# PolarisRisingWar/rgb-experiment

Measured on AMD Instinct MI355X. Metric: aggregated edges/sec (full-graph GCN d=128, reference epoch = train fwd+bwd+Adam + 2 eval fwd), higher is better.
Workload: dtype f32

## Files before the change

include/rgbx_hip.h:

```cpp
#ifndef RGBX_HIP_H
#define RGBX_HIP_H

#include <stddef.h>
#include <stdint.h>

#ifdef __cplusplus
extern "C" {
#endif

#define RGBX_VERSION 501

#define RGBX_OK 0
#define RGBX_E_ARG (-1)
#define RGBX_E_RANGE (-2)
#define RGBX_E_ALIGN (-3)
#define RGBX_E_WS (-4)
#define RGBX_E_SHAPE (-5)

typedef void* rgbx_stream_t;

enum {
  RGBX_LOOPS_KEEP = 0,
  RGBX_LOOPS_ADD_REMAINING = 1,
  RGBX_LOOPS_REMOVE_ADD = 2
// ... 169 lines not shown
  int64_t N, K, Nout;
  const rgbx_row_split_t* split;
  const float* w_pos;
  float* z_pos_out;
  const uint8_t* col_sel;
} rgbx_fused_layer_t;

int rgbx_fused_layer_f32(const rgbx_fused_layer_t* layer, rgbx_stream_t stream);

int rgbx_blocked_to_rows_f32(const float* src, int64_t blk_cols, int64_t blk_stride, float* dst, int64_t ldd,
                             int64_t n, int64_t d, const float* bias, rgbx_stream_t stream);

int rgbx_appnp_f32(const int32_t* rowptr, const int32_t* col, const float* w, const float* h,
                   int64_t ldh, float* out, float* tmp, int64_t ldo, int64_t N, int64_t d, int K,
                   float alpha, const rgbx_row_split_t* split, rgbx_stream_t stream);


int rgbx_dagnn_gate_fwd_f32(const float* h0, int64_t ld0, const float* hops, int64_t hop_stride, int64_t ldh,
                            const float* s, const float* b, float* out, int64_t ldo, int64_t N, int64_t d, int K,
                            rgbx_stream_t stream);

int rgbx_dagnn_gate_bwd_workspace_bytes(int64_t d, size_t* bytes);
int rgbx_dagnn_gate_bwd_f32(const float* h0, int64_t ld0, const float* hops, int64_t hop_stride, int64_t ldh,
                            const float* s, const float* b, const float* gout, int64_t ldg, float* d0,
                            int64_t ldd0, float* dk, int64_t d_stride, int64_t ldd, float* g_s, float* g_b,
                            void* ws, size_t ws_bytes, int64_t N, int64_t d, int K, rgbx_stream_t stream);


int rgbx_gru_step_supported(int64_t C);
int rgbx_gru_step_f32(const int32_t* rowptr, const int32_t* col, const float* x, int64_t ldx, const float* wt,
                      const float* wt_root, const float* bias, float* out, int64_t ldo, float* z_out, int64_t ldz,
                      float* pre_out, int64_t ldp, int64_t N, int64_t C, const rgbx_row_split_t* split,
                      rgbx_stream_t stream);

int rgbx_gru_gate_fwd_f32(const float* pre, int64_t ldp, const float* x, int64_t ldx, float* out, int64_t ldo,
                          int64_t N, int64_t C, rgbx_stream_t stream);

int rgbx_gru_gate_bwd_f32(const float* pre, int64_t ldp, const float* x, int64_t ldx, const float* gout, int64_t ldg,
                          float* dpre, int64_t lddp, float* dx, int64_t lddx, int64_t N, int64_t C,
                          rgbx_stream_t stream);


int rgbx_gat_scores_f32(const float* hfeat, int64_t ldh, const float* att_src,
                        const float* att_dst, float* a_src, float* a_dst, int64_t n, int H, int C,
                        rgbx_stream_t stream);

int rgbx_gat_scores_bwd_scratch_floats(int64_t n, int H, int C, int64_t* count);

int rgbx_gat_scores_bwd_f32(const float* hfeat, int64_t ldh, const float* g_a_src, const float* g_a_dst,
                            int64_t n_dst, const float* att_src, const float* att_dst, float* g_hfeat,
                            int64_t ldgh, float* g_att_src, float* g_att_dst, float* scratch,
                            int64_t scratch_floats, int64_t n, int H, int C, rgbx_stream_t stream);

int rgbx_gat_aggregate_fwd_f32(const int32_t* rowptr, const int32_t* col, const float* hfeat,
                               int64_t ldh, const float* a_src, const float* att_src,
                               float* a_dst, const float* att_dst, const float* out_scale, const float* bias,
                               float* out, int64_t ldo, float* m, float* rden, float* out_pos, float* a_pos,
                               int64_t N, int H, int C, float slope, const rgbx_row_split_t* split,
                               rgbx_stream_t stream);

int rgbx_gat_edge_softmax_f32(const int32_t* rowptr, const int32_t* col, const float* a_src, const float* a_dst,
                              float slope, float* alpha, float* alpha_pos, float* m, float* rden, float* a_pos,
                              int64_t N, const rgbx_row_split_t* split, rgbx_stream_t stream);

int rgbx_gat_bwd_dst_f32(const int32_t* rowptr, const int32_t* col, const float* hfeat,
                         int64_t ldh, const float* a_src, const float* a_dst, const float* m,
                         const float* rden, const float* out, int64_t ldo, const float* gout,
                         int64_t ldg, float* nodeq, float* g_a_dst, int64_t N, int H, int C,
                         float slope, rgbx_stream_t stream);

int rgbx_gat_bwd_prep_f32(const float* a_dst, const float* m, const float* rden, const float* out,
                          int64_t ldo, const float* bias, const float* gout, int64_t ldg, float* nodeq,
                          const float* out_pos, const float* a_pos, float slope, float* g_a_dst,
                          int64_t N, int H, int C, rgbx_stream_t stream);

int rgbx_gat_bwd_src_f32(const int32_t* rowptr_t, const int32_t* col_t, const float* hfeat,
                         int64_t ldh, const float* a_src, const float* nodeq, const float* gout,
                         int64_t ldg, float* g_hfeat, int64_t ldgh, float* g_a_src, float* ds,
                         const float* att2, const float* g_a_dst, int64_t N, int H, int C, float slope,
                         const rgbx_row_split_t* split, rgbx_stream_t stream);



int rgbx_supergat_supported(int H, int C);

int rgbx_supergat_loss_records(int64_t N, const rgbx_row_split_t* split, int64_t* count);

int rgbx_supergat_aggregate_fwd_f32(const int32_t* rowptr, const int32_t* col, const float* hfeat, int64_t ldh,
                                    const float* att_l, const float* att_r, const float* bias, float* out, int64_t ldo,
                                    float* m, float* rden, int64_t N, int H, int C, float slope, const uint32_t* seed,
                                    float p_drop, float pos_ratio, float* loss_records, int64_t n_loss_records,
                                    double* pos_stats, const rgbx_row_split_t* split, rgbx_stream_t stream);

int rgbx_supergat_bwd_dst_f32(const int32_t* rowptr, const int32_t* col, const float* hfeat, int64_t ldh,
                              const float* att_l, const float* att_r, const float* m, const float* rden,
                              const float* out, int64_t ldo, const float* bias, const float* gout, int64_t ldg,
                              float* nodeq, float* g_hfeat, int64_t ldgh, float* g_ar, int64_t N, int H, int C,
                              float slope, const uint32_t* seed, float p_drop, float pos_ratio, const float* gl,
                              const rgbx_row_split_t* split, rgbx_stream_t stream);

int rgbx_supergat_bwd_src_f32(const int32_t* rowptr_t, const int32_t* col_t, const int32_t* t2f, const float* hfeat,
                              int64_t ldh, const float* att_l, const float* nodeq, const float* gout, int64_t ldg,
                              float* g_hfeat, int64_t ldgh, float* g_al, int64_t N, int H, int C, float slope,
                              const uint32_t* seed, float p_drop, float pos_ratio, const float* gl,
                              const rgbx_row_split_t* split, rgbx_stream_t stream);

int rgbx_supergat_sample_negatives(const uint64_t* keys, int64_t n_keys, int64_t N, const uint32_t* seed, int64_t n_neg,
                                   int redraws, int64_t* neg, uint8_t* valid, rgbx_stream_t stream);

int rgbx_supergat_neg_loss_fwd_f32(const float* hfeat, int64_t ldh, const int64_t* neg, const uint8_t* valid,
                                   int64_t n_neg, int H, int C, float* loss_records, int64_t n_loss_records,
                                   double* neg_stats, rgbx_stream_t stream);

int rgbx_supergat_neg_loss_bwd_f32(const float* hfeat, int64_t ldh, const int64_t* neg, const uint8_t* valid,
                                   int64_t n_neg, int H, int C, const float* gl, float* g_hfeat, int64_t ldgh,
                                   rgbx_stream_t stream);

int rgbx_supergat_draws_u8(const uint32_t* seed, int64_t nnz, int H, float p_drop, float pos_ratio, uint8_t* pos,
                           uint8_t* drop, rgbx_stream_t stream);



int rgbx_gatv2_supported(int H, int C);

int rgbx_gatv2_fwd_f32(const int32_t* rowptr, const int32_t* col, const float* xl, int64_t ldl, const float* xr,
                       int64_t ldr, const float* att, const float* bias, float* out, int64_t ldo, float* m, float* rden,
                       int64_t N, int H, int C, float slope, const uint32_t* seed, float p_drop,
                       const rgbx_row_split_t* split, rgbx_stream_t stream);

int rgbx_gatv2_att_partial_floats(int64_t N, int H, int C, const rgbx_row_split_t* split, int64_t* count);

int rgbx_gatv2_bwd_dst_f32(const int32_t* rowptr, const int32_t* col, const float* xl, int64_t ldl, const float* xr,
                           int64_t ldr, const float* att, const float* m, const float* rden, const float* out,
                           int64_t ldo, const float* bias, const float* gout, int64_t ldg, float* nodeq, float* g_xr,
                           int64_t ldgr, float* g_att, float* att_partial, int64_t n_att_partial, int64_t N, int H,
                           int C, float slope, const uint32_t* seed, float p_drop, const rgbx_row_split_t* split,
                           rgbx_stream_t stream);

int rgbx_gatv2_bwd_src_f32(const int32_t* rowptr_t, const int32_t* col_t, const int32_t* t2f, const float* xl,
                           int64_t ldl, const float* xr, int64_t ldr, const float* att, const float* nodeq,
                           const float* gout, int64_t ldg, float* g_xl, int64_t ldgl, int64_t N, int H, int C,
                           float slope, const uint32_t* seed, float p_drop, const rgbx_row_split_t* split,
                           rgbx_stream_t stream);

int rgbx_gatv2_draws_u8(const uint32_t* seed, int64_t nnz, int H, float p_drop, uint8_t* keep, rgbx_stream_t stream);


int rgbx_gemm_tn_workspace_bytes(int64_t K, int64_t M, int64_t N, size_t* bytes);

int rgbx_gemm_tn_f32(const float* A, int64_t lda, const float* B, int64_t ldb, float* C, int64_t ldc,
                     float* a_colsum, int64_t K, int64_t M, int64_t N, float alpha, void* workspace,
                     size_t workspace_bytes, rgbx_stream_t stream);


int rgbx_bn_scratch_doubles(int64_t N, int64_t d, int64_t* count);

int rgbx_bn_stats_f32(const float* x, int64_t ldx, int64_t N, int64_t d, double* sums, double* scratch,
                      int64_t scratch_doubles, rgbx_stream_t stream);

int rgbx_bn_finalize_f32(const double* packed, const float* weight, const float* bias, float eps, float momentum,
                         float* running_mean, float* running_var, float* mean, float* rstd, float* scale,
                         float* shift, int64_t d, rgbx_stream_t stream);

int rgbx_fold_bn_linear_f32(const float* W, int64_t ldw, const float* Wr, int64_t ldwr, const float* bias,
                            const float* bias2, const float* gamma, const float* beta, const float* running_mean,
                            const float* running_var, float eps, float* wt, float* wrt, float* b_out, int64_t Nout,
                            int64_t K, rgbx_stream_t stream);

int rgbx_bn_bwd_finalize_f32(const double* glob, const double* local, const double* count, const float* weight,
                             const float* rstd, float* ca, float* cb, float* ck, float* g_weight, float* g_bias,
                             int64_t d, rgbx_stream_t stream);

int rgbx_affine_cols_f32(const float* x, int64_t ldx, const float* scale, const float* shift, float* y,
                         int64_t ldy, int64_t N, int64_t d, rgbx_stream_t stream);

int rgbx_bn_bwd_reduce_f32(const float* gy, int64_t ldg, const float* x, int64_t ldx, const float* mean,
                           const float* rstd, int64_t N, int64_t d, double* sums, double* scratch,
                           int64_t scratch_doubles, rgbx_stream_t stream);

int rgbx_bn_bwd_apply_f32(const float* gy, int64_t ldg, const float* x, int64_t ldx, const float* mean,
                          const float* rstd, const float* ca, const float* cb, const float* ck, float* gx,
                          int64_t ldgx, int64_t N, int64_t d, rgbx_stream_t stream);


int rgbx_masked_nll_scratch_doubles(int64_t N, int want_accuracy, int64_t* count);

int rgbx_masked_nll_fwd_f32(const float* logp, int64_t ld, const int64_t* y, const uint8_t* mask,
                            int64_t N, int64_t C, double* stats, double* scratch,
                            int64_t scratch_doubles, int want_accuracy, rgbx_stream_t stream);

int rgbx_masked_nll_bwd_f32(const int64_t* y, const uint8_t* mask, int64_t N, int64_t C,
                            const float* scale, float* grad, int64_t ldg, rgbx_stream_t stream);

int rgbx_masked_ce_fwd_f32(const float* logits, int64_t ld, const int64_t* y, const uint8_t* mask, int64_t N,
                           int64_t C, double* stats, double* scratch, int64_t scratch_doubles,
                           rgbx_stream_t stream);

int rgbx_masked_ce_fwd_blocked_f32(const float* logits, int64_t blk_cols, int64_t blk_stride, const float* bias,
                                   const int64_t* y, const uint8_t* mask, int64_t N, int64_t C, double* stats,
                                   double* scratch, int64_t scratch_doubles, rgbx_stream_t stream);

int rgbx_masked_ce_bwd_f32(const float* logits, int64_t ld, const int64_t* y, const uint8_t* mask, int64_t N,
                           int64_t C, const float* scale, float* grad, int64_t ldg, rgbx_stream_t stream);


int rgbx_coalesce_workspace_bytes(int64_t E, int64_t N, int mirror, size_t* bytes);
int rgbx_coalesce_keys_i64(const int64_t* row, const int64_t* col, int64_t E, int64_t N, int mirror,
                           uint64_t* keys_out, uint64_t* counts, void* workspace, size_t workspace_bytes,
                           rgbx_stream_t stream);
int rgbx_split_edge_keys_i64(const uint64_t* keys, const uint64_t* counts, int64_t cap, int64_t N, int64_t* out_row,
                             int64_t* out_col, rgbx_stream_t stream);

int rgbx_py_random_shuffle_i64(int64_t seed, int64_t n, int64_t* perm);


int rgbx_gather_rows_f32(const float* src, int64_t lds, const int32_t* idx, int64_t n, int64_t d,
                         float* dst, int64_t ldd, rgbx_stream_t stream);

int rgbx_scatter_add_rows_f32(const float* src, int64_t lds, const int32_t* idx, int64_t n,
                              int64_t d, float* dst, int64_t ldd, rgbx_stream_t stream);

int rgbx_paced_copy_f32(const float* src, float* dst, int64_t n, int workgroups, int nontemporal, rgbx_stream_t stream);



int rgbx_faconv_supported(int64_t C);

int rgbx_faconv_scores_f32(const float* x, int64_t ldx, const float* att_l, const float* att_r, float* alr, int64_t N,
                           int64_t C, rgbx_stream_t stream);

int rgbx_faconv_fwd_f32(const int32_t* rowptr, const int32_t* col, const float* w, const float* x, int64_t ldx,
                        const float* alr, const float* x0, int64_t ldx0, float eps, float* out, int64_t ldo, int64_t N,
                        int64_t C, const uint32_t* seed, float p_drop, const rgbx_row_split_t* split,
                        rgbx_stream_t stream);

int rgbx_faconv_bwd_dst_f32(const int32_t* rowptr, const int32_t* col, const float* w, const float* x, int64_t ldx,
                            const float* alr, const float* gout, int64_t ldg, float* g_alr, int64_t N, int64_t C,
                            const uint32_t* seed, float p_drop, const rgbx_row_split_t* split, rgbx_stream_t stream);

int rgbx_faconv_bwd_src_f32(const int32_t* rowptr_t, const int32_t* col_t, const float* w_t, const int32_t* t2f,
                            const float* x, int64_t ldx, const float* alr, const float* gout, int64_t ldg,
                            const float* att_l, const float* att_r, float* g_alr, float* g_x, int64_t ldgx, int64_t N,
                            int64_t C, const uint32_t* seed, float p_drop, const rgbx_row_split_t* split,
                            rgbx_stream_t stream);

int rgbx_faconv_edge_coef_f32(const int32_t* rowptr, const int32_t* col, const float* w, const int32_t* slot,
                              const float* alr, int transposed, int64_t N, const uint32_t* seed, float p_drop,
                              float* coef, float* q, rgbx_stream_t stream);

int rgbx_faconv_edge_dot_f32(const int32_t* rowptr, const int32_t* col, const float* q, const float* a, int64_t lda,
                             const float* b, int64_t ldb, float* out, int64_t out_stride, int64_t N, int64_t C,
                             rgbx_stream_t stream);

int rgbx_faconv_draws_u8(const uint32_t* seed, int64_t nnz, float p_drop, uint8_t* keep, rgbx_stream_t stream);

#ifdef __cplusplus
}
#endif
#endif
```

rgb_experiment_amd/_lib.py:

```python
import ctypes
import os

import torch

_HERE = os.path.dirname(os.path.abspath(__file__))
LIB_PATH = os.path.join(_HERE, "csrc", "librgbx_hip.so")

_P = ctypes.c_void_p
_I64 = ctypes.c_int64
_I = ctypes.c_int
_F = ctypes.c_float

class RowSplit(ctypes.Structure):
    _fields_ = [("threshold", ctypes.c_int32), ("n_chunks", ctypes.c_int32), ("n_long", ctypes.c_int32),
                ("chunk_begin", ctypes.c_void_p), ("chunk_end", ctypes.c_void_p), ("chunk_row", ctypes.c_void_p),
                ("long_row", ctypes.c_void_p),
                ("long_chunk_ptr", ctypes.c_void_p), ("partial", ctypes.c_void_p)]


class MultiOut(ctypes.Structure):
    _fields_ = [(f, t) for name in ("sum", "mean", "var", "std", "max", "argmax", "min", "argmin")
                for f, t in ((name, ctypes.c_void_p), ("ld_" + name, ctypes.c_int64))]


class MultiGrad(ctypes.Structure):
    _fields_ = [(f, t) for name in ("a", "b", "x", "gmax", "argmax", "gmin", "argmin")
                for f, t in ((name, ctypes.c_void_p), ("ld_" + name, ctypes.c_int64))]


class CeEpilogue(ctypes.Structure):
    _fields_ = [("y", ctypes.c_void_p), ("mask", ctypes.c_void_p), ("grad_scale", ctypes.c_void_p),
                ("stats", ctypes.c_void_p), ("scratch", ctypes.c_void_p), ("mask_groups", ctypes.c_int32),
                ("rows", ctypes.c_void_p), ("n_rows", ctypes.c_int64), ("skip_unselected", ctypes.c_int32)]


class SpmmEpilogue(ctypes.Structure):
    _fields_ = [("ce", ctypes.c_void_p), ("n_classes", ctypes.c_int64), ("out_colsums", ctypes.c_void_p),
                ("stats_ws", ctypes.c_void_p), ("stats_ws_bytes", ctypes.c_size_t)]


class FusedLayer(ctypes.Structure):
    _fields_ = [("rowptr", _P), ("col", _P), ("w", _P), ("rs", _P), ("x", _P), ("ldx", _I64),
                ("x_blk_cols", _I64), ("x_blk_stride", _I64), ("wt", _P), ("x_root", _P), ("ldr", _I64),
                ("xr_blk_cols", _I64), ("xr_blk_stride", _I64), ("wt_root", _P), ("bias", _P), ("out", _P),
                ("ldo", _I64), ("out_blk", _P), ("ob_cols", _I64), ("ob_stride", _I64), ("z_out", _P), ("ldz", _I64),
                ("pre_scale", _P), ("pre_shift", _P), ("pre_rowsum", _P), ("out_colsums", _P), ("stats_ws", _P),
                ("stats_ws_bytes", ctypes.c_size_t), ("ce", _P), ("N", _I64), ("K", _I64), ("Nout", _I64),
                ("split", _P), ("w_pos", _P), ("z_pos_out", _P), ("col_sel", _P)]


SIGNATURES = {
    "rgbx_csr_workspace_bytes": [_I64, _I64, ctypes.POINTER(ctypes.c_size_t)],
    "rgbx_csr_build": [_P, _P, _I64, _I64, _I, _P, _P, _P, _P, ctypes.c_size_t, _P],
    "rgbx_deg_inv_sqrt_f32": [_P, _I64, _P, _P],
    "rgbx_gcn_norm_f32": [_P, _P, _I64, _P, _P, _P],
    "rgbx_inv_degree_f32": [_P, _I64, _P, _P],
    "rgbx_loop_weights_f32": [_P, _P, _P, _I64, _I64, _I, _F, _P, _P, _P],
    "rgbx_edge_slot_weights_f32": [_P, _I64, _P, _I64, _P, _P, _P],
    "rgbx_weighted_deg_inv_sqrt_f32": [_P, _P, _I64, _P, _P],
    "rgbx_gcn_norm_weighted_f32": [_P, _P, _P, _I64, _P, _P, _P],
    "rgbx_edge_dot_supported": [_I64],
    "rgbx_edge_dot_f32": [_P, _P, _P, _I64, _P, _I64, _P, _I64, _I64, _P, _P],
    "rgbx_gcn_norm_bwd_f32": [_P, _P, _P, _P, _P, _P, _P, _P, _P, _P, _I64, _I64, _P, _P, _P],
    "rgbx_spmm_csr_f32": [_P, _P, _P, _P, _P, _I64, _P, _I64, _P, _P, _I64, _I64, _I64, _F, _F, _P, _P],
    "rgbx_spmm_csr_extremum_supported": [_I64],
    "rgbx_spmm_csr_extremum_f32": [_P, _P, _P, _I64, _P, _I64, _P, _I64, _I64, _I, _P, _P],
    "rgbx_extremum_bwd_f32": [_P, _P, _P, _P, _I64, _P, _P, _I64, _I64, _I64, _P, _P],
    "rgbx_spmm_csr_multi_supported": [_I64],
    "rgbx_spmm_csr_multi_partial_words": [_I64, _I64, _I, ctypes.POINTER(ctypes.c_int64)],
    "rgbx_spmm_csr_multi_f32": [_P, _P, _P, _I64, _P, _I64, _I64, _P, _P],
    "rgbx_multi_bwd_f32": [_P, _P, _P, _P, _P, _I64, _I64, _I64, _P, _P],
    "rgbx_spmm_csr_epilogue_supported": [_I64],
    "rgbx_spmm_csr_epilogue_f32": [_P, _P, _P, _P, _P, _I64, _P, _I64, _P, _P, _I64, _I64, _I64, _F, _F, _P, _P, _P],
    "rgbx_spmm_csr_short_rows_supported": [_I64],
    "rgbx_spmm_csr_short_rows_f32": [_P, _P, _P, _P, _I64, _P, _P, _I64, _I64, _I64, _P],
    "rgbx_spmm_linear_supported": [_I64, _I64, _I],
    "rgbx_spmm_linear_stats_workspace_bytes": [_I64, _I64, ctypes.POINTER(ctypes.c_size_t)],
    "rgbx_spmm_linear_f32": [_P, _P, _P, _P, _P, _I64, _P, _P, _I64, _P, _P, _P, _I64, _P, _I64, _P, _P, _P, _P, _P,
                             ctypes.c_size_t, _P, _I64, _I64, _I64, _P, _P],
    "rgbx_fused_layer_f32": [_P, _P],
    "rgbx_blocked_to_rows_f32": [_P, _I64, _I64, _P, _I64, _I64, _I64, _P, _P],
    "rgbx_appnp_f32": [_P, _P, _P, _P, _I64, _P, _P, _I64, _I64, _I64, _I, _F, _P, _P],
    "rgbx_dagnn_gate_fwd_f32": [_P, _I64, _P, _I64, _I64, _P, _P, _P, _I64, _I64, _I64, _I, _P],
    "rgbx_dagnn_gate_bwd_workspace_bytes": [_I64, ctypes.POINTER(ctypes.c_size_t)],
    "rgbx_dagnn_gate_bwd_f32": [_P, _I64, _P, _I64, _I64, _P, _P, _P, _I64, _P, _I64, _P, _I64, _I64, _P, _P, _P,
                                ctypes.c_size_t, _I64, _I64, _I, _P],
    "rgbx_gru_step_supported": [_I64],
    "rgbx_gru_step_f32": [_P, _P, _P, _I64, _P, _P, _P, _P, _I64, _P, _I64, _P, _I64, _I64, _I64, _P, _P],
    "rgbx_gru_gate_fwd_f32": [_P, _I64, _P, _I64, _P, _I64, _I64, _I64, _P],
    "rgbx_gru_gate_bwd_f32": [_P, _I64, _P, _I64, _P, _I64, _P, _I64, _P, _I64, _I64, _I64, _P],
    "rgbx_gat_scores_f32": [_P, _I64, _P, _P, _P, _P, _I64, _I, _I, _P],
    "rgbx_gat_scores_bwd_scratch_floats": [_I64, _I, _I, ctypes.POINTER(ctypes.c_int64)],
    "rgbx_gat_scores_bwd_f32": [_P, _I64, _P, _P, _I64, _P, _P, _P, _I64, _P, _P, _P, _I64, _I64, _I, _I, _P],
    "rgbx_gat_aggregate_fwd_f32": [_P, _P, _P, _I64, _P, _P, _P, _P, _P, _P, _P, _I64, _P, _P, _P, _P, _I64, _I, _I, _F, _P,
                                   _P],
    "rgbx_gat_edge_softmax_f32": [_P, _P, _P, _P, _F, _P, _P, _P, _P, _P, _I64, _P, _P],
    "rgbx_gat_bwd_dst_f32": [_P, _P, _P, _I64, _P, _P, _P, _P, _P, _I64, _P, _I64, _P, _P, _I64, _I, _I,
                             _F, _P],
    "rgbx_gat_bwd_prep_f32": [_P, _P, _P, _P, _I64, _P, _P, _I64, _P, _P, _P, _F, _P, _I64, _I, _I, _P],
    "rgbx_gat_bwd_src_f32": [_P, _P, _P, _I64, _P, _P, _P, _I64, _P, _I64, _P, _P, _P, _P, _I64, _I, _I, _F, _P, _P],
    "rgbx_supergat_supported": [_I, _I],
    "rgbx_supergat_loss_records": [_I64, _P, ctypes.POINTER(ctypes.c_int64)],
    "rgbx_supergat_aggregate_fwd_f32": [_P, _P, _P, _I64, _P, _P, _P, _P, _I64, _P, _P, _I64, _I, _I, _F, _P, _F, _F, _P,
                                        _I64, _P, _P, _P],
    "rgbx_supergat_bwd_dst_f32": [_P, _P, _P, _I64, _P, _P, _P, _P, _P, _I64, _P, _P, _I64, _P, _P, _I64, _P, _I64, _I, _I,
                                  _F, _P, _F, _F, _P, _P, _P],
    "rgbx_supergat_bwd_src_f32": [_P, _P, _P, _P, _I64, _P, _P, _P, _I64, _P, _I64, _P, _I64, _I, _I, _F, _P, _F, _F, _P,
                                  _P, _P],
    "rgbx_supergat_sample_negatives": [_P, _I64, _I64, _P, _I64, _I, _P, _P, _P],
    "rgbx_supergat_neg_loss_fwd_f32": [_P, _I64, _P, _P, _I64, _I, _I, _P, _I64, _P, _P],
    "rgbx_supergat_neg_loss_bwd_f32": [_P, _I64, _P, _P, _I64, _I, _I, _P, _P, _I64, _P],
    "rgbx_supergat_draws_u8": [_P, _I64, _I, _F, _F, _P, _P, _P],
    "rgbx_gatv2_supported": [_I, _I],
    "rgbx_gatv2_fwd_f32": [_P, _P, _P, _I64, _P, _I64, _P, _P, _P, _I64, _P, _P, _I64, _I, _I, _F, _P, _F, _P, _P],
    "rgbx_gatv2_att_partial_floats": [_I64, _I, _I, _P, ctypes.POINTER(ctypes.c_int64)],
    "rgbx_gatv2_bwd_dst_f32": [_P, _P, _P, _I64, _P, _I64, _P, _P, _P, _P, _I64, _P, _P, _I64, _P, _P, _I64, _P, _P, _I64,
                               _I64, _I, _I, _F, _P, _F, _P, _P],
    "rgbx_gatv2_bwd_src_f32": [_P, _P, _P, _P, _I64, _P, _I64, _P, _P, _P, _I64, _P, _I64, _I64, _I, _I, _F, _P, _F, _P,
                               _P],
    "rgbx_gatv2_draws_u8": [_P, _I64, _I, _F, _P, _P],
    "rgbx_gemm_tn_workspace_bytes": [_I64, _I64, _I64, ctypes.POINTER(ctypes.c_size_t)],
    "rgbx_gemm_tn_f32": [_P, _I64, _P, _I64, _P, _I64, _P, _I64, _I64, _I64, _F, _P, ctypes.c_size_t, _P],
    "rgbx_bn_scratch_doubles": [_I64, _I64, ctypes.POINTER(ctypes.c_int64)],
    "rgbx_bn_stats_f32": [_P, _I64, _I64, _I64, _P, _P, _I64, _P],
    "rgbx_bn_finalize_f32": [_P, _P, _P, _F, _F, _P, _P, _P, _P, _P, _P, _I64, _P],
    "rgbx_fold_bn_linear_f32": [_P, _I64, _P, _I64, _P, _P, _P, _P, _P, _P, _F, _P, _P, _P, _I64, _I64, _P],
    "rgbx_bn_bwd_finalize_f32": [_P, _P, _P, _P, _P, _P, _P, _P, _P, _P, _I64, _P],
    "rgbx_affine_cols_f32": [_P, _I64, _P, _P, _P, _I64, _I64, _I64, _P],
    "rgbx_bn_bwd_reduce_f32": [_P, _I64, _P, _I64, _P, _P, _I64, _I64, _P, _P, _I64, _P],
    "rgbx_bn_bwd_apply_f32": [_P, _I64, _P, _I64, _P, _P, _P, _P, _P, _P, _I64, _I64, _I64, _P],
    "rgbx_masked_nll_scratch_doubles": [_I64, _I, ctypes.POINTER(ctypes.c_int64)],
    "rgbx_masked_nll_fwd_f32": [_P, _I64, _P, _P, _I64, _I64, _P, _P, _I64, _I, _P],
    "rgbx_masked_ce_fwd_f32": [_P, _I64, _P, _P, _I64, _I64, _P, _P, _I64, _P],
    "rgbx_masked_ce_fwd_blocked_f32": [_P, _I64, _I64, _P, _P, _P, _I64, _I64, _P, _P, _I64, _P],
    "rgbx_masked_ce_bwd_f32": [_P, _I64, _P, _P, _I64, _I64, _P, _P, _I64, _P],
    "rgbx_masked_nll_bwd_f32": [_P, _P, _I64, _I64, _P, _P, _I64, _P],
    "rgbx_coalesce_workspace_bytes": [_I64, _I64, _I, ctypes.POINTER(ctypes.c_size_t)],
    "rgbx_coalesce_keys_i64": [_P, _P, _I64, _I64, _I, _P, _P, _P, ctypes.c_size_t, _P],
    "rgbx_split_edge_keys_i64": [_P, _P, _I64, _I64, _P, _P, _P],
    "rgbx_gather_rows_f32": [_P, _I64, _P, _I64, _I64, _P, _I64, _P],
    "rgbx_scatter_add_rows_f32": [_P, _I64, _P, _I64, _I64, _P, _I64, _P],
    "rgbx_paced_copy_f32": [_P, _P, _I64, _I, _I, _P],
    "rgbx_py_random_shuffle_i64": [_I64, _I64, _P],
    "rgbx_faconv_supported": [_I64],
    "rgbx_faconv_scores_f32": [_P, _I64, _P, _P, _P, _I64, _I64, _P],
    "rgbx_faconv_fwd_f32": [_P, _P, _P, _P, _I64, _P, _P, _I64, _F, _P, _I64, _I64, _I64, _P, _F, _P, _P],
    "rgbx_faconv_bwd_dst_f32": [_P, _P, _P, _P, _I64, _P, _P, _I64, _P, _I64, _I64, _P, _F, _P, _P],
    "rgbx_faconv_bwd_src_f32": [_P, _P, _P, _P, _P, _I64, _P, _P, _I64, _P, _P, _P, _P, _I64, _I64, _I64, _P, _F, _P,
                                _P],
    "rgbx_faconv_edge_coef_f32": [_P, _P, _P, _P, _P, _I, _I64, _P, _F, _P, _P, _P],
    "rgbx_faconv_edge_dot_f32": [_P, _P, _P, _P, _I64, _P, _I64, _P, _I64, _I64, _I64, _P],
    "rgbx_faconv_draws_u8": [_P, _I64, _F, _P, _P],
}
EXPORTS = ["rgbx_version", "rgbx_last_error_string"] + list(SIGNATURES)

_lib = None


def bind(path, strict=True):
    lib = ctypes.CDLL(path)
    lib.rgbx_version.restype = _I
    lib.rgbx_version.argtypes = []
    lib.rgbx_last_error_string.restype = ctypes.c_char_p
    lib.rgbx_last_error_string.argtypes = []
    for name, argtypes in SIGNATURES.items():
        if not strict and not hasattr(lib, name):
            continue
        fn = getattr(lib, name)
        fn.restype = _I
        fn.argtypes = argtypes
    return lib


def load():
    global _lib
    if _lib is not None:
        return _lib
    if not os.path.exists(LIB_PATH):
        raise RuntimeError(
            f"rgb_experiment_amd: {LIB_PATH} is not built — run `python -c 'import __graft_entry__ as g; "
            "g.build()'` (or `make -C rgb_experiment_amd/csrc`). There is no CPU fallback.")
    _lib = bind(LIB_PATH)
    return _lib


def use(lib):
    global _lib
    _lib = lib


def check(rc, what):
    if rc != 0:
        msg = load().rgbx_last_error_string().decode(errors="replace")
        kind = "argument error" if rc < 0 else "hipError"
        raise RuntimeError(f"{what} failed ({kind} {rc}): {msg}")


def require_device(*tensors):
    for t in tensors:
        if t is not None and not t.is_cuda:
            raise RuntimeError(
                "rgb_experiment_amd: the message-passing path runs in HIP kernels on an MI355X device; "
                f"got a tensor on '{t.device}'. There is no CPU fallback (oracle/ is test-only).")


def stream_ptr():
    return torch.cuda.current_stream().cuda_stream


def ptr(t):
    return 0 if t is None else t.data_ptr()


def mat(t, name="tensor"):
    if t.dtype != torch.float32 or t.dim() != 2:
        raise RuntimeError(f"{name}: expected a 2-D float32 tensor, got {t.dtype} {tuple(t.shape)}")
    if t.size(1) > 1 and t.stride(1) != 1:
        raise RuntimeError(f"{name}: rows must be contiguous (stride {t.stride()})")
    ld = t.stride(0) if t.size(0) > 1 else max(t.size(1), 1)
    return t.data_ptr(), ld
```

rgb_experiment_amd/csrc/bn.hip:

```cpp
#include "rgbx_common.h"

namespace rgbx {
namespace {

constexpr int kMaxBlocks = 1024;

struct ColMap {
  int cv;
  int rg;
};

__host__ __device__ inline ColMap col_map(int d, int vec) {
  int cv = (d + vec - 1) / vec;
  if (cv > 256) cv = 256;
  ColMap m{cv, 256 / cv};
  return m;
}

template <int VEC, bool BWD>
__global__ void __launch_bounds__(256)
col_reduce_kernel(const float* __restrict__ a, int64_t lda, const float* __restrict__ b, int64_t ldb,
                  const float* __restrict__ mean, const float* __restrict__ rstd, int64_t N, int d,
                  double* __restrict__ part) {
  extern __shared__ double sh[];
  const ColMap M = col_map(d, VEC);
  const int tid = threadIdx.x;
  const int cvi = tid % M.cv, rgi = tid / M.cv;
  const bool thread_ok = rgi < M.rg;
  const int stride_c = M.cv * VEC;
  for (int cbase = 0; cbase < d; cbase += stride_c) {
    const int c = cbase + cvi * VEC;
    const bool active = thread_ok && c < d;
    double s0[VEC], s1[VEC];
    float mu[VEC], rs[VEC];
#pragma unroll
    for (int i = 0; i < VEC; ++i) { s0[i] = s1[i] = 0.0; mu[i] = 0.f; rs[i] = 1.f; }
    if (BWD && active) {
      load_vec<VEC>(mu, mean + c);
      load_vec<VEC>(rs, rstd + c);
    }
    if (active) {
      for (int64_t r = (int64_t)blockIdx.x * M.rg + rgi; r < N; r += (int64_t)gridDim.x * M.rg) {
        float va[VEC];
        load_vec<VEC>(va, a + r * lda + c);
        if constexpr (BWD) {
          float vb[VEC];
          load_vec<VEC>(vb, b + r * ldb + c);
#pragma unroll
          for (int i = 0; i < VEC; ++i) {
            s0[i] += (double)va[i];
            s1[i] += (double)(va[i] * ((vb[i] - mu[i]) * rs[i]));
          }
        } else {
#pragma unroll
          for (int i = 0; i < VEC; ++i) {
            s0[i] += (double)va[i];
            s1[i] += (double)va[i] * (double)va[i];
          }
        }
      }
    }
    __syncthreads();
    if (thread_ok) {
#pragma unroll
      for (int i = 0; i < VEC; ++i) {
        sh[(rgi * 2 + 0) * stride_c + cvi * VEC + i] = s0[i];
        sh[(rgi * 2 + 1) * stride_c + cvi * VEC + i] = s1[i];
      }
    }
    __syncthreads();
    if (rgi == 0 && active) {
#pragma unroll
      for (int i = 0; i < VEC; ++i) {
        if (c + i < d) {
          double t0 = 0.0, t1 = 0.0;
          for (int g = 0; g < M.rg; ++g) {
            t0 += sh[(g * 2 + 0) * stride_c + cvi * VEC + i];
            t1 += sh[(g * 2 + 1) * stride_c + cvi * VEC + i];
          }
          part[((int64_t)blockIdx.x * 2 + 0) * d + c + i] = t0;
          part[((int64_t)blockIdx.x * 2 + 1) * d + c + i] = t1;
        }
      }
    }
  }
}

__global__ void __launch_bounds__(256)
col_finish_kernel(const double* __restrict__ part, int n_blocks, int d, double* __restrict__ sums) {
  __shared__ double sh[32][8];
  const int j = threadIdx.x & 7, q = threadIdx.x >> 3;
  const int c = blockIdx.x * 8 + j;
  double s = 0.0;
  if (c < 2 * d) {
    const int which = c / d, col = c % d;
    for (int b = q; b < n_blocks; b += 32) s += part[((int64_t)b * 2 + which) * d + col];
  }
  sh[q][j] = s;
  __syncthreads();
  if (q == 0 && c < 2 * d) {
    double t = 0.0;
#pragma unroll
    for (int k = 0; k < 32; ++k) t += sh[k][j];
    sums[c] = t;
  }
}

template <int VEC>
__global__ void __launch_bounds__(256)
affine_kernel(const float* __restrict__ x, int64_t ldx, const float* __restrict__ scale,
              const float* __restrict__ shift, float* __restrict__ y, int64_t ldy, int64_t N, int d) {
  const int per_row = (d + VEC - 1) / VEC;
  const int64_t total = N * per_row;
  for (int64_t idx = (int64_t)blockIdx.x * blockDim.x + threadIdx.x; idx < total;
       idx += (int64_t)gridDim.x * blockDim.x) {
    const int64_t r = idx / per_row;
    const int c = (int)(idx % per_row) * VEC;
    float v[VEC], sc[VEC], sf[VEC];
    load_vec<VEC>(v, x + r * ldx + c);
    load_vec<VEC>(sc, scale + c);
    load_vec<VEC>(sf, shift + c);
#pragma unroll
    for (int i = 0; i < VEC; ++i) v[i] = fmaf(v[i], sc[i], sf[i]);
    store_vec<VEC>(y + r * ldy + c, v);
  }
}

template <int VEC>
__global__ void __launch_bounds__(256)
bn_bwd_apply_kernel(const float* __restrict__ gy, int64_t ldg, const float* __restrict__ x, int64_t ldx,
                    const float* __restrict__ mean, const float* __restrict__ rstd, const float* __restrict__ ca,
                    const float* __restrict__ cb, const float* __restrict__ ck, float* __restrict__ gx,
                    int64_t ldgx, int64_t N, int d) {
  const int per_row = (d + VEC - 1) / VEC;
  const int64_t total = N * per_row;
  for (int64_t idx = (int64_t)blockIdx.x * blockDim.x + threadIdx.x; idx < total;
       idx += (int64_t)gridDim.x * blockDim.x) {
    const int64_t r = idx / per_row;
    const int c = (int)(idx % per_row) * VEC;
    float g[VEC], v[VEC], mu[VEC], rs[VEC], a[VEC], b[VEC], k[VEC];
    load_vec<VEC>(g, gy + r * ldg + c);
    load_vec<VEC>(v, x + r * ldx + c);
    load_vec<VEC>(mu, mean + c);
    load_vec<VEC>(rs, rstd + c);
    load_vec<VEC>(a, ca + c);
    load_vec<VEC>(b, cb + c);
    load_vec<VEC>(k, ck + c);
#pragma unroll
    for (int i = 0; i < VEC; ++i) g[i] = (g[i] - a[i] - (v[i] - mu[i]) * rs[i] * b[i]) * k[i];
    store_vec<VEC>(gx + r * ldgx + c, g);
  }
}

int reduce_grid(int64_t N, int d, int vec) {
  const ColMap M = col_map(d, vec);
  int64_t b = cdiv(N, (int64_t)M.rg * 16);
  if (b > kMaxBlocks) b = kMaxBlocks;
  return (int)(b < 1 ? 1 : b);
}

bool vec4_ok(int64_t d, std::initializer_list<const void*> ptrs, std::initializer_list<int64_t> lds) {
  bool ok = d % 4 == 0;
  for (const void* p : ptrs) ok = ok && aligned16(p);
  for (int64_t ld : lds) ok = ok && ld % 4 == 0;
  return ok;
}

template <bool BWD>
int run_reduce(const float* a, int64_t lda, const float* b, int64_t ldb, const float* mean, const float* rstd,
               int64_t N, int64_t d, double* sums, double* scratch, int64_t scratch_doubles, hipStream_t s,
               const char* name) {
  if (N < 0 || d <= 0 || !sums) return fail(RGBX_E_ARG, "%s: bad argument", name);
  if (d >= INT32_MAX) return fail(RGBX_E_RANGE, "%s: d exceeds int32", name);
  if (N == 0) {
    RGBX_HIP(hipMemsetAsync(sums, 0, 2 * d * sizeof(double), s));
    return RGBX_OK;
  }
  if (!a || lda < d || (BWD && (!b || ldb < d || !mean || !rstd)) || !scratch)
    return fail(RGBX_E_ARG, "%s: null pointer or leading dimension < d", name);
  const bool v4 = BWD ? vec4_ok(d, {a, b, mean, rstd}, {lda, ldb}) : vec4_ok(d, {a}, {lda});
  const int vec = v4 ? 4 : 1;
  const int grid = reduce_grid(N, (int)d, vec);
  if (scratch_doubles < (int64_t)grid * 2 * d)
    return fail(RGBX_E_WS, "%s: scratch %lld < %lld doubles", name, (long long)scratch_doubles,
                (long long)grid * 2 * d);
  const ColMap M = col_map((int)d, vec);
  const size_t lds = (size_t)M.rg * 2 * M.cv * vec * sizeof(double);
  if (v4)
    col_reduce_kernel<4, BWD><<<grid, 256, lds, s>>>(a, lda, b, ldb, mean, rstd, N, (int)d, scratch);
  else
    col_reduce_kernel<1, BWD><<<grid, 256, lds, s>>>(a, lda, b, ldb, mean, rstd, N, (int)d, scratch);
  RGBX_CHECK_LAUNCH(name);
  col_finish_kernel<<<(int)cdiv(2 * d, 8), 256, 0, s>>>(scratch, grid, (int)d, sums);
  RGBX_CHECK_LAUNCH("col_finish_kernel");
  return RGBX_OK;
}

__global__ void __launch_bounds__(256)
bn_finalize_kernel(const double* __restrict__ packed, const float* __restrict__ weight,
                   const float* __restrict__ bias, float eps, float momentum, float* __restrict__ running_mean,
                   float* __restrict__ running_var, float* __restrict__ mean, float* __restrict__ rstd,
                   float* __restrict__ scale, float* __restrict__ shift, int d) {
  const int c = blockIdx.x * blockDim.x + threadIdx.x;
  if (c >= d) return;
  const double n = packed[2 * d];
  const double m64 = packed[c] / n;
  double v64 = packed[d + c] / n - m64 * m64;
  v64 = v64 > 0.0 ? v64 : 0.0;
  const float m = (float)m64, var = (float)v64;
  const float r = 1.0f / sqrtf(var + eps);
  const float sc = weight[c] * r;
  mean[c] = m;
  rstd[c] = r;
  scale[c] = sc;
  shift[c] = bias[c] - m * sc;
  if (running_mean) {
    const double nm1 = n > 1.0 ? n - 1.0 : 1.0;
    const float unbiased = var * (float)(n / nm1);
    running_mean[c] = running_mean[c] * (1.0f - momentum) + momentum * m;
    running_var[c] = running_var[c] * (1.0f - momentum) + momentum * unbiased;
  }
}

__global__ void __launch_bounds__(256)
bn_bwd_finalize_kernel(const double* __restrict__ glob, const double* __restrict__ local,
                       const double* __restrict__ count, const float* __restrict__ weight,
                       const float* __restrict__ rstd, float* __restrict__ ca, float* __restrict__ cb,
                       float* __restrict__ ck, float* __restrict__ g_weight, float* __restrict__ g_bias, int d) {
  const int c = blockIdx.x * blockDim.x + threadIdx.x;
  if (c >= d) return;
  const double n = *count;
  ca[c] = (float)(glob[c] / n);
  cb[c] = (float)(glob[d + c] / n);
  ck[c] = weight[c] * rstd[c];
  g_bias[c] = (float)local[c];
  g_weight[c] = (float)local[d + c];
}

__global__ void __launch_bounds__(256)
fold_bn_linear_kernel(const float* __restrict__ W, int64_t ldw, const float* __restrict__ Wr, int64_t ldwr,
                      const float* __restrict__ bias, const float* __restrict__ bias2,
                      const float* __restrict__ gamma, const float* __restrict__ beta,
                      const float* __restrict__ rmean, const float* __restrict__ rvar, float eps,
                      float* __restrict__ wt, float* __restrict__ wrt, float* __restrict__ b_out, int Nout, int K) {
  __shared__ float tile[2][32][33];
  __shared__ float sc[32];
  const int n0 = blockIdx.x * 32, k0 = blockIdx.y * 32;
  const int tx = threadIdx.x & 31, ty = threadIdx.x >> 5;
  if (threadIdx.x < 32) {
    const int n = n0 + threadIdx.x;
    float s = 1.f, t = 0.f;
    if (n < Nout && gamma) {
      s = gamma[n] * (1.0f / sqrtf(rvar[n] + eps));
      t = beta[n] - rmean[n] * s;
    }
    sc[threadIdx.x] = s;
    if (n < Nout && b_out && blockIdx.y == 0) {
      float b = bias ? bias[n] : 0.f;
      if (bias2) b += bias2[n];
      b_out[n] = b * s + t;
    }
  }
  for (int r = ty; r < 32; r += 8) {
    const int n = n0 + r, k = k0 + tx;
    const bool ok = n < Nout && k < K;
    tile[0][r][tx] = ok ? W[(int64_t)n * ldw + k] : 0.f;
    if (Wr) tile[1][r][tx] = ok ? Wr[(int64_t)n * ldwr + k] : 0.f;
  }
  __syncthreads();
  for (int r = ty; r < 32; r += 8) {
    const int k = k0 + r, n = n0 + tx;
    if (k < K && n < Nout) {
      wt[(int64_t)k * Nout + n] = tile[0][tx][r] * sc[tx];
      if (Wr) wrt[(int64_t)k * Nout + n] = tile[1][tx][r] * sc[tx];
    }
  }
}

int elt_grid(int64_t total) {
  int64_t b = cdiv(total, 256);
  return (int)(b < kMaxGrid ? (b < 1 ? 1 : b) : kMaxGrid);
}

}
}

using namespace rgbx;

extern "C" int rgbx_fold_bn_linear_f32(const float* W, int64_t ldw, const float* Wr, int64_t ldwr, const float* bias,
                                       const float* bias2, const float* gamma, const float* beta,
                                       const float* running_mean, const float* running_var, float eps, float* wt,
                                       float* wrt, float* b_out, int64_t Nout, int64_t K, rgbx_stream_t stream) {
  if (Nout <= 0 || K <= 0) return fail(RGBX_E_ARG, "fold_bn_linear: bad size");
  if (!W || !wt || (Wr && !wrt)) return fail(RGBX_E_ARG, "fold_bn_linear: null pointer");
  const bool bn = gamma || beta || running_mean || running_var;
  if (bn && !(gamma && beta && running_mean && running_var))
    return fail(RGBX_E_ARG, "fold_bn_linear: gamma, beta, running_mean and running_var go together");
  if (ldw < K || (Wr && ldwr < K)) return fail(RGBX_E_ARG, "fold_bn_linear: leading dimension too small");
  if (Nout >= INT32_MAX || K >= INT32_MAX) return fail(RGBX_E_RANGE, "fold_bn_linear: size exceeds int32");
  dim3 grid((unsigned)cdiv(Nout, 32), (unsigned)cdiv(K, 32));
  fold_bn_linear_kernel<<<grid, 256, 0, (hipStream_t)stream>>>(W, ldw, Wr, ldwr, bias, bias2, gamma, beta, running_mean,
                                                            running_var, eps, wt, wrt, b_out, (int)Nout, (int)K);
// ... 80 lines not shown
```

rgb_experiment_amd/csrc/gemm.hip:

```cpp
#include "rgbx_common.h"

namespace rgbx {
namespace {

constexpr int BM = 128, BN = 128, KT = 32;
using f32x16 = __attribute__((ext_vector_type(16))) float;

template <int W>
__device__ __forceinline__ void stage_tile(float* __restrict__ lds, const float* __restrict__ src,
                                           int64_t ld, int64_t k0, int64_t k_end, int c0, int ncols) {
  const int tid = threadIdx.x;
#pragma unroll 4
  for (int p = 0; p < KT * W / 256; ++p) {
    const int idx = p * 256 + tid;
    const int r = idx / W, c = idx % W;
    const int64_t k = k0 + r;
    lds[r * W + c] = (k < k_end && c0 + c < ncols) ? src[k * ld + c0 + c] : 0.f;
  }
}

template <int W>
__device__ __forceinline__ void fetch_tile(float4 (&regs)[KT * (W / 4) / 256], const float* __restrict__ src, int64_t ld,
                                           int64_t k0, int64_t k_end, int c0, int ncols) {
#pragma unroll
  for (int p = 0; p < KT * (W / 4) / 256; ++p) {
    const int idx = p * 256 + threadIdx.x;
    const int r = idx / (W / 4), c = (idx % (W / 4)) * 4;
    const int64_t k = k0 + r;
    regs[p] = make_float4(0.f, 0.f, 0.f, 0.f);
    if (k < k_end && c0 + c < ncols) regs[p] = *reinterpret_cast<const float4*>(src + k * ld + c0 + c);
  }
}

template <int W>
__device__ __forceinline__ void put_tile(float* __restrict__ lds, const float4 (&regs)[KT * (W / 4) / 256]) {
#pragma unroll
  for (int p = 0; p < KT * (W / 4) / 256; ++p) {
    const int idx = p * 256 + threadIdx.x;
    const int r = idx / (W / 4), c = (idx % (W / 4)) * 4;
    *reinterpret_cast<float4*>(lds + r * W + c) = regs[p];
  }
}

template <bool VEC4, int MT>
__global__ void __launch_bounds__(256)
gemm_tn_partial_kernel(const float* __restrict__ A, int64_t lda, const float* __restrict__ B, int64_t ldb,
                       float* __restrict__ part, float* __restrict__ colpart, int64_t K, int M, int N,
                       int64_t slab) {
  constexpr int MI = MT / 64;
  __shared__ float lds[KT * (MT + 128)];
  float* la = lds;
  float* lb = lds + KT * MT;
  const int split = blockIdx.x;
  const int m0 = blockIdx.y * MT, n0 = blockIdx.z * BN;
  const int64_t k_begin = (int64_t)split * slab;
  const int64_t k_end = k_begin + slab < K ? k_begin + slab : K;
  const int wave = threadIdx.x >> 6, lane = threadIdx.x & 63;
  const int wm = (wave >> 1) * (MT / 2), wn = (wave & 1) * 64;
  const int kr = lane >> 5, cc = lane & 31;

  f32x16 acc[MI][2];
#pragma unroll
  for (int i = 0; i < MI; ++i)
#pragma unroll
    for (int j = 0; j < 2; ++j)
#pragma unroll
      for (int r = 0; r < 16; ++r) acc[i][j][r] = 0.f;

  const bool sums = colpart != nullptr && blockIdx.z == 0 && threadIdx.x < MT;
  float csum = 0.f;
  auto consume = [&]() {
    if (sums) {
#pragma unroll 8
      for (int r = 0; r < KT; ++r) csum += la[r * MT + threadIdx.x];
    }
#pragma unroll 4
    for (int kk = 0; kk < KT; kk += 2) {
      float a[MI];
#pragma unroll
      for (int i = 0; i < MI; ++i) a[i] = la[(kk + kr) * MT + wm + i * 32 + cc];
      const float b0 = lb[(kk + kr) * 128 + wn + cc];
      const float b1 = lb[(kk + kr) * 128 + wn + 32 + cc];
#pragma unroll
      for (int i = 0; i < MI; ++i) {
        acc[i][0] = __builtin_amdgcn_mfma_f32_32x32x2f32(a[i], b0, acc[i][0], 0, 0, 0);
        acc[i][1] = __builtin_amdgcn_mfma_f32_32x32x2f32(a[i], b1, acc[i][1], 0, 0, 0);
      }
    }
  };
  if constexpr (VEC4) {
    float4 ra[KT * (MT / 4) / 256], rb[KT * 32 / 256];
    fetch_tile<MT>(ra, A, lda, k_begin, k_end, m0, M);
    fetch_tile<128>(rb, B, ldb, k_begin, k_end, n0, N);
    for (int64_t k0 = k_begin; k0 < k_end; k0 += KT) {
      __syncthreads();
      put_tile<MT>(la, ra);
      put_tile<128>(lb, rb);
      __syncthreads();
      if (k0 + KT < k_end) {
        fetch_tile<MT>(ra, A, lda, k0 + KT, k_end, m0, M);
        fetch_tile<128>(rb, B, ldb, k0 + KT, k_end, n0, N);
      }
      consume();
    }
  } else {
    for (int64_t k0 = k_begin; k0 < k_end; k0 += KT) {
      __syncthreads();
      stage_tile<MT>(la, A, lda, k0, k_end, m0, M);
      stage_tile<128>(lb, B, ldb, k0, k_end, n0, N);
      __syncthreads();
      consume();
    }
  }

  if (sums && m0 + (int)threadIdx.x < M) colpart[(int64_t)split * M + m0 + threadIdx.x] = csum;
  float* out = part + (int64_t)split * M * N;
#pragma unroll
  for (int i = 0; i < MI; ++i)
#pragma unroll
    for (int j = 0; j < 2; ++j)
#pragma unroll
      for (int r = 0; r < 16; ++r) {
        const int m = m0 + wm + i * 32 + (r & 3) + 8 * (r >> 2) + 4 * kr;
        const int n = n0 + wn + j * 32 + cc;
        if (m < M && n < N) out[(int64_t)m * N + n] = acc[i][j][r];
      }
}

__global__ void __launch_bounds__(256)
gemm_tn_reduce_kernel(const float* __restrict__ part, int S, int64_t MN, float* __restrict__ C, int N,
                      int64_t ldc, float alpha) {
  __shared__ float sh[8][32];
  const int j = threadIdx.x & 31, q = threadIdx.x >> 5;
  for (int64_t base = (int64_t)blockIdx.x * 32; base < MN; base += (int64_t)gridDim.x * 32) {
    const int64_t i = base + j;
    float s = 0.f;
    if (i < MN)
      for (int p = q; p < S; p += 8) s += part[(int64_t)p * MN + i];
    __syncthreads();
    sh[q][j] = s;
    __syncthreads();
    if (q == 0 && i < MN) {
      float t = 0.f;
#pragma unroll
      for (int k = 0; k < 8; ++k) t += sh[k][j];
      C[(i / N) * ldc + (i % N)] = alpha * t;
    }
  }
}

int tile_rows(int M) { return M <= 64 ? 64 : BM; }

int choose_splits(int64_t K, int M, int N) {
  const int64_t tiles = cdiv(M, tile_rows(M)) * cdiv(N, BN);
  int64_t s = cdiv(tile_rows(M) == 64 ? 1024 : 768, tiles);
  const int64_t max_s = cdiv(K, 16 * KT);
  if (s > max_s) s = max_s;
  if (s < 1) s = 1;
  return (int)s;
}

}
}

using namespace rgbx;

extern "C" int rgbx_gemm_tn_workspace_bytes(int64_t K, int64_t M, int64_t N, size_t* bytes) {
  if (!bytes || K < 0 || M < 0 || N < 0) return fail(RGBX_E_ARG, "gemm_tn_workspace_bytes: bad argument");
  if (M >= INT32_MAX || N >= INT32_MAX) return fail(RGBX_E_RANGE, "gemm_tn: M or N exceeds int32");
  *bytes = (size_t)choose_splits(K, (int)M, (int)N) * ((size_t)M * (size_t)N + (size_t)M) * sizeof(float);
  return RGBX_OK;
}

extern "C" int rgbx_gemm_tn_f32(const float* A, int64_t lda, const float* B, int64_t ldb, float* C,
                                int64_t ldc, float* a_colsum, int64_t K, int64_t M, int64_t N, float alpha,
                                void* workspace, size_t workspace_bytes, rgbx_stream_t stream) {
  if (K < 0 || M < 0 || N < 0) return fail(RGBX_E_ARG, "gemm_tn: negative size");
  if (M == 0 || N == 0) return RGBX_OK;
  if (!C || (K > 0 && (!A || !B))) return fail(RGBX_E_ARG, "gemm_tn: null pointer");
  if (M >= INT32_MAX || N >= INT32_MAX) return fail(RGBX_E_RANGE, "gemm_tn: M or N exceeds int32");
  if (lda < M || ldb < N || ldc < N) return fail(RGBX_E_ARG, "gemm_tn: leading dimension too small");
  size_t need = 0;
  if (int rc = rgbx_gemm_tn_workspace_bytes(K, M, N, &need)) return rc;
  if (!workspace || workspace_bytes < need)
    return fail(RGBX_E_WS, "gemm_tn: workspace %zu < %zu bytes", workspace_bytes, need);
  hipStream_t s = (hipStream_t)stream;
  const int S = choose_splits(K, (int)M, (int)N);
  const int64_t slab = cdiv(cdiv(K > 0 ? K : 1, S), KT) * KT;
  float* part = static_cast<float*>(workspace);
  float* colpart = a_colsum ? part + (size_t)S * M * N : nullptr;
  const int mt = tile_rows((int)M);
  dim3 grid(S, (unsigned)cdiv(M, mt), (unsigned)cdiv(N, BN));
  const bool v4 = aligned16(A) && aligned16(B) && lda % 4 == 0 && ldb % 4 == 0;
#define RGBX_GEMM_TN(V4, MT) \
  gemm_tn_partial_kernel<V4, MT><<<grid, 256, 0, s>>>(A, lda, B, ldb, part, colpart, K, (int)M, (int)N, slab)
  if (v4) { if (mt == 64) RGBX_GEMM_TN(true, 64); else RGBX_GEMM_TN(true, 128); }
  else { if (mt == 64) RGBX_GEMM_TN(false, 64); else RGBX_GEMM_TN(false, 128); }
#undef RGBX_GEMM_TN
  RGBX_CHECK_LAUNCH("gemm_tn_partial_kernel");
  const int64_t MN = M * N;
  int64_t rb = cdiv(MN, 32);
  if (rb > kMaxGrid) rb = kMaxGrid;
  gemm_tn_reduce_kernel<<<(int)rb, 256, 0, s>>>(part, S, MN, C, (int)N, ldc, alpha);
  RGBX_CHECK_LAUNCH("gemm_tn_reduce_kernel");
  if (a_colsum) {
    gemm_tn_reduce_kernel<<<(int)cdiv(M, 32), 256, 0, s>>>(colpart, S, M, a_colsum, (int)M, M, 1.0f);
    RGBX_CHECK_LAUNCH("gemm_tn_reduce_kernel");
  }
  return RGBX_OK;
}
```

rgb_experiment_amd/csrc/rgbx_common.h:

```cpp
#pragma once
#include <cstring>
#include <hip/hip_runtime.h>

#include <algorithm>
#include <cstdarg>
#include <cstdint>
#include <cstdio>
#include <initializer_list>

#include "../../include/rgbx_hip.h"

namespace rgbx {

constexpr int kWave = 64;

char* err_buf();

inline int fail(int code, const char* fmt, ...) {
  va_list ap;
  va_start(ap, fmt);
  vsnprintf(err_buf(), 256, fmt, ap);
  va_end(ap);
  return code;
}

inline int hip_fail(hipError_t e, const char* what) {
  snprintf(err_buf(), 256, "%s: %s", what, hipGetErrorString(e));
  return (int)e;
}

#define RGBX_CHECK_LAUNCH(what)                               \
  do {                                                        \
    hipError_t e_ = hipGetLastError();                        \
    if (e_ != hipSuccess) return ::rgbx::hip_fail(e_, what);  \
  } while (0)

#define RGBX_HIP(call)                                         \
  do {                                                         \
    hipError_t e_ = (call);                                    \
    if (e_ != hipSuccess) return ::rgbx::hip_fail(e_, #call);  \
  } while (0)

inline bool aligned16(const void* p) { return (reinterpret_cast<uintptr_t>(p) & 15u) == 0; }

inline int64_t cdiv(int64_t a, int64_t b) { return (a + b - 1) / b; }

template <int VEC> struct VecT;
template <> struct VecT<4> { using type = float4; };
template <> struct VecT<2> { using type = float2; };
template <> struct VecT<1> { using type = float; };

template <int VEC>
__device__ __forceinline__ void load_vec(float (&v)[VEC], const float* p) {
  using V = typename VecT<VEC>::type;
  const V t = *reinterpret_cast<const V*>(p);
  if constexpr (VEC == 4) { v[0] = t.x; v[1] = t.y; v[2] = t.z; v[3] = t.w; }
  else if constexpr (VEC == 2) { v[0] = t.x; v[1] = t.y; }
  else { v[0] = t; }
}

template <int VEC>
__device__ __forceinline__ void store_vec(float* p, const float (&v)[VEC]) {
  using V = typename VecT<VEC>::type;
  V t;
  if constexpr (VEC == 4) { t.x = v[0]; t.y = v[1]; t.z = v[2]; t.w = v[3]; }
  else if constexpr (VEC == 2) { t.x = v[0]; t.y = v[1]; }
  else { t = v[0]; }
  *reinterpret_cast<V*>(p) = t;
}

constexpr int kMaxGrid = 256 * 8 * 4;

}
```

rgb_experiment_amd/models/_stack.py:

```python
import torch
import torch.nn as nn
import torch.nn.functional as F

from ..nn import BatchNorm1d


class ModelOutput(dict):

    _LAZY = ("out", "x")

    def __init__(self, logits):
        super().__init__(emb=logits)

    def _log_probs(self):
        out = F.log_softmax(dict.__getitem__(self, "emb"), dim=1)
        dict.__setitem__(self, "out", out)
        dict.__setitem__(self, "x", out)
        return out

    def __missing__(self, key):
        if key in self._LAZY:
            return self._log_probs()
        raise KeyError(key)

    def get(self, key, default=None):
        if key in self._LAZY and not dict.__contains__(self, key):
            return self._log_probs()
        return dict.get(self, key, default)

    def __contains__(self, key):
        return key in self._LAZY or dict.__contains__(self, key)

    def keys(self):
        return ["out", "emb", "x"]

    def __iter__(self):
        return iter(self.keys())

    def __len__(self):
        return 3

    def values(self):
        return [self[k] for k in self.keys()]

    def items(self):
        return [(k, self[k]) for k in self.keys()]

    def copy(self):
        return dict(self.items())

    def pop(self, key, *default):
        if key in self._LAZY and not dict.__contains__(self, key):
            self._log_probs()
        return dict.pop(self, key, *default)

    def __eq__(self, other):
        return dict(self.items()) == other

    __hash__ = None

    def __repr__(self):
        return repr(dict(self.items()))


def model_output(logits):
    return ModelOutput(logits)


class ConvStack(nn.Module):

    def __init__(self, num_layers, dropout_rate, widths, make_conv, bn_width):
        super().__init__()
        if num_layers < 2:
            raise ValueError("num_layers must be at least 2")
        self.num_layers = num_layers
        self.dropout_rate = dropout_rate
        self.convs = nn.ModuleList(make_conv(i, widths[i], widths[i + 1]) for i in range(num_layers))
        self.bns = nn.ModuleList(BatchNorm1d(bn_width) for _ in range(num_layers - 1))

    def forward(self, x, edge_index, edge_weight=None):
        return model_output(self._run(x, edge_index, edge_weight=edge_weight))

    def masked_ce(self, x, edge_index, y, mask, edge_weight=None):
        return self._run(x, edge_index, ce=(y, mask), edge_weight=edge_weight)

    def masked_ce_pair(self, x, edge_index, y, mask_a, mask_b, edge_weight=None):
        return self._run(x, edge_index, ce=(y, (mask_a, mask_b)), edge_weight=edge_weight)[1]

    def _run(self, x, edge_index, ce=None, edge_weight=None):
        from .. import ops
        last = self.num_layers - 1
        ew = {}
        if edge_weight is not None:
            if any(type(c).__name__ != "GCNConv" for c in self.convs):
                raise ValueError(f"{type(self).__name__}: edge_weight is taken by stacks of GCNConv only")
            ew["edge_weight"] = edge_weight
        learned = edge_weight is not None and edge_weight.requires_grad and torch.is_grad_enabled()
        pending = None
        if self.training and torch.is_grad_enabled():
            self._train_forwards = getattr(self, "_train_forwards", 0) + 1
        folded = self._eval_operands() if (not torch.is_grad_enabled() and not self.training and x.is_cuda) else None
        agg0 = (self._input_aggregate(x, edge_index, edge_weight)
                if getattr(self, "cache_input_aggregate", False) and not learned else None)
        if folded is not None and agg0 is None and getattr(self, "collapse_eval", True):
            out = self._run_collapsed(x, edge_index, ce, edge_weight)
            if out is not None:
                return out
        for i, conv in enumerate(self.convs):
            bn = self.bns[i] if i < last else None
            if i == 0 and agg0 is not None and i < last:
                if folded is not None and folded[0] is not None:
                    x = conv.forward_from_aggregate(agg0, x, folded=folded[0])
                    continue
                if torch.is_grad_enabled() or bn is None or bn.training:
                    want = (bn is not None and bn.training and torch.is_grad_enabled()
                            and hasattr(bn, "begin_training_step"))
                    x, pending = conv.forward_from_aggregate(agg0, x, want_colsums=want), bn
                    continue
            if folded is not None and pending is None and folded[i] is not None:
                res = conv.forward_folded(x, edge_index, folded[i], ce=ce if i == last else None, **ew)
                if res is not None:
                    x = res
                    continue
            extra = dict(ew)
            if (bn is not None and bn.training and torch.is_grad_enabled() and getattr(conv, "emits_colsums", False)
                    and hasattr(bn, "begin_training_step")):
                extra["want_colsums"] = True
            if (i == last and ce is not None and getattr(conv, "accepts_ce", False)
                    and (not isinstance(ce[1], (tuple, list)) or getattr(conv, "accepts_ce_pair", False))):
                extra["ce"] = ce
            if pending is not None:
                sums = getattr(x, ops.COLSUMS, None)
                after = getattr(conv, "forward_after_bn", None)
                if after is not None:
                    x, pending = after(x, edge_index, pending, colsums=sums, **extra), bn
                    continue
                x, pending = (pending(x, colsums=sums) if sums is not None else pending(x)), None
            affine = None
            if bn is not None and getattr(conv, "folds_post_affine", False) and not torch.is_grad_enabled():
                fold = getattr(bn, "eval_affine", None)
                affine = fold() if fold is not None else None
            if affine is not None:
                x = conv(x, edge_index, post_affine=affine, **ew)
            else:
                x, pending = conv(x, edge_index, **extra), bn
        if ce is not None and not isinstance(x, tuple):
            x = ops.ce_from_logits(x, ce[0], ce[1])
        return x


def _layer_maps(conv):
    from ..graph import LOOPS_ADD_REMAINING, LOOPS_KEEP, LOOPS_REMOVE_ADD
    name = type(conv).__name__
    if getattr(conv, "aggr", "mean") != "mean":
        return None
    if name == "GCNConv":
        return conv.lin.weight, None, conv.bias, "gcn", LOOPS_ADD_REMAINING
    if name == "MySAGEConv" and conv.add_self_loops:
        return conv.lin_l.weight, conv.lin_r.weight, conv.lin_l.bias + conv.lin_r.bias, "mean", LOOPS_REMOVE_ADD
    if name == "SAGEConv":
        return conv.lin_l.weight, conv.lin_r.weight, conv.lin_l.bias, "mean", LOOPS_KEEP
    return None


def _collapsed_operands(self):
    from .. import ops
    tensors = list(self.parameters()) + list(self.buffers())
    key = (getattr(self, "_train_forwards", 0), ops.weights_epoch()) + tuple((t._version, t.data_ptr()) for t in tensors)
    cached = getattr(self, "_collapsed", None)
    if cached is not None and cached[0] == key:
        return cached[1]
    out = None
    convs, last = list(self.convs), self.num_layers - 1
    maps = [_layer_maps(c) for c in convs]
    C = getattr(convs[-1], "out_channels", 0)
    Cp = (C + 3) // 4 * 4
    if (all(m is not None for m in maps) and len({(m[3], m[4]) for m in maps}) == 1 and 0 < Cp <= 256
            and all(c.out_channels > Cp for c in convs[:-1])):
        affines = [getattr(self.bns[i], "eval_affine", lambda: None)() for i in range(last)]
        if all(a is not None for a in affines):
            with torch.no_grad():
                Q, d = None, None
                for l, (wl, wr, b, _, _) in enumerate(maps):
                    scale, shift = affines[l] if l < last else (None, None)
                    ml = wl.t() if scale is None else wl.t() * scale[None, :]
                    mr = None if wr is None else (wr.t() if scale is None else wr.t() * scale[None, :])
                    if Q is None:
                        Q, d = [mr, ml], [None, None]
                    else:
                        nq, nd = [None] * (len(Q) + 1), [None] * (len(Q) + 1)
                        for k in range(len(Q)):
                            for src, m, dst in ((Q, mr, k), (Q, ml, k + 1)):
                                if src[k] is not None and m is not None:
                                    nq[dst] = src[k] @ m if nq[dst] is None else nq[dst] + src[k] @ m
                            for m, dst in ((mr, k), (ml, k + 1)):
                                if d[k] is not None and m is not None:
                                    nd[dst] = d[k] @ m if nd[dst] is None else nd[dst] + d[k] @ m
                        Q, d = nq, nd
                    const = b if scale is None else b * scale + shift
                    d[0] = const if d[0] is None else d[0] + const
                pad = torch.nn.functional.pad
                have = [k for k, q in enumerate(Q) if q is not None]
                weight = torch.cat([pad(Q[k].t(), (0, 0, 0, Cp - C)) for k in have], dim=0).contiguous()
                shifts = [None if v is None else pad(v.detach(), (0, Cp - C)).contiguous() for v in d]
                out = (weight, have, shifts, C, Cp, maps[0][3], maps[0][4])
    self._collapsed = (key, out)
    return out


def _run_collapsed(self, x, edge_index, ce, edge_weight=None):
    from .. import ops
    from ..graph import get_graph
    operands = self._collapsed_operands()
    if operands is None:
        return None
    weight, have, shifts, C, Cp, kind, loops_mode = operands
    graph = get_graph(edge_index, x.size(0), loops_mode, edge_weight)
    if getattr(graph, "is_distributed", False) or not ops.rows_epilogue_ok(graph, Cp, x, None if ce is None else ce[0]):
        return None
    z = ops.linear(x, weight)
    block = {k: z[:, j * Cp:(j + 1) * Cp] for j, k in enumerate(have)}
    w, rs = ops._kind_weights(graph, kind)
    top = len(shifts) - 1
    u = block[top]
    for k in range(top - 1, 0, -1):
        u = ops.spmm_raw(graph.fwd, w, rs, u, y=block.get(k), a=1.0, b=1.0, bias=shifts[k], kind=f"{kind}_fwd")
    if ce is None:
        return ops.spmm_raw(graph.fwd, w, rs, u, y=block.get(0), a=1.0, b=1.0, bias=shifts[0], kind=f"{kind}_fwd")[:, :C]
    labels, mask = ce
    _, stats = ops.spmm_epilogue_raw(graph.fwd, w, rs, u, y=block.get(0), a=1.0, b=1.0, bias=shifts[0],
                                     ce=(labels, mask, None), n_classes=C, kind=f"{kind}_fwd")
    return None, stats


ConvStack._collapsed_operands = _collapsed_operands
ConvStack._run_collapsed = _run_collapsed


def _eval_operands(self):
    tensors = list(self.parameters()) + list(self.buffers())
    from .. import ops
    key = (getattr(self, "_train_forwards", 0), ops.weights_epoch()) + tuple((t._version, t.data_ptr()) for t in tensors)
    cached = getattr(self, "_folded_eval", None)
    if cached is None or cached[0] != key:
        last = self.num_layers - 1
        out = []
        for i, conv in enumerate(self.convs):
            bn = self.bns[i] if i < last else None
            make = getattr(conv, "eval_operands", None)
            ok = make is not None and (bn is None or (hasattr(bn, "eval_affine") and bn.affine and bn.track_running_stats))
            out.append(make(bn) if ok else None)
        cached = (key, out)
        self._folded_eval = cached
    return cached[1]


ConvStack._eval_operands = _eval_operands


def _input_aggregate(self, x, edge_index, edge_weight=None):
    if x.requires_grad or not x.is_cuda:
        return None
    key = (x.data_ptr(), x._version, tuple(x.shape), edge_index.data_ptr(), edge_index._version, tuple(edge_index.shape))
    if edge_weight is not None:
        key += (edge_weight.data_ptr(), edge_weight._version, tuple(edge_weight.shape))
    cached = getattr(self, "_agg0", None)
    if cached is None or cached[0] != key:
        make = getattr(self.convs[0], "aggregate_input", None)
        args = (x, edge_index) if edge_weight is None else (x, edge_index, edge_weight)
        cached = (key, make(*args) if make is not None else None, x, edge_index, edge_weight)
        self._agg0 = cached
    return cached[1]


ConvStack._input_aggregate = _input_aggregate


def _weighted_call(fn, fwd):
    import inspect
    return set(fwd) == {"x", "edge_index", "edge_weight"} and "edge_weight" in inspect.signature(fn).parameters


def masked_ce_pair(model, fwd, y, mask_a, mask_b):
    from .. import ops
    fn = getattr(model, "masked_ce_pair", None)
    if fn is not None and set(fwd) == {"x", "edge_index"} and fwd["x"].is_cuda:
        return fn(fwd["x"], fwd["edge_index"], y, mask_a, mask_b)
    if fn is not None and fwd["x"].is_cuda and _weighted_call(fn, fwd):
        return fn(fwd["x"], fwd["edge_index"], y, mask_a, mask_b, edge_weight=fwd["edge_weight"])
    emb = model(**fwd)["emb"]
    return torch.stack([ops.masked_ce_accuracy(emb, y, mask_a), ops.masked_ce_accuracy(emb, y, mask_b)])


def masked_ce(model, fwd, y, mask):
    from .. import ops
    fn = getattr(model, "masked_ce", None)
    if fn is not None and set(fwd) == {"x", "edge_index"} and fwd["x"].is_cuda:
# ... 5 lines not shown
```

rgb_experiment_amd/nn/batchnorm.py:

```python
import ctypes

import torch
import torch.nn as nn

from .. import _lib


def _scratch(n, d, device):
    cnt = ctypes.c_int64(0)
    _lib.check(_lib.load().rgbx_bn_scratch_doubles(n, d, ctypes.byref(cnt)), "rgbx_bn_scratch_doubles")
    return torch.empty(cnt.value, dtype=torch.float64, device=device), cnt.value


def column_sums(x):
    if not x.is_cuda:
        xd = x.double()
        return torch.stack([xd.sum(0), (xd * xd).sum(0)])
    px, ldx = _lib.mat(x, "x")
    n, d = x.shape
    sums = torch.empty((2, d), dtype=torch.float64, device=x.device)
    scratch, cnt = _scratch(n, d, x.device)
    _lib.check(_lib.load().rgbx_bn_stats_f32(px, ldx, n, d, _lib.ptr(sums), _lib.ptr(scratch), cnt, _lib.stream_ptr()),
               "rgbx_bn_stats_f32")
    return sums


def affine_cols(x, scale, shift):
    if not x.is_cuda:
        return x * scale + shift
    px, ldx = _lib.mat(x, "x")
    y = torch.empty((x.size(0), x.size(1)), dtype=torch.float32, device=x.device)
    _lib.check(_lib.load().rgbx_affine_cols_f32(px, ldx, _lib.ptr(scale), _lib.ptr(shift), _lib.ptr(y), y.stride(0),
                                                x.size(0), x.size(1), _lib.stream_ptr()), "rgbx_affine_cols_f32")
    return y


def bwd_sums(gy, x, mean, rstd):
    if not gy.is_cuda:
        xhat = (x - mean) * rstd
        return torch.stack([gy.double().sum(0), (gy * xhat).double().sum(0)])
    pg, ldg = _lib.mat(gy, "gy")
    px, ldx = _lib.mat(x, "x")
    n, d = x.shape
    sums = torch.empty((2, d), dtype=torch.float64, device=x.device)
    scratch, cnt = _scratch(n, d, x.device)
    _lib.check(_lib.load().rgbx_bn_bwd_reduce_f32(pg, ldg, px, ldx, _lib.ptr(mean), _lib.ptr(rstd), n, d, _lib.ptr(sums),
                                                  _lib.ptr(scratch), cnt, _lib.stream_ptr()), "rgbx_bn_bwd_reduce_f32")
    return sums


def bwd_apply(gy, x, mean, rstd, ca, cb, ck):
    if not gy.is_cuda:
        return (gy - ca - (x - mean) * rstd * cb) * ck
    pg, ldg = _lib.mat(gy, "gy")
    px, ldx = _lib.mat(x, "x")
    gx = torch.empty((x.size(0), x.size(1)), dtype=torch.float32, device=x.device)
    _lib.check(_lib.load().rgbx_bn_bwd_apply_f32(pg, ldg, px, ldx, _lib.ptr(mean), _lib.ptr(rstd), _lib.ptr(ca),
                                                 _lib.ptr(cb), _lib.ptr(ck), _lib.ptr(gx), gx.stride(0), x.size(0),
                                                 x.size(1), _lib.stream_ptr()), "rgbx_bn_bwd_apply_f32")
    return gx


class _BNTrain(torch.autograd.Function):

    @staticmethod
    def forward(ctx, x, weight, bias, eps, reduce, running, colsums=None):
        x = x if x.stride(-1) == 1 else x.contiguous()
        mean, rstd, scale, shift, n = train_statistics(x, weight, bias, eps, reduce, running, colsums)
        y = affine_cols(x, scale.contiguous(), shift.contiguous())
        ctx.save_for_backward(x, weight, mean, rstd, n)
        ctx.reduce = reduce
        return y

    @staticmethod
    def backward(ctx, gy):
        x, weight, mean, rstd, n = ctx.saved_tensors
        gx, gw, gb = train_backward(gy, x, weight, mean, rstd, n, ctx.reduce)
        return gx, gw, gb, None, None, None, None


def pack_statistics(x, colsums=None):
    d = x.size(1)
    count = torch.full((1,), float(x.size(0)), dtype=torch.float64, device=x.device)
    sums = colsums if colsums is not None and tuple(colsums.shape) == (2, d) else column_sums(x)
    return torch.cat([sums.reshape(-1), count])


def train_statistics(x, weight, bias, eps, reduce, running, colsums=None, packed=None):
    d = x.size(1)
    if packed is None:
        packed = reduce(pack_statistics(x, colsums))
    n = packed[2 * d:2 * d + 1]
    if x.is_cuda:
        mean, rstd, scale, shift = (torch.empty(d, dtype=torch.float32, device=x.device) for _ in range(4))
        rm, rv, mom = running if running is not None else (None, None, 0.0)
        _lib.check(_lib.load().rgbx_bn_finalize_f32(
            _lib.ptr(packed), _lib.ptr(weight.detach().contiguous()), _lib.ptr(bias.detach().contiguous()),
            float(eps), float(mom), _lib.ptr(rm), _lib.ptr(rv), _lib.ptr(mean), _lib.ptr(rstd), _lib.ptr(scale),
            _lib.ptr(shift), d, _lib.stream_ptr()), "rgbx_bn_finalize_f32")
    else:
        mean64 = packed[:d] / n
        var64 = (packed[d:2 * d] / n - mean64 * mean64).clamp_(min=0.0)
        mean, var = mean64.float(), var64.float()
        rstd = torch.rsqrt(var + eps)
        scale = weight.detach() * rstd
        shift = bias.detach() - mean * scale
        if running is not None:
            rm, rv, mom = running
            unbiased = var * (n / (n - 1).clamp(min=1)).float()
            rm.mul_(1 - mom).add_(mean, alpha=mom)
            rv.mul_(1 - mom).add_(unbiased, alpha=mom)
    return mean, rstd, scale, shift, n


def train_backward(gy, x, weight, mean, rstd, n, reduce, grads_out=None, sums=None):
    gy = gy if gy.stride(-1) == 1 else gy.contiguous()
    d = x.size(1)
    if sums is None:
        local = bwd_sums(gy, x, mean, rstd)
        glob = reduce(local.reshape(-1).clone())
    else:
        local, glob = sums
    if gy.is_cuda:
        ca, cb, ck = (torch.empty(d, dtype=torch.float32, device=gy.device) for _ in range(3))
        gw, gb = grads_out if grads_out is not None else (torch.empty(d, dtype=torch.float32, device=gy.device)
                                                          for _ in range(2))
        _lib.check(_lib.load().rgbx_bn_bwd_finalize_f32(
            _lib.ptr(glob), _lib.ptr(local), _lib.ptr(n), _lib.ptr(weight.detach().contiguous()), _lib.ptr(rstd),
            _lib.ptr(ca), _lib.ptr(cb), _lib.ptr(ck), _lib.ptr(gw), _lib.ptr(gb), d, _lib.stream_ptr()),
            "rgbx_bn_bwd_finalize_f32")
    else:
        glob = glob.reshape(2, -1)
        ca = (glob[0] / n).float().contiguous()
        cb = (glob[1] / n).float().contiguous()
        ck = (weight * rstd).contiguous()
        gw, gb = local[1].float(), local[0].float()
        if grads_out is not None:
            grads_out[0].copy_(gw)
            grads_out[1].copy_(gb)
            gw, gb = grads_out
    return bwd_apply(gy, x, mean, rstd, ca, cb, ck), gw, gb


class _AffineCols(torch.autograd.Function):

    @staticmethod
    def forward(ctx, x, scale, shift):
        x = x if x.stride(-1) == 1 else x.contiguous()
        ctx.save_for_backward(x, scale)
        return affine_cols(x, scale.detach().contiguous(), shift.detach().contiguous())

    @staticmethod
    def backward(ctx, gy):
        x, scale = ctx.saved_tensors
        gy = gy if gy.stride(-1) == 1 else gy.contiguous()
        gx = g_scale = g_shift = None
        if ctx.needs_input_grad[0]:
            gx = affine_cols(gy, scale.detach().contiguous(), torch.zeros_like(scale))
        if ctx.needs_input_grad[1]:
            g_scale = (gy * x).sum(0)
        if ctx.needs_input_grad[2]:
            g_shift = gy.sum(0)
        return gx, g_scale, g_shift


class BatchNorm1d(nn.BatchNorm1d):

    def _reduce(self, packed):
        return packed

    def _reducer(self, x):
        return self._reduce

    def eval_affine(self):
        if self.training or not self.affine or not self.track_running_stats:
            return None
        scale = self.weight * torch.rsqrt(self.running_var + self.eps)
        return scale, self.bias - self.running_mean * scale

    def forward(self, x, colsums=None):
        if x.dim() != 2 or not self.affine or not self.track_running_stats:
            return super().forward(x)
        if not self.training:
            scale, shift = self.eval_affine()
            if torch.is_grad_enabled() and (x.requires_grad or self.weight.requires_grad or self.bias.requires_grad):
                return _AffineCols.apply(x, scale, shift)
            return affine_cols(x if x.stride(-1) == 1 else x.contiguous(), scale.contiguous(), shift.contiguous())
        return _BNTrain.apply(x, self.weight, self.bias, self.eps, self._reducer(x), self.begin_training_step(), colsums)

    def begin_training_step(self):
        with torch.no_grad():
            self.num_batches_tracked += 1
        if self.momentum is None:
            m = 1.0 / float(self.num_batches_tracked)
        else:
            m = self.momentum
        return self.running_mean, self.running_var, m

    def folds_into_next_layer(self, x):
        return (self.training and self.affine and self.track_running_stats and x.dim() == 2 and x.is_cuda
                and torch.is_grad_enabled())
```

rgb_experiment_amd/nn/conv.py:

```python
import math

import torch
import torch.nn as nn

from .. import _lib, ops
from ..graph import LOOPS_ADD_REMAINING, LOOPS_KEEP, LOOPS_REMOVE_ADD, get_graph


def glorot_(t):
    a = math.sqrt(6.0 / (t.size(-2) + t.size(-1)))
    with torch.no_grad():
        t.uniform_(-a, a)
    return t


def _no_weight_grad(edge_weight, who):
    if edge_weight is not None and edge_weight.requires_grad:
        raise ValueError(f"{who}: edge_weight must not require grad (the gradient in the edge weights is implemented for "
                         "GCNConv only)")


AGGRS = {"mean": "mean", "max": "max", "min": "min", "add": "add", "sum": "add", "std": "std", "var": "var"}


def _set_aggr(conv, aggr, lists=False):
    if isinstance(aggr, (list, tuple)):
        if not lists:
            raise ValueError(f"{type(conv).__name__}: aggr must be one name out of {sorted(AGGRS)} (the layer has no "
                             f"projection for a concatenation of aggregates), got {aggr!r}")
        names = tuple(AGGRS.get(a) if isinstance(a, str) else None for a in aggr)
        if not names or None in names or len(set(names)) != len(names):
            raise ValueError(f"{type(conv).__name__}: aggr must be one of {sorted(AGGRS)} or a non-empty list of distinct "
                             f"ones, got {aggr!r}")
        conv.aggr = names
    elif not isinstance(aggr, str) or aggr not in AGGRS:
        raise ValueError(f"{type(conv).__name__}: aggr must be one of {sorted(AGGRS)}, got {aggr!r}")
    else:
        conv.aggr = AGGRS[aggr]
    if conv.aggr != "mean":
        conv.accepts_ce = conv.accepts_ce_pair = conv.folds_post_affine = conv.emits_colsums = False
    return len(conv.aggr) if isinstance(conv.aggr, tuple) else 1


def _aggregate(x, graph, aggr):
    if getattr(graph, "is_distributed", False):
        raise NotImplementedError(f"aggr={aggr!r} is not implemented on the partitioned (distributed) route")
    if isinstance(aggr, tuple):
        return ops.propagate_multi(x, graph, aggr)
    if aggr == "add":
        return ops.propagate_sum(x, graph)
    if aggr in ("std", "var"):
        return ops.propagate_std(x, graph) if aggr == "std" else ops.propagate_var(x, graph)
    return ops.propagate_max(x, graph) if aggr == "max" else ops.propagate_min(x, graph)


def _finish_composed(out, post_affine, ce):
    if post_affine is not None:
        out = out * post_affine[0] + post_affine[1]
    return out if ce is None else ops.ce_from_logits(out, ce[0], ce[1])


def _forward_folded(conv, x, edge_index, operands, ce, loops_mode, kind, root, edge_weight=None):
    if operands is None or torch.is_grad_enabled() or not x.is_cuda:
        return None
    graph = get_graph(edge_index, x.size(0), loops_mode, edge_weight)
    if getattr(graph, "is_distributed", False) or not ops.fused_linear_ok(graph, conv.in_channels, conv.out_channels,
                                                                          root=root, x=x):
        return None
    wt, b, wtr = operands
    w = graph.w if kind == "gcn" else None
    rs = graph.inv_deg if kind == "mean" else None
    if ce is not None:
        y, mask = ce
        if not ops.fused_ce_ok(graph, conv.in_channels, conv.out_channels, root, x, y):
            return None
        _, _, stats = ops.fused_layer(x, wt, csr=graph.fwd, w=w, rs=rs, bias=b, x_root=x if root else None,
                                      wt_root=wtr if root else None, ce=(y, mask, None), kind=f"{kind}_linear_fwd",
                                      select_rows=True)
        return None, stats
    out, _, _ = ops.fused_layer(x, wt, csr=graph.fwd, w=w, rs=rs, bias=b, x_root=x if root else None,
                                wt_root=wtr if root else None, kind=f"{kind}_linear_fwd")
    return out


def _aggregate_input(x, edge_index, loops_mode, kind, edge_weight=None):
    if edge_weight is not None and edge_weight.requires_grad:
        return None
    graph = get_graph(edge_index, x.size(0), loops_mode, edge_weight)
    if getattr(graph, "is_distributed", False) or not x.is_cuda or x.requires_grad:
        return None
    with torch.no_grad():
        return ops.propagate_gcn(x, graph) if kind == "gcn" else ops.propagate_mean(x, graph)


def _folded_from_aggregate(z, x, operands, root):
    wt, b, wtr = operands
    out, _, _ = ops.fused_layer(z, wt, bias=b, x_root=x if root else None, wt_root=wtr if root else None,
                                kind="cached_aggregate_linear_fwd")
    return out


class GCNConv(nn.Module):

    folds_post_affine = True
    emits_colsums = True

    def __init__(self, in_channels, out_channels):
        super().__init__()
        self.in_channels, self.out_channels = in_channels, out_channels
        self.lin = nn.Linear(in_channels, out_channels, bias=False)
        self.bias = nn.Parameter(torch.zeros(out_channels))
        self.reset_parameters()

    def reset_parameters(self):
        glorot_(self.lin.weight)
        nn.init.zeros_(self.bias)

    accepts_ce = True
    accepts_ce_pair = True

    def forward(self, x, edge_index, edge_weight=None, post_affine=None, want_colsums=False, ce=None):
        if ce is not None:
            return self._ce(x, edge_index, ce, None, None, edge_weight)
        weight, bias = self.lin.weight, self.bias
        if post_affine is not None:
            scale, shift = post_affine
            weight, bias = weight * scale[:, None], bias * scale + shift
        return self._conv(x, edge_index, weight, bias, want_colsums, edge_weight)

    def eval_operands(self, bn=None):
        return ops.fold_bn_linear(self.lin.weight, self.bias, bn=bn)

    def aggregate_input(self, x, edge_index, edge_weight=None):
        if self.in_channels > self.out_channels or not ops.aggregate_linear_ok(self.in_channels, self.out_channels):
            return None
        return _aggregate_input(x, edge_index, LOOPS_ADD_REMAINING, "gcn", edge_weight)

    def forward_from_aggregate(self, z, x, want_colsums=False, folded=None):
        if folded is not None:
            return _folded_from_aggregate(z, x, folded, False)
        return ops.aggregate_linear(z, self.lin.weight, self.bias, want_colsums=want_colsums)

    def forward_folded(self, x, edge_index, operands, ce=None, edge_weight=None):
        return _forward_folded(self, x, edge_index, operands, ce, LOOPS_ADD_REMAINING, "gcn", False, edge_weight)

    @staticmethod
    def _learned(edge_weight):
        return edge_weight is not None and edge_weight.requires_grad and torch.is_grad_enabled()

    def _ce(self, x, edge_index, ce, bn, colsums, edge_weight=None):
        y, mask = ce
        if self._learned(edge_weight):
            if bn is not None:
                x = bn(x, colsums=colsums)
            return ops.ce_from_logits(self.forward(x, edge_index, edge_weight), y, mask)
        graph = get_graph(edge_index, x.size(0), LOOPS_ADD_REMAINING, edge_weight)
        hand_over = bn is not None and bn.folds_into_next_layer(x)
        if ops.fused_ce_ok(graph, self.in_channels, self.out_channels, False, x, y) and (bn is None or hand_over):
            return ops.propagate_linear_ce(x, graph, "gcn", self.lin.weight, self.bias, None, y, mask, bn=bn,
                                           colsums=colsums)
        if bn is not None:
            x = bn(x, colsums=colsums)
        weight, bias, n = ops.pad_rows4(self.lin.weight, self.bias)
        if ops.rows_epilogue_ok(graph, n, x, y) and not ops.fused_linear_ok(graph, self.in_channels, self.out_channels, x=x):
            return ops.propagate_rows_ce(ops.linear(x, weight), graph, "gcn", n, self.out_channels, y, mask, bias=bias)
        return ops.ce_from_logits(self.forward(x, edge_index, edge_weight), y, mask)

    def forward_after_bn(self, x, edge_index, bn, colsums=None, want_colsums=False, ce=None, edge_weight=None):
        if ce is not None:
            return self._ce(x, edge_index, ce, bn, colsums, edge_weight)
        if self._learned(edge_weight):
            return self.forward(bn(x, colsums=colsums), edge_index, edge_weight, want_colsums=want_colsums)
        graph = get_graph(edge_index, x.size(0), LOOPS_ADD_REMAINING, edge_weight)
        if (bn.folds_into_next_layer(x) and not getattr(graph, "is_distributed", False)
                and ops.fused_linear_ok(graph, self.in_channels, self.out_channels, x=x)):
            return ops.bn_propagate_linear(x, bn, graph, "gcn", self.lin.weight, self.bias, colsums=colsums,
                                           want_colsums=want_colsums)
        return self.forward(bn(x, colsums=colsums), edge_index, edge_weight, want_colsums=want_colsums)

    def _conv(self, x, edge_index, weight, bias, want_colsums=False, edge_weight=None):
        graph = get_graph(edge_index, x.size(0), LOOPS_ADD_REMAINING, edge_weight)
        if self._learned(edge_weight):
            return ops.propagate_gcn_edge_weight(ops.linear(x, weight), edge_weight, graph, bias=bias)
        if ops.fused_linear_ok(graph, self.in_channels, self.out_channels, x=x):
            return ops.propagate_linear(x, graph, "gcn", weight, bias, want_colsums=want_colsums)
        if not x.requires_grad and self.in_channels <= self.out_channels:
            return ops.linear(ops.propagate_gcn(x, graph), weight, bias)
        if want_colsums and ops.rows_epilogue_ok(graph, self.out_channels, x):
            return ops.propagate_rows(ops.linear(x, weight), graph, "gcn", bias=bias, want_colsums=True)
        return ops.propagate_gcn(ops.linear(x, weight), graph, bias=bias)


class SAGEConv(nn.Module):

    folds_post_affine = True
    emits_colsums = True

    def __init__(self, in_channels, out_channels, aggr="mean"):
        super().__init__()
        self.in_channels, self.out_channels = in_channels, out_channels
        k = _set_aggr(self, aggr, lists=True)
        self.lin_l = nn.Linear(k * in_channels, out_channels, bias=True)
        self.lin_r = nn.Linear(in_channels, out_channels, bias=False)

    accepts_ce = True
    accepts_ce_pair = True

    def eval_operands(self, bn=None):
        if self.aggr != "mean":
            return None
        return ops.fold_bn_linear(self.lin_l.weight, self.lin_l.bias, root_weight=self.lin_r.weight, bn=bn)

    def aggregate_input(self, x, edge_index):
        if (self.aggr != "mean" or self.in_channels > self.out_channels
                or not ops.aggregate_linear_ok(self.in_channels, self.out_channels, True)):
            return None
        return _aggregate_input(x, edge_index, LOOPS_KEEP, "mean")

    def _forward_composed(self, x, edge_index):
        graph = get_graph(edge_index, x.size(0), LOOPS_KEEP)
        agg = _aggregate(x, graph, self.aggr)
        return ops.linear(agg, self.lin_l.weight, self.lin_l.bias) + ops.linear(x, self.lin_r.weight)

    def forward_from_aggregate(self, z, x, want_colsums=False, folded=None):
        if folded is not None:
            return _folded_from_aggregate(z, x, folded, True)
        return ops.aggregate_linear(z, self.lin_l.weight, self.lin_l.bias, self.lin_r.weight, x, want_colsums)

    def forward_folded(self, x, edge_index, operands, ce=None):
        if self.aggr != "mean":
            return None
        return _forward_folded(self, x, edge_index, operands, ce, LOOPS_KEEP, "mean", True)

    def _ce(self, x, edge_index, ce, bn, colsums):
        y, mask = ce
        graph = get_graph(edge_index, x.size(0), LOOPS_KEEP)
        hand_over = bn is not None and bn.folds_into_next_layer(x)
        if ops.fused_ce_ok(graph, self.in_channels, self.out_channels, True, x, y) and (bn is None or hand_over):
            return ops.propagate_linear_ce(x, graph, "mean", self.lin_l.weight, self.lin_l.bias, self.lin_r.weight, y,
                                           mask, bn=bn, colsums=colsums)
        if bn is not None:
            x = bn(x, colsums=colsums)
        if (ops.rows_epilogue_ok(graph, (self.out_channels + 3) // 4 * 4, x, y)
                and not ops.fused_linear_ok(graph, self.in_channels, self.out_channels, root=True, x=x)):
            h, n = self._transform_first(x, self.lin_l.weight, self.lin_l.bias, self.lin_r.weight)
            return ops.propagate_rows_ce(h, graph, "mean", n, self.out_channels, y, mask)
        return ops.ce_from_logits(self.forward(x, edge_index), y, mask)

    @staticmethod
    def _transform_first(x, w_l, b_l, w_r):
        w_l, b_l, n = ops.pad_rows4(w_l, b_l)
        w_r = ops.pad_rows4(w_r)[0]
        return ops.linear(x, torch.cat([w_l, w_r]), torch.cat([torch.zeros_like(b_l), b_l])), n

    def forward_after_bn(self, x, edge_index, bn, colsums=None, want_colsums=False, ce=None):
        if self.aggr != "mean":
            return _finish_composed(self._forward_composed(bn(x, colsums=colsums), edge_index), None, ce)
        if ce is not None:
            return self._ce(x, edge_index, ce, bn, colsums)
        graph = get_graph(edge_index, x.size(0), LOOPS_KEEP)
        if (bn.folds_into_next_layer(x) and not getattr(graph, "is_distributed", False)
                and ops.fused_linear_ok(graph, self.in_channels, self.out_channels, root=True, x=x)):
            return ops.bn_propagate_linear(x, bn, graph, "mean", self.lin_l.weight, self.lin_l.bias,
                                           root_weight=self.lin_r.weight, colsums=colsums, want_colsums=want_colsums)
        return self.forward(bn(x, colsums=colsums), edge_index, want_colsums=want_colsums)

    def forward(self, x, edge_index, post_affine=None, want_colsums=False, ce=None):
        if self.aggr != "mean":
            return _finish_composed(self._forward_composed(x, edge_index), post_affine, ce)
        if ce is not None:
            return self._ce(x, edge_index, ce, None, None)
        w_l, b_l, w_r = self.lin_l.weight, self.lin_l.bias, self.lin_r.weight
        if post_affine is not None:
            scale, shift = post_affine
            w_l, b_l, w_r = w_l * scale[:, None], b_l * scale + shift, w_r * scale[:, None]
        graph = get_graph(edge_index, x.size(0), LOOPS_KEEP)
        if ops.fused_linear_ok(graph, self.in_channels, self.out_channels, root=True, x=x):
            return ops.propagate_linear(x, graph, "mean", w_l, b_l, root_weight=w_r, want_colsums=want_colsums)
        if self.in_channels > self.out_channels and x.is_cuda and not getattr(graph, "is_distributed", False):
            h, n = self._transform_first(x, w_l, b_l, w_r)
            out = ops.propagate_rows(h, graph, "mean", n=n, want_colsums=want_colsums and n == self.out_channels)
            return out if n == self.out_channels else out[:, :self.out_channels]
        x_r = ops.linear(ops.target_rows(x, graph), w_r)
        if ops.fused_linear_ok(graph, self.in_channels, self.out_channels, x=x):
            return ops.propagate_linear(x, graph, "mean", w_l, b_l) + x_r
        if self.in_channels > self.out_channels:
            return ops.propagate_mean(ops.linear(x, w_l), graph) + b_l + x_r
        agg = ops.propagate_mean(x, graph)
        return ops.linear(agg, w_l, b_l) + x_r


class MySAGEConv(nn.Module):

    folds_post_affine = True
    emits_colsums = True

    def __init__(self, in_channels, out_channels, add_self_loops=True, aggr="mean"):
        super().__init__()
        self.in_channels, self.out_channels = in_channels, out_channels
        self.add_self_loops = add_self_loops
        _set_aggr(self, aggr)
        self.lin_l = nn.Linear(in_channels, out_channels)
        self.lin_r = nn.Linear(in_channels, out_channels)

    accepts_ce = True
    accepts_ce_pair = True

    def _forward_composed(self, x, edge_index):
        graph = get_graph(edge_index, x.size(0), LOOPS_REMOVE_ADD if self.add_self_loops else LOOPS_KEEP)
        h, n = self._transform_both(x, self.lin_l.weight, self.lin_l.bias, self.lin_r.weight, self.lin_r.bias)
        out = _aggregate(h[:, :n], graph, self.aggr) + h[:, n:]
        return out if n == self.out_channels else out[:, :self.out_channels]

    def eval_operands(self, bn=None):
        if not self.add_self_loops or self.aggr != "mean":
            return None
        return ops.fold_bn_linear(self.lin_l.weight, self.lin_l.bias, self.lin_r.bias, root_weight=self.lin_r.weight,
                                  bn=bn)

    def aggregate_input(self, x, edge_index):
        if (not self.add_self_loops or self.aggr != "mean" or self.in_channels > self.out_channels
                or not ops.aggregate_linear_ok(self.in_channels, self.out_channels, True)):
            return None
        return _aggregate_input(x, edge_index, LOOPS_REMOVE_ADD, "mean")

    def forward_from_aggregate(self, z, x, want_colsums=False, folded=None):
        if folded is not None:
            return _folded_from_aggregate(z, x, folded, True)
        return ops.aggregate_linear(z, self.lin_l.weight, self.lin_l.bias + self.lin_r.bias, self.lin_r.weight, x,
                                    want_colsums)

    def forward_folded(self, x, edge_index, operands, ce=None):
        if self.aggr != "mean":
            return None
        return _forward_folded(self, x, edge_index, operands, ce, LOOPS_REMOVE_ADD, "mean", True)

    def _ce(self, x, edge_index, ce, bn, colsums):
        y, mask = ce
        if self.add_self_loops:
            graph = get_graph(edge_index, x.size(0), LOOPS_REMOVE_ADD)
            hand_over = bn is not None and bn.folds_into_next_layer(x)
            if ops.fused_ce_ok(graph, self.in_channels, self.out_channels, True, x, y) and (bn is None or hand_over):
                return ops.propagate_linear_ce(x, graph, "mean", self.lin_l.weight, self.lin_l.bias + self.lin_r.bias,
                                               self.lin_r.weight, y, mask, bn=bn, colsums=colsums)
        if bn is not None:
            x = bn(x, colsums=colsums)
        mode = LOOPS_REMOVE_ADD if self.add_self_loops else LOOPS_KEEP
        graph = get_graph(edge_index, x.size(0), mode)
        fused = self.add_self_loops and ops.fused_linear_ok(graph, self.in_channels, self.out_channels, root=True, x=x)
        if ops.rows_epilogue_ok(graph, (self.out_channels + 3) // 4 * 4, x, y) and not fused:
            h, n = self._transform_both(x, self.lin_l.weight, self.lin_l.bias, self.lin_r.weight, self.lin_r.bias)
            return ops.propagate_rows_ce(h, graph, "mean", n, self.out_channels, y, mask)
        return ops.ce_from_logits(self.forward(x, edge_index), y, mask)

    @staticmethod
    def _transform_both(x, w_l, b_l, w_r, b_r):
        w_l, b_l, n = ops.pad_rows4(w_l, b_l)
        w_r, b_r, _ = ops.pad_rows4(w_r, b_r)
        return ops.linear(x, torch.cat([w_l, w_r]), torch.cat([b_l, b_r])), n

    def forward_after_bn(self, x, edge_index, bn, colsums=None, want_colsums=False, ce=None):
        if self.aggr != "mean":
            return _finish_composed(self._forward_composed(bn(x, colsums=colsums), edge_index), None, ce)
        if ce is not None:
            return self._ce(x, edge_index, ce, bn, colsums)
        if self.add_self_loops:
            graph = get_graph(edge_index, x.size(0), LOOPS_REMOVE_ADD)
            if (bn.folds_into_next_layer(x) and not getattr(graph, "is_distributed", False)
                    and ops.fused_linear_ok(graph, self.in_channels, self.out_channels, root=True, x=x)):
                return ops.bn_propagate_linear(x, bn, graph, "mean", self.lin_l.weight,
                                               self.lin_l.bias + self.lin_r.bias, root_weight=self.lin_r.weight,
                                               colsums=colsums, want_colsums=want_colsums)
        return self.forward(bn(x, colsums=colsums), edge_index, want_colsums=want_colsums)

    def forward(self, x, edge_index, post_affine=None, want_colsums=False, ce=None):
        if self.aggr != "mean":
            return _finish_composed(self._forward_composed(x, edge_index), post_affine, ce)
        if ce is not None:
            return self._ce(x, edge_index, ce, None, None)
        w_l, b_l, w_r, b_r = self.lin_l.weight, self.lin_l.bias, self.lin_r.weight, self.lin_r.bias
        if post_affine is not None and self.add_self_loops:
            scale, shift = post_affine
            w_l, b_l = w_l * scale[:, None], b_l * scale
            w_r, b_r = w_r * scale[:, None], b_r * scale + shift
        out = self._conv(x, edge_index, w_l, b_l, w_r, b_r, want_colsums)
        if post_affine is not None and not self.add_self_loops:
            out = out * post_affine[0] + post_affine[1]
        return out

    def _conv(self, x, edge_index, w_l, b_l, w_r, b_r, want_colsums=False):
        mode = LOOPS_REMOVE_ADD if self.add_self_loops else LOOPS_KEEP
        graph = get_graph(edge_index, x.size(0), mode)
        if self.add_self_loops and ops.fused_linear_ok(graph, self.in_channels, self.out_channels, root=True, x=x):
            return ops.propagate_linear(x, graph, "mean", w_l, b_l + b_r, root_weight=w_r, want_colsums=want_colsums)
        fused_left = self.add_self_loops and ops.fused_linear_ok(graph, self.in_channels, self.out_channels, x=x)
        input_layer = not x.requires_grad and self.add_self_loops and self.in_channels <= self.out_channels
        if x.is_cuda and not getattr(graph, "is_distributed", False) and not fused_left and not input_layer:
            return self._conv_rows(x, graph, w_l, b_l, w_r, b_r, want_colsums)
        x_r = ops.linear(ops.target_rows(x, graph), w_r, b_r)
        if fused_left:
            return ops.propagate_linear(x, graph, "mean", w_l, b_l) + x_r
        if input_layer:
            return ops.linear(ops.propagate_mean(x, graph), w_l, b_l) + x_r
        x_l = ops.linear(x, w_l, b_l)
        return ops.propagate_mean(x_l, graph) + x_r

    def _conv_rows(self, x, graph, w_l, b_l, w_r, b_r, want_colsums):
        h, n = self._transform_both(x, w_l, b_l, w_r, b_r)
        out = ops.propagate_rows(h, graph, "mean", n=n, want_colsums=want_colsums and n == self.out_channels)
        return out if n == self.out_channels else out[:, :self.out_channels]


class GATConv(nn.Module):

    def __init__(self, in_channels, out_channels, heads=1, concat=True, negative_slope=0.2):
        super().__init__()
        self.in_channels, self.out_channels = in_channels, out_channels
        self.heads, self.concat, self.negative_slope = heads, concat, negative_slope
        self.lin_src = nn.Linear(in_channels, heads * out_channels, bias=False)
        self.lin_dst = self.lin_src
        self.att_src = nn.Parameter(torch.empty(1, heads, out_channels))
        self.att_dst = nn.Parameter(torch.empty(1, heads, out_channels))
        self.bias = nn.Parameter(torch.zeros(heads * out_channels if concat else out_channels))
        self.reset_parameters()

    def reset_parameters(self):
        glorot_(self.lin_src.weight)
        glorot_(self.att_src)
        glorot_(self.att_dst)
        nn.init.zeros_(self.bias)

    folds_post_affine = True
    accepts_ce = True

    @staticmethod
    def kernel_channels(C):
        if C <= 64 or (C % 2 == 0 and C <= 128) or (C % 4 == 0 and C <= 256):
            return C
        Cp = (C + 3) // 4 * 4
        if Cp > 256:
            raise NotImplementedError(f"GATConv: {C} channels per head; the attention kernels take at most 256")
        return Cp

    def forward(self, x, edge_index, post_affine=None, ce=None):
        H, C = self.heads, self.out_channels
        Cp = self.kernel_channels(C)
        if Cp == C:
            return self._forward(x, edge_index, self.lin_src.weight, self.att_src, self.att_dst, self.bias, C, post_affine, ce)
        pad = torch.nn.functional.pad
        in_kernel = self.concat or H == 1
        weight = pad(self.lin_src.weight.view(H, C, -1), (0, 0, 0, Cp - C)).reshape(H * Cp, -1)
        bias = pad(self.bias.view(H, C), (0, Cp - C)).reshape(-1) if in_kernel else pad(self.bias, (0, Cp - C))
        out = self._forward(x, edge_index, weight, pad(self.att_src, (0, Cp - C)), pad(self.att_dst, (0, Cp - C)), bias, Cp,
                            None, None)
        out = out.view(-1, H, Cp)[:, :, :C].reshape(-1, H * C) if (self.concat and H > 1) else out[:, :C]
        if post_affine is not None:
            out = out * post_affine[0] + post_affine[1]
        return out if ce is None else ops.ce_from_logits(out, ce[0], ce[1])

    def _forward(self, x, edge_index, weight, att_src, att_dst, bias, C, post_affine, ce):
        H = self.heads
        graph = get_graph(edge_index, x.size(0), LOOPS_REMOVE_ADD)
        if (H == 1 and post_affine is None
                and ops.gat_linear_ok(graph, self.in_channels, C, x, None if ce is None else ce[0])):
            return ops.gat_attend_linear(x, weight, att_src, att_dst, graph, self.negative_slope, bias=bias, ce=ce)
        if ce is not None:
            return ops.ce_from_logits(self._forward(x, edge_index, weight, att_src, att_dst, bias, C, post_affine, None),
                                      ce[0], ce[1])
        in_kernel = self.concat or H == 1
        dist_resident = getattr(graph, "is_distributed", False) and graph.is_resident(x)
        if dist_resident:
            out = graph.gat(x, att_src, att_dst, H, C, self.negative_slope, weight=weight)
            out = out + bias if in_kernel else out.view(-1, H, C).mean(dim=1) + bias
        else:
            h = ops.linear(x, weight)
            if in_kernel and post_affine is not None and not getattr(graph, "is_distributed", False):
                scale, shift = post_affine
                return ops.gat_attend(h, att_src, att_dst, graph, H, C, self.negative_slope,
                                      bias=bias * scale + shift, out_scale=scale)
            out = ops.gat_attend(h, att_src, att_dst, graph, H, C, self.negative_slope,
                                 bias=bias if in_kernel else None)
            if not in_kernel:
                out = out.view(-1, H, C).mean(dim=1) + bias
        if post_affine is not None:
            out = out * post_affine[0] + post_affine[1]
        return out


class APPNP(nn.Module):

    def __init__(self, K, alpha):
        super().__init__()
        self.K, self.alpha = K, alpha

    def forward(self, x, edge_index, edge_weight=None):
        _no_weight_grad(edge_weight, "APPNP")
        graph = get_graph(edge_index, x.size(0), LOOPS_ADD_REMAINING, edge_weight)
        return ops.appnp_propagate(x, graph, self.K, self.alpha)


class SGConv(nn.Module):

    def __init__(self, in_channels, out_channels, K=1, cached=False, add_self_loops=True, bias=True):
        super().__init__()
        self.in_channels, self.out_channels, self.K = in_channels, out_channels, K
        self.cached, self.add_self_loops = cached, add_self_loops
        self.lin = nn.Linear(in_channels, out_channels, bias=bias)
        self._cached_x = None

    def forward(self, x, edge_index, edge_weight=None):
        _no_weight_grad(edge_weight, "SGConv")
        h = self._cached_x
        if h is None:
            mode = LOOPS_ADD_REMAINING if self.add_self_loops else LOOPS_KEEP
            graph = get_graph(edge_index, x.size(0), mode, edge_weight)
            if not self.cached and self.in_channels > self.out_channels:
                out = ops.appnp_propagate(ops.linear(x, self.lin.weight), graph, self.K, 0.0)
                return out if self.lin.bias is None else out + self.lin.bias
            h = ops.appnp_propagate(x, graph, self.K, 0.0)
            if self.cached:
                self._cached_x = h if h.requires_grad else h.detach()
        return ops.linear(h, self.lin.weight, self.lin.bias)


class GINConv(nn.Module):

    def __init__(self, nn_module, eps=0.0, train_eps=False):
        super().__init__()
        self.nn = nn_module
        self.initial_eps = eps
        if train_eps:
            self.eps = nn.Parameter(torch.tensor([float(eps)]))
        else:
            self.register_buffer("eps", torch.tensor([float(eps)]))

    def forward(self, x, edge_index):
        graph = get_graph(edge_index, x.size(0), LOOPS_KEEP)
        first = self.nn[0] if isinstance(self.nn, nn.Sequential) and len(self.nn) else None
        if (isinstance(first, nn.Linear) and x.is_cuda
                and ops.fused_linear_ok(graph, first.in_features, first.out_features, root=True, x=x)):
            h = ops.propagate_linear(x, graph, "sum", first.weight, first.bias,
                                     root_weight=(1 + self.eps) * first.weight)
            for layer in list(self.nn)[1:]:
                h = layer(h)
            return h
        if isinstance(first, nn.Linear) and first.in_features > first.out_features:
            h = ops.linear(x, first.weight)
# ... 216 lines not shown
```

rgb_experiment_amd/ops.py:

```python
import ctypes

import torch

from . import _lib

_EVENT_SINK = None


def set_event_sink(sink):
    global _EVENT_SINK
    _EVENT_SINK = sink


class Kind(str):
    variant = None


class _Timed:
    def __init__(self, kind, variant=None):
        if variant is not None and _EVENT_SINK is not None:
            kind = Kind(kind)
            kind.variant = variant
        self.kind = kind

# ... 759 lines not shown
                                 _lib.ptr(ce_scratch), groups)
        if select_rows and not dense and w_pos is None:
            if grad_scale is not None:
                ce_arg.skip_unselected = 1
            elif not want_z and z is None and mask is not None:
                rows = selected_rows(y, mask, n_out)
                if rows is not None:
                    ce_arg.rows, ce_arg.n_rows = rows.data_ptr(), rows.numel()
                    keep.append(rows)
        keep += [y, mask, ce_scratch, ce_arg]
        L.ce = ctypes.addressof(ce_arg)
        want_out = grad_scale is not None
    if out is not None:
        if tuple(out.shape) != (N, n_out) or out.stride(1) != 1 or out.dtype != torch.float32:
            raise RuntimeError(f"fused_layer: out is {tuple(out.shape)}, expected a float32 [{N}, {n_out}] with contiguous rows")
    elif want_out:
        out = torch.empty((N, n_out), dtype=torch.float32, device=x.device)
    if out is not None:
        L.out, L.ldo = out.data_ptr(), out.stride(0) if N > 1 else n_out
    else:
        L.ldo = n_out
    if out_blocked is not None:
        L.out_blk, L.ob_cols, L.ob_stride = _blocked(out_blocked, "out_blocked")
        if out_blocked.size(1) != N or out_blocked.size(0) * out_blocked.size(2) != n_out:
            raise RuntimeError(f"fused_layer: out_blocked is {tuple(out_blocked.shape)} for a [{N}, {n_out}] output")
    if z is not None:
        if tuple(z.shape) != (N, K) or z.stride(1) != 1 or z.dtype != torch.float32:
            raise RuntimeError(f"fused_layer: z is {tuple(z.shape)}, expected a float32 [{N}, {K}] with contiguous rows")
    elif want_z or w_pos is not None:
        z = torch.empty((N, K), dtype=torch.float32, device=x.device)
    L.ldz = K
    if z is not None:
        L.z_out, L.ldz = z.data_ptr(), z.stride(0) if N > 1 else K
    z_pos = None
    if w_pos is not None:
        _lib.require_device(w_pos)
        z_pos = torch.empty_strided((N, K), (L.ldz, 1), dtype=torch.float32, device=x.device)
        keep.append(w_pos)
        L.w_pos, L.z_pos_out = w_pos.data_ptr(), z_pos.data_ptr()
    colsums = None
    if want_colsums:
        nbytes = ctypes.c_size_t(0)
        _lib.check(lib.rgbx_spmm_linear_stats_workspace_bytes(N, n_out, ctypes.byref(nbytes)),
                   "rgbx_spmm_linear_stats_workspace_bytes")
        ws = torch.empty(max(nbytes.value, 8), dtype=torch.uint8, device=x.device)
        colsums = torch.empty((2, n_out), dtype=torch.float64, device=x.device)
        keep.append(ws)
        L.out_colsums, L.stats_ws, L.stats_ws_bytes = colsums.data_ptr(), ws.data_ptr(), nbytes.value
    L.N, L.K, L.Nout = N, K, n_out
    variant = None
    if _EVENT_SINK is not None:
        variant = "+".join([name for name, on in (
            ("dense", dense), ("pre", pre is not None), ("root", wt_root is not None), ("z", z is not None),
            ("zpos", w_pos is not None), ("stats", want_colsums), ("ce_stats", ce is not None and ce[2] is None),
            ("ce_grad", ce is not None and ce[2] is not None), ("noout", out is None and out_blocked is None and ce is None),
            ("blk", out_blocked is not None)) if on]) or "plain"
    with _Timed(kind, variant):
        _lib.check(lib.rgbx_fused_layer_f32(ctypes.byref(L), _lib.stream_ptr()), "rgbx_fused_layer_f32")
    del keep
    if groups == 2:
        ce_stats = ce_stats.view(2, 3)
    return out, (z if w_pos is None else (z, z_pos)), (ce_stats if ce is not None else colsums)


def blocked_to_rows(src, out=None, bias=None):
    _lib.require_device(src, bias)
    ptr, bc, bs = _blocked(src, "src")
    n, d = src.size(1), src.size(0) * src.size(2)
    if out is None:
        out = torch.empty((n, d), dtype=torch.float32, device=src.device)
    b = None if bias is None else bias.detach().contiguous()
    _lib.check(_lib.load().rgbx_blocked_to_rows_f32(ptr, bc, bs, out.data_ptr(), out.stride(0), n, d, _lib.ptr(b),
                                                    _lib.stream_ptr()), "rgbx_blocked_to_rows_f32")
    return out


def spmm_linear_raw(csr, w, rs, x, wt, bias=None, want_z=False, x_root=None, wt_root=None, kind="linear", pre=None,
                    want_colsums=False, ce=None, select_rows=False):
    out, z, extra = fused_layer(x, wt, csr=csr, w=w, rs=rs, bias=bias, x_root=x_root if wt_root is not None else None,
                                wt_root=wt_root, pre=pre, want_z=want_z, want_colsums=want_colsums, ce=ce, kind=kind,
                                select_rows=select_rows)
    if ce is not None or want_colsums:
        return out, z, extra
    return out, z


class _AggregateLinear(torch.autograd.Function):

    @staticmethod
    def forward(ctx, z, weight, bias, root_weight, x_root, want_colsums):
        out, _, cs = fused_layer(z, weight_t(weight), bias=None if bias is None else bias.detach(),
                                 x_root=x_root if root_weight is not None else None,
                                 wt_root=None if root_weight is None else weight_t(root_weight),
                                 want_colsums=want_colsums, kind="cached_aggregate_linear_fwd")
        ctx.save_for_backward(z, x_root if root_weight is not None else None)
        ctx.has_bias = bias is not None
        if want_colsums:
            ctx.mark_non_differentiable(cs)
            return out, cs
        return out

    @staticmethod
    def backward(ctx, gy, _g_cs=None):
        z, x_root = ctx.saved_tensors
        gy = gy.contiguous()
        gw = gb = gwr = None
        want_b = ctx.has_bias and ctx.needs_input_grad[2]
        if ctx.needs_input_grad[1]:
            if want_b:
                gw, gb = gemm_tn(gy, z, colsum=True)
            else:
                gw = gemm_tn(gy, z)
        elif want_b:
            gb = gy.sum(0)
        if x_root is not None and ctx.needs_input_grad[3]:
            gwr = gemm_tn(gy, x_root)
        return None, gw, gb, gwr, None, None


def aggregate_linear_ok(in_channels, out_channels, root=False):
    return bool(_lib.load().rgbx_spmm_linear_supported(in_channels, out_channels, int(root)))


def aggregate_linear(z, weight, bias=None, root_weight=None, x_root=None, want_colsums=False):
    return _tag_colsums(_AggregateLinear.apply(z, weight, bias, root_weight, x_root, want_colsums), want_colsums)


def fold_bn_linear(weight, bias=None, bias2=None, root_weight=None, bn=None):
    _lib.require_device(weight, bias, bias2, root_weight)
    W = weight.detach()
    W = W if W.stride(-1) == 1 else W.contiguous()
    n_out, K = W.shape
    Wr = None
    if root_weight is not None:
        Wr = root_weight.detach()
        Wr = Wr if Wr.stride(-1) == 1 else Wr.contiguous()
    wt = torch.empty((K, n_out), dtype=torch.float32, device=W.device)
    wrt = torch.empty_like(wt) if Wr is not None else None
    has_b = bias is not None or bias2 is not None or bn is not None
    b_out = torch.empty(n_out, dtype=torch.float32, device=W.device) if has_b else None
    c = lambda t: None if t is None else t.detach().contiguous()
    b1, b2 = c(bias), c(bias2)
    g = be = rm = rv = None
    eps = 0.0
    if bn is not None:
        g, be, rm, rv, eps = c(bn.weight), c(bn.bias), c(bn.running_mean), c(bn.running_var), bn.eps
    _lib.check(_lib.load().rgbx_fold_bn_linear_f32(
        _lib.ptr(W), W.stride(0), _lib.ptr(Wr), 0 if Wr is None else Wr.stride(0), _lib.ptr(b1), _lib.ptr(b2),
        _lib.ptr(g), _lib.ptr(be), _lib.ptr(rm), _lib.ptr(rv), float(eps), _lib.ptr(wt), _lib.ptr(wrt), _lib.ptr(b_out),
        n_out, K, _lib.stream_ptr()), "rgbx_fold_bn_linear_f32")
    return wt, b_out, wrt


class _PropagateLinear(torch.autograd.Function):

    @staticmethod
    def forward(ctx, x, graph, kind, weight, bias, need_z=True, root_weight=None, x_root=None, want_colsums=False):
        x = x.contiguous()
        xr = x if x_root is None else x_root.contiguous()
        w = graph.w if kind == "gcn" else None
        rs = graph.inv_deg if kind == "mean" else None
        if kind not in ("gcn", "mean", "sum"):
            raise ValueError(kind)
        res = spmm_linear_raw(graph.fwd, w, rs, x, weight_t(weight), None if bias is None else bias.detach(),
                              need_z, xr if root_weight is not None else None,
                              None if root_weight is None else weight_t(root_weight),
                              kind=f"{getattr(graph, 'event_prefix', '')}{kind}_linear_fwd", want_colsums=want_colsums)
        out, z = res[0], res[1]
        ctx.save_for_backward(z, weight, root_weight, xr if root_weight is not None else None)
        ctx.graph, ctx.kind, ctx.has_bias = graph, kind, bias is not None
        if want_colsums:
            ctx.mark_non_differentiable(res[2])
            return out, res[2]
        return out

    @staticmethod
    def backward(ctx, gy, _g_colsums=None):
        z, weight, root_weight, x = ctx.saved_tensors
        g, kind = ctx.graph, ctx.kind
        gy = gy.contiguous()
        gx = gw = gb = gwr = None
        want_b = ctx.has_bias and ctx.needs_input_grad[4]
        if ctx.needs_input_grad[3]:
            if want_b:
                gw, gb = gemm_tn(gy, z, colsum=True)
            else:
                gw = gemm_tn(gy, z)
        elif want_b:
            gb = gy.sum(0)
        if root_weight is not None and ctx.needs_input_grad[6]:
            gwr = gemm_tn(gy, x)
        if ctx.needs_input_grad[0]:
            gx = _propagate_linear_input_grad(g, kind, gy, weight, root_weight)
        return gx, None, None, gw, gb, None, gwr, None, None


def _propagate_linear_input_grad(g, kind, gy, weight, root_weight, ce_sel=None):
    csr = g.bwd
    wt = {"gcn": lambda: g.w_t, "mean": lambda: g.w_mean_t, "sum": lambda: None}[kind]()
    prefix = getattr(g, "event_prefix", "")
    n_out, n_in = weight.shape
    if n_out <= n_in and _lib.load().rgbx_spmm_linear_supported(n_out, n_in, int(root_weight is not None)):
        gx, _, _ = fused_layer(gy, weight.detach().contiguous(), csr=csr, w=wt,
                               x_root=gy if root_weight is not None else None,
                               wt_root=None if root_weight is None else root_weight.detach().contiguous(),
                               col_sel=None if ce_sel is None else selected_cols(*ce_sel), kind=f"{prefix}{kind}_linear_bwd")
        return gx
    gz = gy @ weight
    gr = gy @ root_weight if root_weight is not None else None
    if gr is None:
        return spmm_raw(csr, wt, None, gz, kind=f"{prefix}{kind}_bwd")
    return spmm_raw(csr, wt, None, gz, y=gr, a=1.0, b=1.0, out=gr, kind=f"{prefix}{kind}_bwd")


class _BNPropagateLinear(torch.autograd.Function):

    @staticmethod
    def forward(ctx, x, bn_weight, bn_bias, graph, kind, weight, bias, root_weight, eps, reduce, running, need_z,
                colsums=None, want_colsums=False):
        from .nn import batchnorm as B
        x = x.contiguous()
        mean, rstd, scale, shift, n = B.train_statistics(x, bn_weight, bn_bias, eps, reduce, running, colsums)
        w, rs = (graph.w, None) if kind == "gcn" else (None, graph.inv_deg)
        res = spmm_linear_raw(graph.fwd, w, rs, x, weight_t(weight), None if bias is None else bias.detach(), need_z,
                              x if root_weight is not None else None,
                              None if root_weight is None else weight_t(root_weight), kind=f"{kind}_linear_fwd",
                              pre=(scale, shift, graph.rowsum(kind)), want_colsums=want_colsums)
        out, z = res[0], res[1]
        ctx.save_for_backward(x, bn_weight, mean, rstd, n, z, weight, root_weight, scale, shift)
        ctx.graph, ctx.kind, ctx.has_bias, ctx.reduce = graph, kind, bias is not None, reduce
        if want_colsums:
            ctx.mark_non_differentiable(res[2])
            return out, res[2]
        return out

    @staticmethod
    def backward(ctx, gy, _g_colsums=None):
        from .nn import batchnorm as B
        x, bn_weight, mean, rstd, n, z, weight, root_weight, scale, shift = ctx.saved_tensors
        g, kind = ctx.graph, ctx.kind
        gy = gy.contiguous()
        gw = gb = gwr = None
        if ctx.needs_input_grad[5]:
            gw, gcol = gemm_tn(gy, z, colsum=True)
            gb = gcol if ctx.has_bias and ctx.needs_input_grad[6] else None
        else:
            gcol = gy.sum(0)
            gb = gcol if ctx.has_bias and ctx.needs_input_grad[6] else None
        if root_weight is not None and ctx.needs_input_grad[7]:
            gwr = gemm_tn(gy, x) * scale + gcol[:, None] * shift
        g_h = _propagate_linear_input_grad(g, kind, gy, weight, root_weight)
        gx, g_bnw, g_bnb = B.train_backward(g_h, x, bn_weight, mean, rstd, n, ctx.reduce)
        return gx, g_bnw, g_bnb, None, None, gw, gb, gwr, None, None, None, None, None, None


_SCALE_CACHE = {}


def mask_scale(y, mask, C):
    key = (y.data_ptr(), y._version, y.numel(), None if mask is None else (mask.data_ptr(), mask._version), int(C))
    hit = _SCALE_CACHE.get(key)
    if hit is None:
        sel = (y >= 0) & (y < C)
        if mask is not None:
            sel = sel & mask.bool()
        hit = (_MadeOn((1.0 / sel.sum().double()).float().reshape(1)), y, mask)
        _SCALE_CACHE[key] = hit
        while len(_SCALE_CACHE) > 32:
            _SCALE_CACHE.pop(next(iter(_SCALE_CACHE)))
    return hit[0].get()


_GROUP_MASKS = {}


def group_masks(mask_a, mask_b):
    _lib.require_device(mask_a, mask_b)
    key = (mask_a.data_ptr(), mask_a._version, mask_b.data_ptr(), mask_b._version, mask_a.numel())
    hit = _GROUP_MASKS.get(key)
    if hit is None:
        g = (mask_a.bool().to(torch.uint8) | (mask_b.bool().to(torch.uint8) << 1)).contiguous()
        hit = (_MadeOn(g), mask_a, mask_b)
        _GROUP_MASKS[key] = hit
        while len(_GROUP_MASKS) > 16:
            _GROUP_MASKS.pop(next(iter(_GROUP_MASKS)))
    return hit[0].get()


def ce_selection(y, mask, C):
    sel = (y >= 0) & (y < C)
    if mask is not None:
        sel = sel & mask.bool()
    return sel


def _sel_key(y, mask, C):
    return (y.data_ptr(), y._version, y.numel(),
            None if mask is None else (mask.data_ptr(), mask._version, mask.numel()), int(C))


_SEL_ROWS = {}


def selected_rows(y, mask, C):
    key = _sel_key(y, mask, C)
    hit = _SEL_ROWS.get(key)
    if hit is None:
        if torch.cuda.is_current_stream_capturing():
            return None
        rows = ce_selection(y, mask, C).nonzero().reshape(-1).to(torch.int32).contiguous()
        hit = (_MadeOn(rows), y, mask)
        _SEL_ROWS[key] = hit
        while len(_SEL_ROWS) > 16:
            _SEL_ROWS.pop(next(iter(_SEL_ROWS)))
    return hit[0].get()


_SEL_COLS = {}


def selected_cols(y, mask, C):
    key = _sel_key(y, mask, C)
    hit = _SEL_COLS.get(key)
    if hit is None:
        if torch.cuda.is_current_stream_capturing():
            return None
        hit = (_MadeOn(ce_selection(y, mask, C).to(torch.uint8).contiguous()), y, mask)
        _SEL_COLS[key] = hit
        while len(_SEL_COLS) > 16:
            _SEL_COLS.pop(next(iter(_SEL_COLS)))
    return hit[0].get()



def ce_from_logits(logits, y, mask):
    if isinstance(mask, (tuple, list)):
        return None, torch.stack([masked_ce_accuracy(logits, y, m) for m in mask])
    if torch.is_grad_enabled() and logits.requires_grad:
        return masked_ce_loss(logits, y, mask, with_stats=True)
    stats = masked_ce_accuracy(logits, y, mask)
    return (stats[0] / stats[1]).float(), stats


def fused_ce_ok(graph, in_channels, out_channels, root, x, y):
    return (not _is_dist(graph) and out_channels <= 128 and y is not None and y.is_cuda and y.dtype == torch.int64
            and fused_linear_ok(graph, in_channels, out_channels, root=root, x=x))


class _PropagateLinearCE(torch.autograd.Function):

    @staticmethod
    def forward(ctx, x, graph, kind, weight, bias, root_weight, y, mask, want_grad, bn_weight, bn_bias, bn_args):
        from .nn import batchnorm as B
        x = x.contiguous()
        pre = None
        if bn_weight is not None:
            eps, reduce, running, colsums = bn_args
            mean, rstd, scale, shift, n = B.train_statistics(x, bn_weight, bn_bias, eps, reduce, running, colsums)
            pre = (scale, shift, graph.rowsum(kind))
        w, rs = (graph.w, None) if kind == "gcn" else (None, graph.inv_deg)
        grad_scale = mask_scale(y, mask, weight.size(0)) if want_grad else None
        dlogits, z, stats = spmm_linear_raw(
            graph.fwd, w, rs, x, weight_t(weight), None if bias is None else bias.detach(),
            want_grad and weight.requires_grad, x if root_weight is not None else None,
            None if root_weight is None else weight_t(root_weight), kind=f"{kind}_linear_fwd", pre=pre,
            ce=(y, mask, grad_scale), select_rows=True)
        ctx.graph, ctx.kind, ctx.has_bias, ctx.has_bn = graph, kind, bias is not None, bn_weight is not None
        ctx.ce_sel = (y, mask, weight.size(0)) if want_grad else None
        if want_grad:
            if ctx.has_bn:
                ctx.save_for_backward(dlogits, z, weight, root_weight, x, bn_weight, mean, rstd, n, scale, shift)
                ctx.reduce = bn_args[1]
            else:
                ctx.save_for_backward(dlogits, z, weight, root_weight, x if root_weight is not None else None)
        ctx.mark_non_differentiable(stats)
        if stats.dim() == 2:
            return stats.new_zeros(()).float(), stats
        return (stats[0] / stats[1]).float(), stats

    @staticmethod
    def backward(ctx, g, _g_stats):
        from .nn import batchnorm as B
        saved = ctx.saved_tensors
        if ctx.has_bn:
            gy, z, weight, root_weight, x, bn_weight, mean, rstd, n, scale, shift = saved
        else:
            gy, z, weight, root_weight, x = saved
        graph, kind = ctx.graph, ctx.kind
        g = g.reshape(()).float()
        gw = gb = gwr = gx = g_bnw = g_bnb = None
        gcol = None
        if ctx.needs_input_grad[3]:
            gw, gcol = gemm_tn(gy, z, colsum=True)
        if ctx.has_bias and ctx.needs_input_grad[4]:
            gb = gcol if gcol is not None else gy.sum(0)
        if root_weight is not None and ctx.needs_input_grad[5]:
            if ctx.has_bn:
                gcol = gcol if gcol is not None else gy.sum(0)
                gwr = gemm_tn(gy, x) * scale + gcol[:, None] * shift
            else:
                gwr = gemm_tn(gy, x)
        need_h = ctx.needs_input_grad[0] or (ctx.has_bn and (ctx.needs_input_grad[9] or ctx.needs_input_grad[10]))
        items = [(k, t) for k, t in (("gw", gw), ("gb", gb), ("gwr", gwr)) if t is not None]
        if need_h:
            items.append(("w", weight.detach()))
            if root_weight is not None:
                items.append(("wr", root_weight.detach()))
        sc = dict(zip((k for k, _ in items), torch._foreach_mul([t for _, t in items], g))) if items else {}
        gw, gb, gwr = sc.get("gw"), sc.get("gb"), sc.get("gwr")
        if need_h:
            g_h = _propagate_linear_input_grad(graph, kind, gy, sc["w"], sc.get("wr"), ce_sel=ctx.ce_sel)
            if ctx.has_bn:
                gx, g_bnw, g_bnb = B.train_backward(g_h, x, bn_weight, mean, rstd, n, ctx.reduce)
            else:
                gx = g_h
        return gx, None, None, gw, gb, gwr, None, None, None, g_bnw, g_bnb, None


def propagate_linear_ce(x, graph, kind, weight, bias, root_weight, y, mask, bn=None, colsums=None):
    want_grad = not isinstance(mask, (tuple, list)) and torch.is_grad_enabled() and any(
        t is not None and t.requires_grad
        for t in (weight, x, bias, root_weight) + ((bn.weight, bn.bias) if bn is not None else ()))
    if bn is not None:
        bn_args = (bn.eps, bn._reduce, bn.begin_training_step(), colsums)
        return _PropagateLinearCE.apply(x, graph, kind, weight, bias, root_weight, y, mask, want_grad, bn.weight, bn.bias,
                                        bn_args)
    return _PropagateLinearCE.apply(x, graph, kind, weight, bias, root_weight, y, mask, want_grad, None, None, None)


def bn_propagate_linear(x, bn, graph, kind, weight, bias=None, root_weight=None, colsums=None, want_colsums=False):
    need_z = weight.requires_grad
    return _tag_colsums(_BNPropagateLinear.apply(x, bn.weight, bn.bias, graph, kind, weight, bias, root_weight, bn.eps,
                                                 bn._reduce, bn.begin_training_step(), need_z, colsums, want_colsums),
                        want_colsums)


COLSUMS = "_rgbx_colsums"


def _tag_colsums(res, want_colsums):
    if not want_colsums:
        return res
    out, colsums = res
    setattr(out, COLSUMS, colsums)
    return out


def propagate_linear(x, graph, kind, weight, bias=None, root_weight=None, want_colsums=False):
    if _is_dist(graph):
        return graph.propagate_linear(x, kind, weight, bias, root_weight)
    need_z = torch.is_grad_enabled() and weight.requires_grad
    return _tag_colsums(_PropagateLinear.apply(x, graph, kind, weight, bias, need_z, root_weight, None, want_colsums),
                        want_colsums)


def appnp_raw(csr, w, h, K, alpha, kind="appnp"):
    _lib.require_device(h)
    h = h.contiguous()
    ph, ldh = _lib.mat(h, "h")
    out = torch.empty_like(h)
    tmp = torch.empty_like(h) if K > 1 else None
    po, ldo = _lib.mat(out, "out")
    split, _scratch = csr.split_arg(h.size(1), h.device)
    with _Timed(kind):
        _lib.check(
            _lib.load().rgbx_appnp_f32(_lib.ptr(csr.rowptr), _lib.ptr(csr.col), _lib.ptr(w), ph, ldh, po,
                                       _lib.ptr(tmp), ldo, csr.N, h.size(1), int(K), float(alpha),
                                       None if split is None else ctypes.byref(split), _lib.stream_ptr()),
            "rgbx_appnp_f32")
    return out


class _APPNP(torch.autograd.Function):

    @staticmethod
    def forward(ctx, h, graph, K, alpha):
        ctx.graph, ctx.K, ctx.alpha = graph, K, alpha
        return appnp_raw(graph.fwd, graph.w, h, K, alpha, kind="appnp_fwd")

    @staticmethod
    def backward(ctx, gy):
        g = ctx.graph
        return appnp_raw(g.bwd, g.w_t, gy, ctx.K, ctx.alpha, kind="appnp_bwd"), None, None, None


class _APPNPCE(torch.autograd.Function):

    @staticmethod
    def forward(ctx, h, graph, K, alpha, labels, mask, n_classes, want_grad):
        h = h.contiguous()
        z = appnp_raw(graph.fwd, graph.w, h, K - 1, alpha, kind="appnp_fwd") if K > 1 else h
        grad_scale = mask_scale(labels, mask, n_classes) if want_grad else None
        dlogits, stats = spmm_epilogue_raw(graph.fwd, graph.w, None, z, y=h, a=1.0 - alpha, b=alpha,
                                           ce=(labels, mask, grad_scale), n_classes=n_classes, kind="appnp_fwd")
        ctx.graph, ctx.K, ctx.alpha = graph, K, alpha
        if want_grad:
            ctx.save_for_backward(dlogits)
        ctx.mark_non_differentiable(stats)
        if stats.dim() == 2:
            return stats.new_zeros(()).float(), stats
        return (stats[0] / stats[1]).float(), stats

    @staticmethod
    def backward(ctx, g, _g_stats=None):
        if not ctx.saved_tensors:
            raise RuntimeError("appnp_propagate_ce: backward asked of a forward that was run without want_grad")
        gy = ctx.saved_tensors[0] * g.reshape(()).float()
        gr = ctx.graph
        return appnp_raw(gr.bwd, gr.w_t, gy, ctx.K, ctx.alpha, kind="appnp_bwd"), None, None, None, None, None, None, None


def appnp_propagate_ce(h, graph, K, alpha, n_classes, y, mask):
    pair = isinstance(mask, (tuple, list))
    want_grad = (not pair) and torch.is_grad_enabled() and h.requires_grad
    loss, stats = _APPNPCE.apply(h, graph, int(K), float(alpha), y, mask, int(n_classes), want_grad)
    return (None if pair else loss), stats


def appnp_propagate(h, graph, K, alpha):
    if _is_dist(graph):
        out = graph.appnp(h, K, alpha)
        if out is not None:
            return out
        z = h
        for _ in range(K):
            z = (1.0 - alpha) * graph.propagate(z, "gcn") + alpha * h
        return z
    hp, d = _pad4(h)
    out = _APPNP.apply(hp, graph, K, alpha)
    return out if hp is h else out[:, :d]


class _DAGNNProp(torch.autograd.Function):

    @staticmethod
    def forward(ctx, x, graph, K, s, b):
        lib = _lib.load()
        N, d = x.shape
        x = x.contiguous()
        hops = torch.empty((K, N, d), dtype=torch.float32, device=x.device)
        src = x
        for k in range(K):
            spmm_raw(graph.fwd, graph.w, None, src, out=hops[k], kind="gcn_fwd")
            src = hops[k]
        out = torch.empty_like(x)
        sv = s.detach().reshape(-1).contiguous()
        bv = None if b is None else b.detach().reshape(-1).contiguous()
        with _Timed("dagnn_gate_fwd"):
            _lib.check(lib.rgbx_dagnn_gate_fwd_f32(_lib.ptr(x), x.stride(0), _lib.ptr(hops), N * d, d, _lib.ptr(sv),
                                                   _lib.ptr(bv), _lib.ptr(out), out.stride(0), N, d, K,
                                                   _lib.stream_ptr()), "rgbx_dagnn_gate_fwd_f32")
        ctx.graph, ctx.K, ctx.has_b = graph, K, b is not None
        ctx.save_for_backward(x, hops, sv, bv)
        return out

    @staticmethod
    def backward(ctx, gout):
        lib = _lib.load()
        x, hops, sv, bv = ctx.saved_tensors
        g, K = ctx.graph, ctx.K
        N, d = x.shape
        gout = gout.contiguous()
        d0 = torch.empty_like(x)
        dk = torch.empty((K, N, d), dtype=torch.float32, device=x.device)
        g_s = torch.empty(d, dtype=torch.float32, device=x.device)
        g_b = torch.empty(1, dtype=torch.float32, device=x.device) if ctx.has_b else None
        need = ctypes.c_size_t(0)
        _lib.check(lib.rgbx_dagnn_gate_bwd_workspace_bytes(d, ctypes.byref(need)), "rgbx_dagnn_gate_bwd_workspace_bytes")
        ws = torch.empty(need.value, dtype=torch.uint8, device=x.device)
        with _Timed("dagnn_gate_bwd"):
            _lib.check(lib.rgbx_dagnn_gate_bwd_f32(_lib.ptr(x), x.stride(0), _lib.ptr(hops), N * d, d, _lib.ptr(sv),
                                                   _lib.ptr(bv), _lib.ptr(gout), gout.stride(0), _lib.ptr(d0),
                                                   d0.stride(0), _lib.ptr(dk), N * d, d, _lib.ptr(g_s), _lib.ptr(g_b),
                                                   _lib.ptr(ws), need.value, N, d, K, _lib.stream_ptr()),
                       "rgbx_dagnn_gate_bwd_f32")
        gx = None
        if ctx.needs_input_grad[0]:
            cur = dk[K - 1] if K else d0
            for k in range(K - 1, -1, -1):
                dst = dk[k - 1] if k else d0
                spmm_raw(g.bwd, g.w_t, None, cur, y=dst, a=1.0, b=1.0, out=dst, kind="gcn_bwd")
                cur = dst
            gx = d0
        return gx, None, None, g_s, g_b


def dagnn_prop(x, graph, K, proj_weight, proj_bias=None):
    if _is_dist(graph) or x.size(1) > 256:
        return None
    _lib.require_device(x, proj_weight, proj_bias)
    xp, d = _pad4(x)
    s = proj_weight.reshape(-1)
    if xp is not x:
        s = torch.nn.functional.pad(s, (0, xp.size(1) - d))
    out = _DAGNNProp.apply(xp, graph, int(K), s, proj_bias)
    return out if xp is x else out[:, :d]



GRU_FORMS = ("fused", "composed", "general")
GRU_FORM = None


def gru_step_supported(C):
    return bool(_lib.load().rgbx_gru_step_supported(int(C)))

# ... 807 lines not shown
                                                        _lib.stream_ptr()), "rgbx_faconv_edge_dot_f32")


class _FAConv(torch.autograd.Function):

    @staticmethod
    def forward(ctx, x, x0, att_l, att_r, graph, eps, train, p_drop, form, record):
        _lib.require_device(x, x0, att_l, att_r)
        lib = _lib.load()
        csr, N, dev = graph.fwd, graph.fwd.N, x.device
        x = x.contiguous()
        C = x.size(1)
        if x.size(0) != N:
            raise RuntimeError(f"faconv: {x.size(0)} feature rows for a graph of {N} nodes")
        use_x0 = x0 is not None and eps != 0.0
        x0c = x0.contiguous() if use_x0 else None
        att = torch.cat([att_l.detach().reshape(1, C), att_r.detach().reshape(1, C)]).contiguous()
        seed = None
        if train and p_drop > 0.0:
            seed = torch.randint(0, 2 ** 31 - 1, (2,), dtype=torch.int32, device=dev)
        if record is not None:
            record.update(seed=seed, p_drop=float(p_drop))
        alr = torch.empty((N, 2), dtype=torch.float32, device=dev)
        px, ldx = _lib.mat(x, "x")
        with _Timed("faconv_scores"):
            _lib.check(lib.rgbx_faconv_scores_f32(px, ldx, att[0].data_ptr(), att[1].data_ptr(), _lib.ptr(alr), N, C,
                                                  _lib.stream_ptr()), "rgbx_faconv_scores_f32")
        if form == "fused":
            out = torch.empty((N, C), dtype=torch.float32, device=dev)
            po, ldo = _lib.mat(out, "out")
            p0, ld0 = _lib.mat(x0c, "x_0") if use_x0 else (None, 0)
            split, _scratch = csr.split_arg(C + 1, dev)
            with _Timed("faconv_fwd"):
                _lib.check(lib.rgbx_faconv_fwd_f32(_lib.ptr(csr.rowptr), _lib.ptr(csr.col), _lib.ptr(graph.w), px, ldx,
                                                   _lib.ptr(alr), p0, ld0, float(eps), po, ldo, N, C, _lib.ptr(seed),
                                                   float(p_drop), None if split is None else ctypes.byref(split),
                                                   _lib.stream_ptr()), "rgbx_faconv_fwd_f32")
        else:
            coef, _ = _faconv_edge_coef(csr, graph.w, None, alr, 0, seed, p_drop, False)
            out = spmm_raw(csr, coef, None, x, y=x0c, a=1.0, b=float(eps), kind="faconv_fwd_composed")
        ctx.graph, ctx.eps, ctx.p_drop, ctx.form, ctx.use_x0 = graph, float(eps), float(p_drop), form, use_x0
        ctx.att_shapes = (att_l.shape, att_r.shape)
        ctx.save_for_backward(x, alr, att, seed)
        return out

    @staticmethod
    def backward(ctx, gout):
        x, alr, att, seed = ctx.saved_tensors
        g, p_drop = ctx.graph, ctx.p_drop
        lib = _lib.load()
        N, C, dev = x.size(0), x.size(1), x.device
        gout = gout.contiguous()
        g_alr = torch.empty((N, 2), dtype=torch.float32, device=dev)
        px, ldx = _lib.mat(x, "x")
        pg, ldg = _lib.mat(gout, "gout")
        t2f = g.t2f if seed is not None else None
        if ctx.form == "fused":
            g_x = torch.empty_like(x)
            pgx, ldgx = _lib.mat(g_x, "g_x")
            split, _scratch = g.fwd.split_arg(C + 1, dev)
            with _Timed("faconv_bwd_dst"):
                _lib.check(lib.rgbx_faconv_bwd_dst_f32(_lib.ptr(g.fwd.rowptr), _lib.ptr(g.fwd.col), _lib.ptr(g.w), px, ldx,
                                                       _lib.ptr(alr), pg, ldg, _lib.ptr(g_alr), N, C, _lib.ptr(seed), p_drop,
                                                       None if split is None else ctypes.byref(split),
                                                       _lib.stream_ptr()), "rgbx_faconv_bwd_dst_f32")
            split, _scratch2 = g.bwd.split_arg(C + 1, dev)
            with _Timed("faconv_bwd_src"):
                _lib.check(lib.rgbx_faconv_bwd_src_f32(_lib.ptr(g.bwd.rowptr), _lib.ptr(g.bwd.col), _lib.ptr(g.w_t),
                                                       _lib.ptr(t2f), px, ldx, _lib.ptr(alr), pg, ldg, att[0].data_ptr(),
                                                       att[1].data_ptr(), _lib.ptr(g_alr), pgx, ldgx, N, C, _lib.ptr(seed),
                                                       p_drop, None if split is None else ctypes.byref(split),
                                                       _lib.stream_ptr()), "rgbx_faconv_bwd_src_f32")
        else:
            _, q = _faconv_edge_coef(g.fwd, g.w, None, alr, 0, seed, p_drop, True)
            _faconv_edge_dot(g.fwd, q, gout, x, g_alr, 1)
            coef_t, q_t = _faconv_edge_coef(g.bwd, g.w_t, t2f, alr, 1, seed, p_drop, True)
            _faconv_edge_dot(g.bwd, q_t, x, gout, g_alr, 0)
            g_x = torch.addmm(spmm_raw(g.bwd, coef_t, None, gout, kind="faconv_bwd_composed"), g_alr, att)
        g_att = gemm_tn(g_alr, x)
        g_x0 = gout * ctx.eps if ctx.use_x0 and ctx.needs_input_grad[1] else None
        return (g_x, g_x0, g_att[0].reshape(ctx.att_shapes[0]), g_att[1].reshape(ctx.att_shapes[1]), None, None, None,
                None, None, None)


def faconv(x, x0, att_l, att_r, graph, eps=0.1, training=False, p_drop=0.0, form=None, record=None):
    if _is_dist(graph):
        raise RuntimeError("FAConv has no node-partitioned form: run it on one GPU")
    _lib.require_device(x, x0, att_l, att_r)
    if not (0.0 <= p_drop < 1.0):
        raise ValueError("faconv: dropout must be in [0, 1)")
    return _FAConv.apply(x, x0, att_l, att_r, graph, float(eps), bool(training), float(p_drop),
                         faconv_form(x.size(1), form), record)


def _scores_in_kernel(C):
    vec = 4 if C % 4 == 0 else (2 if C % 2 == 0 else 1)
    lanes = 1
    while lanes * vec < C:
        lanes *= 2
    return lanes <= 8


def gather_rows(src, idx, out=None):
    _lib.require_device(src, idx)
    ps, lds = _lib.mat(src, "src")
    n, d = idx.numel(), src.size(1)
    if out is None:
        out = torch.empty((n, d), dtype=torch.float32, device=src.device)
    po, ldo = _lib.mat(out, "dst")
    _lib.check(_lib.load().rgbx_gather_rows_f32(ps, lds, _lib.ptr(idx), n, d, po, ldo, _lib.stream_ptr()),
               "rgbx_gather_rows_f32")
    return out


def scatter_add_rows(src, idx, dst):
    _lib.require_device(src, idx, dst)
    ps, lds = _lib.mat(src, "src")
    pd, ldd = _lib.mat(dst, "dst")
    _lib.check(
        _lib.load().rgbx_scatter_add_rows_f32(ps, lds, _lib.ptr(idx), idx.numel(), src.size(1), pd, ldd,
                                              _lib.stream_ptr()), "rgbx_scatter_add_rows_f32")
    return dst



def gemm_tn(a, b, alpha=1.0, colsum=False, out=None, sums_out=None):
    _lib.require_device(a, b)
    a = a if a.stride(-1) == 1 and _rows_padded_readable(a) else a.contiguous()
    b = b if b.stride(-1) == 1 and _rows_padded_readable(b) else b.contiguous()
    if a.size(0) >= 4096:
        a, b = (_aligned_rows(t) for t in (a, b))
    pa, lda = _lib.mat(a, "a")
    pb, ldb = _lib.mat(b, "b")
    K, M, N = a.size(0), a.size(1), b.size(1)
    lib = _lib.load()
    nbytes = ctypes.c_size_t(0)
    _lib.check(lib.rgbx_gemm_tn_workspace_bytes(K, M, N, ctypes.byref(nbytes)), "rgbx_gemm_tn_workspace_bytes")
    ws = torch.empty(max(nbytes.value, 1), dtype=torch.uint8, device=a.device)
    if out is None:
        out = torch.empty((M, N), dtype=torch.float32, device=a.device)
    elif tuple(out.shape) != (M, N) or not out.is_contiguous() or out.dtype != torch.float32:
        raise RuntimeError(f"gemm_tn: out must be a contiguous float32 [{M}, {N}] tensor")
    sums = None
    if colsum:
        sums = sums_out if sums_out is not None else torch.empty(M, dtype=torch.float32, device=a.device)
        if tuple(sums.shape) != (M,) or not sums.is_contiguous() or sums.dtype != torch.float32:
            raise RuntimeError(f"gemm_tn: sums_out must be a contiguous float32 [{M}] tensor")
    with _Timed("gemm_tn", f"{M}x{N}" if _EVENT_SINK is not None else None):
        _lib.check(lib.rgbx_gemm_tn_f32(pa, lda, pb, ldb, _lib.ptr(out), N, _lib.ptr(sums), K, M, N, float(alpha),
                                        _lib.ptr(ws), ws.numel(), _lib.stream_ptr()), "rgbx_gemm_tn_f32")
    return (out, sums) if colsum else out


class _Linear(torch.autograd.Function):

    @staticmethod
    def forward(ctx, x, weight, bias):
        ctx.save_for_backward(x, weight)
        ctx.has_bias = bias is not None
        if _EVENT_SINK is None or not x.is_cuda:
            return torch.nn.functional.linear(x, weight, bias)
        with _Timed("linear_fwd", f"{weight.size(1)}->{weight.size(0)}"):
            return torch.nn.functional.linear(x, weight, bias)

    @staticmethod
    def backward(ctx, gy):
        x, weight = ctx.saved_tensors
        gy = gy.contiguous()
        gx = gy @ weight if ctx.needs_input_grad[0] else None
        gw = gb = None
        want_b = ctx.has_bias and ctx.needs_input_grad[2]
        if ctx.needs_input_grad[1] and gy.is_cuda and want_b:
            gw, gb = gemm_tn(gy, x, colsum=True)
        else:
            if ctx.needs_input_grad[1]:
                gw = gemm_tn(gy, x) if gy.is_cuda else gy.t() @ x
            gb = gy.sum(0) if want_b else None
        return gx, gw, gb


def linear(x, weight, bias=None):
    sp = getattr(x, "_rgbx_sparse", None)
    if sp is not None and not x.requires_grad:
        return _SparseRowsLinear.apply(sp, weight, bias)
    return _Linear.apply(x, weight, bias)


SHORT_ROWS_TABLE_BYTES = 2 << 20
SHORT_ROWS_MEAN_SLOTS = 64


def short_rows_ok(csr, table):
    d = table.size(1)
    return (table.is_cuda and d % 4 == 0 and 4 <= d <= 64 and table.numel() * 4 <= SHORT_ROWS_TABLE_BYTES
            and csr.nnz <= SHORT_ROWS_MEAN_SLOTS * max(csr.N, 1))


def spmm_short_rows_raw(csr, w, x, bias=None, kind="spmm"):
    _lib.require_device(x, w, bias)
    px, ldx = _lib.mat(x, "x")
    N, d = csr.N, x.size(1)
    out = torch.empty((N, d), dtype=torch.float32, device=x.device)
    with _Timed(kind, f"shortrows+d{d}" if _EVENT_SINK is not None else None):
        _lib.check(_lib.load().rgbx_spmm_csr_short_rows_f32(_lib.ptr(csr.rowptr), _lib.ptr(csr.col), _lib.ptr(w), px, ldx,
                                                            _lib.ptr(bias), _lib.ptr(out), d, N, d, _lib.stream_ptr()),
                   "rgbx_spmm_csr_short_rows_f32")
    return out


class SparseFeatures:
    requires_grad = False

    def __init__(self, sp, like):
        self._rgbx_sparse, self.shape, self.device, self.dtype, self.is_cuda = sp, like.shape, like.device, like.dtype, True

    def size(self, dim=None):
        return self.shape if dim is None else self.shape[dim]

    def dim(self):
        return len(self.shape)


def dropout(x, p, training):
    sp = getattr(x, "_rgbx_sparse", None)
    if sp is None or not training or p <= 0.0 or x.requires_grad:
        return torch.nn.functional.dropout(x, p=p, training=training)
    if p >= 1.0:
        return SparseFeatures(sp.with_values(torch.zeros_like(sp.val)), x)
    keep = torch.rand(sp.val.numel(), device=sp.val.device) >= p
    return SparseFeatures(sp.with_values(sp.val * keep * (1.0 / (1.0 - p))), x)


class SparseRows:

    def __init__(self, x):
        from .graph import CSR, make_row_split
        _lib.require_device(x)
        n, f = x.shape
        step = max(1, (1 << 28) // max(f, 1))
        rows, cols, vals = [], [], []
        for r0 in range(0, n, step):
            blk = x[r0:r0 + step]
            nz = blk.nonzero(as_tuple=False)
            rows.append(nz[:, 0] + r0)
            cols.append(nz[:, 1].contiguous())
            vals.append(blk[nz[:, 0], nz[:, 1]])
        rows, cols, vals = (torch.cat(t).contiguous() if t else x.new_zeros(0, dtype=dt)
                            for t, dt in ((rows, torch.int64), (cols, torch.int64), (vals, x.dtype)))
        self.n, self.f, self.nnz = n, f, int(rows.numel())
        if self.nnz >= 2 ** 31 - 1:
            raise RuntimeError("SparseRows: more than 2^31 non-zeros")
        i32 = lambda t: t.to(torch.int32).contiguous()

        def rowptr_of(idx, m):
            ptr = torch.zeros(m + 1, dtype=torch.int64, device=x.device)
            ptr[1:] = torch.cumsum(torch.bincount(idx, minlength=m), 0)
            return i32(ptr)

        pad = lambda t: t if t.numel() else t.new_zeros(1)
        ptr = rowptr_of(rows, n)
        self.fwd = CSR(ptr, pad(i32(cols)), None, n, self.nnz, make_row_split(ptr))
        self.val = pad(vals)
        order = torch.argsort(cols, stable=True)
        self.order = order
        ptr_t = rowptr_of(cols, f)
        self.bwd = CSR(ptr_t, pad(i32(rows[order])), None, f, self.nnz, make_row_split(ptr_t))
        self.val_t = pad(vals[order].contiguous())

    def with_values(self, vals):
        import copy
        other = copy.copy(self)
        other.val = vals.contiguous()
        other.val_t = vals[self.order].contiguous() if self.nnz else vals
        return other


class _SparseRowsLinear(torch.autograd.Function):

    @staticmethod
    def forward(ctx, sp, weight, bias):
        ctx.sp, ctx.has_bias = sp, bias is not None
        wt = weight.detach().t().contiguous()
        b = None if bias is None else bias.detach().contiguous()
        if short_rows_ok(sp.fwd, wt):
            return spmm_short_rows_raw(sp.fwd, sp.val, wt, bias=b, kind="features_fwd")
        return spmm_raw(sp.fwd, sp.val, None, wt, kind="features_fwd", bias=b)

    @staticmethod
    def backward(ctx, gy):
        sp = ctx.sp
        gy = gy.contiguous()
        gw = gb = None
        if ctx.needs_input_grad[1]:
            gw = spmm_raw(sp.bwd, sp.val_t, None, gy, kind="features_bwd").t()
        if ctx.has_bias and ctx.needs_input_grad[2]:
            gb = gy.sum(0)
        return None, gw, gb


def prepare_features(x, max_density=0.1):
    x = align_rows(x)
    if x.dim() == 2 and x.is_cuda and x.dtype == torch.float32 and not x.requires_grad and x.numel():
        step = max(1, (1 << 28) // x.size(1))
        nnz = sum(int(torch.count_nonzero(x[r0:r0 + step])) for r0 in range(0, x.size(0), step))
        if nnz <= max_density * x.numel() and nnz < 2 ** 31 - 1:
            x._rgbx_sparse = SparseRows(x)
# ... 134 lines not shown
```

Before: 16.01 billion.

## Fuse BN backward apply into weight-grad GEMM and restrict GEMM to selected rows

Adds two gemm_tn variants. The first applies the batch-norm input-gradient formula while loading the A tile, so the BN-backward output never has to be written to memory before the weight-gradient GEMM. The second gathers only the masked/selected rows, skipping the zero rows of the CE gradient. Python autograd gains a BN handover between layers so the next conv's backward owns the BN apply. The cost is extra complexity, an extra X tile load in the fused kernel, and gathered (non-contiguous) loads in the row variant.

```diff
diff --git a/include/rgbx_hip.h b/include/rgbx_hip.h
--- a/include/rgbx_hip.h
+++ b/include/rgbx_hip.h
@@ -345,6 +345,15 @@
                      float* a_colsum, int64_t K, int64_t M, int64_t N, float alpha, void* workspace,
                      size_t workspace_bytes, rgbx_stream_t stream);
 
+int rgbx_gemm_tn_bn_bwd_f32(const float* G, int64_t ldg, const float* X, int64_t ldx, const float* mean,
+                            const float* rstd, const float* ca, const float* cb, const float* ck, const float* B,
+                            int64_t ldb, float* C, int64_t ldc, float* a_colsum, int64_t K, int64_t M, int64_t N,
+                            float alpha, void* workspace, size_t workspace_bytes, rgbx_stream_t stream);
+
+int rgbx_gemm_tn_rows_f32(const float* A, int64_t lda, const float* B, int64_t ldb, const int32_t* rows,
+                          int64_t n_rows, float* C, int64_t ldc, float* a_colsum, int64_t K, int64_t M, int64_t N,
+                          float alpha, void* workspace, size_t workspace_bytes, rgbx_stream_t stream);
+
 
 int rgbx_bn_scratch_doubles(int64_t N, int64_t d, int64_t* count);
 
diff --git a/rgb_experiment_amd/_lib.py b/rgb_experiment_amd/_lib.py
--- a/rgb_experiment_amd/_lib.py
+++ b/rgb_experiment_amd/_lib.py
@@ -121,6 +121,9 @@
     "rgbx_gatv2_draws_u8": [_P, _I64, _I, _F, _P, _P],
     "rgbx_gemm_tn_workspace_bytes": [_I64, _I64, _I64, ctypes.POINTER(ctypes.c_size_t)],
     "rgbx_gemm_tn_f32": [_P, _I64, _P, _I64, _P, _I64, _P, _I64, _I64, _I64, _F, _P, ctypes.c_size_t, _P],
+    "rgbx_gemm_tn_bn_bwd_f32": [_P, _I64, _P, _I64, _P, _P, _P, _P, _P, _P, _I64, _P, _I64, _P, _I64, _I64, _I64, _F, _P,
+                                ctypes.c_size_t, _P],
+    "rgbx_gemm_tn_rows_f32": [_P, _I64, _P, _I64, _P, _I64, _P, _I64, _P, _I64, _I64, _I64, _F, _P, ctypes.c_size_t, _P],
     "rgbx_bn_scratch_doubles": [_I64, _I64, ctypes.POINTER(ctypes.c_int64)],
     "rgbx_bn_stats_f32": [_P, _I64, _I64, _I64, _P, _P, _I64, _P],
     "rgbx_bn_finalize_f32": [_P, _P, _P, _F, _F, _P, _P, _P, _P, _P, _P, _I64, _P],
diff --git a/rgb_experiment_amd/csrc/bn.hip b/rgb_experiment_amd/csrc/bn.hip
--- a/rgb_experiment_amd/csrc/bn.hip
+++ b/rgb_experiment_amd/csrc/bn.hip
@@ -147,7 +147,7 @@
     load_vec<VEC>(b, cb + c);
     load_vec<VEC>(k, ck + c);
 #pragma unroll
-    for (int i = 0; i < VEC; ++i) g[i] = (g[i] - a[i] - (v[i] - mu[i]) * rs[i] * b[i]) * k[i];
+    for (int i = 0; i < VEC; ++i) g[i] = bn_bwd_input_grad(g[i], v[i], mu[i], rs[i], a[i], b[i], k[i]);
     store_vec<VEC>(gx + r * ldgx + c, g);
   }
 }
diff --git a/rgb_experiment_amd/csrc/gemm.hip b/rgb_experiment_amd/csrc/gemm.hip
--- a/rgb_experiment_amd/csrc/gemm.hip
+++ b/rgb_experiment_amd/csrc/gemm.hip
@@ -4,6 +4,15 @@
 namespace {
 
 constexpr int BM = 128, BN = 128, KT = 32;
+enum { A_PLAIN = 0, A_BN = 1, A_ROWS = 2 };
+
+struct TnExtra {
+  const float* X;
+  int64_t ldx;
+  const float *mean, *rstd, *ca, *cb, *ck;
+  const int32_t* rows;
+  int64_t n_rows;
+};
 using f32x16 = __attribute__((ext_vector_type(16))) float;
 
 template <int W>
@@ -42,13 +51,61 @@
   }
 }
 
-template <bool VEC4, int MT>
+template <int W>
+__device__ __forceinline__ void put_tile_bn(float* __restrict__ lds, const float4 (&rg)[KT * (W / 4) / 256],
+                                            const float4 (&rx)[KT * (W / 4) / 256], const float* __restrict__ lc,
+                                            int64_t k0, int64_t k_end, int c0, int ncols) {
+#pragma unroll
+  for (int p = 0; p < KT * (W / 4) / 256; ++p) {
+    const int idx = p * 256 + threadIdx.x;
+    const int r = idx / (W / 4), c = (idx % (W / 4)) * 4;
+    float4 v = rg[p];
+    if (k0 + r < k_end && c0 + c < ncols) {
+      const float4 mu = *reinterpret_cast<const float4*>(lc + 0 * W + c);
+      const float4 rs = *reinterpret_cast<const float4*>(lc + 1 * W + c);
+      const float4 a = *reinterpret_cast<const float4*>(lc + 2 * W + c);
+      const float4 b = *reinterpret_cast<const float4*>(lc + 3 * W + c);
+      const float4 k = *reinterpret_cast<const float4*>(lc + 4 * W + c);
+      v.x = bn_bwd_input_grad(v.x, rx[p].x, mu.x, rs.x, a.x, b.x, k.x);
+      v.y = bn_bwd_input_grad(v.y, rx[p].y, mu.y, rs.y, a.y, b.y, k.y);
+      v.z = bn_bwd_input_grad(v.z, rx[p].z, mu.z, rs.z, a.z, b.z, k.z);
+      v.w = bn_bwd_input_grad(v.w, rx[p].w, mu.w, rs.w, a.w, b.w, k.w);
+    }
+    *reinterpret_cast<float4*>(lds + r * W + c) = v;
+  }
+}
+
+template <int W>
+__device__ __forceinline__ void fetch_tile_rows(float4 (&regs)[KT * (W / 4) / 256], const float* __restrict__ src,
+                                                int64_t ld, const int32_t* __restrict__ rows, int64_t j0, int64_t j_end,
+                                                int c0, int ncols) {
+#pragma unroll
+  for (int p = 0; p < KT * (W / 4) / 256; ++p) {
+    const int idx = p * 256 + threadIdx.x;
+    const int r = idx / (W / 4), c = (idx % (W / 4)) * 4;
+    const int64_t j = j0 + r;
+    regs[p] = make_float4(0.f, 0.f, 0.f, 0.f);
+    if (j < j_end && c0 + c < ncols) regs[p] = *reinterpret_cast<const float4*>(src + (int64_t)rows[j] * ld + c0 + c);
+  }
+}
+
+__device__ __forceinline__ int64_t lower_bound_rows(const int32_t* __restrict__ rows, int64_t n, int64_t key) {
+  int64_t lo = 0, hi = n;
+  while (lo < hi) {
+    const int64_t mid = (lo + hi) >> 1;
+    if (rows[mid] < key) lo = mid + 1; else hi = mid;
+  }
+  return lo;
+}
+
+template <bool VEC4, int MT, int MODE = A_PLAIN>
 __global__ void __launch_bounds__(256)
 gemm_tn_partial_kernel(const float* __restrict__ A, int64_t lda, const float* __restrict__ B, int64_t ldb,
                        float* __restrict__ part, float* __restrict__ colpart, int64_t K, int M, int N,
-                       int64_t slab) {
+                       int64_t slab, TnExtra ex) {
+  static_assert(MODE == A_PLAIN || VEC4, "the A_BN / A_ROWS forms exist on the 16-byte path only");
   constexpr int MI = MT / 64;
-  __shared__ float lds[KT * (MT + 128)];
+  __shared__ float lds[KT * (MT + 128) + (MODE == A_BN ? 5 * MT : 0)];
   float* la = lds;
   float* lb = lds + KT * MT;
   const int split = blockIdx.x;
@@ -88,7 +145,47 @@
       }
     }
   };
-  if constexpr (VEC4) {
+  if constexpr (MODE == A_BN) {
+    float* lc = lds + KT * (MT + 128);
+    for (int i = threadIdx.x; i < 5 * MT; i += 256) {
+      const float* src = i < MT ? ex.mean : i < 2 * MT ? ex.rstd : i < 3 * MT ? ex.ca : i < 4 * MT ? ex.cb : ex.ck;
+      const int c = m0 + i % MT;
+      lc[i] = c < M ? src[c] : 0.f;
+    }
+    float4 ra[KT * (MT / 4) / 256], rx[KT * (MT / 4) / 256], rb[KT * 32 / 256];
+    fetch_tile<MT>(ra, A, lda, k_begin, k_end, m0, M);
+    fetch_tile<MT>(rx, ex.X, ex.ldx, k_begin, k_end, m0, M);
+    fetch_tile<128>(rb, B, ldb, k_begin, k_end, n0, N);
+    for (int64_t k0 = k_begin; k0 < k_end; k0 += KT) {
+      __syncthreads();
+      put_tile_bn<MT>(la, ra, rx, lc, k0, k_end, m0, M);
+      put_tile<128>(lb, rb);
+      __syncthreads();
+      if (k0 + KT < k_end) {
+        fetch_tile<MT>(ra, A, lda, k0 + KT, k_end, m0, M);
+        fetch_tile<MT>(rx, ex.X, ex.ldx, k0 + KT, k_end, m0, M);
+        fetch_tile<128>(rb, B, ldb, k0 + KT, k_end, n0, N);
+      }
+      consume();
+    }
+  } else if constexpr (MODE == A_ROWS) {
+    const int64_t j_begin = lower_bound_rows(ex.rows, ex.n_rows, k_begin);
+    const int64_t j_end = lower_bound_rows(ex.rows, ex.n_rows, k_end);
+    float4 ra[KT * (MT / 4) / 256], rb[KT * 32 / 256];
+    fetch_tile_rows<MT>(ra, A, lda, ex.rows, j_begin, j_end, m0, M);
+    fetch_tile_rows<128>(rb, B, ldb, ex.rows, j_begin, j_end, n0, N);
+    for (int64_t j0 = j_begin; j0 < j_end; j0 += KT) {
+      __syncthreads();
+      put_tile<MT>(la, ra);
+      put_tile<128>(lb, rb);
+      __syncthreads();
+      if (j0 + KT < j_end) {
+        fetch_tile_rows<MT>(ra, A, lda, ex.rows, j0 + KT, j_end, m0, M);
+        fetch_tile_rows<128>(rb, B, ldb, ex.rows, j0 + KT, j_end, n0, N);
+      }
+      consume();
+    }
+  } else if constexpr (VEC4) {
     float4 ra[KT * (MT / 4) / 256], rb[KT * 32 / 256];
     fetch_tile<MT>(ra, A, lda, k_begin, k_end, m0, M);
     fetch_tile<128>(rb, B, ldb, k_begin, k_end, n0, N);
@@ -172,18 +269,34 @@
   return RGBX_OK;
 }
 
-extern "C" int rgbx_gemm_tn_f32(const float* A, int64_t lda, const float* B, int64_t ldb, float* C,
-                                int64_t ldc, float* a_colsum, int64_t K, int64_t M, int64_t N, float alpha,
-                                void* workspace, size_t workspace_bytes, rgbx_stream_t stream) {
-  if (K < 0 || M < 0 || N < 0) return fail(RGBX_E_ARG, "gemm_tn: negative size");
+namespace rgbx {
+namespace {
+
+int run_gemm_tn(const char* name, int mode, const float* A, int64_t lda, const float* B, int64_t ldb, float* C,
+                int64_t ldc, float* a_colsum, int64_t K, int64_t M, int64_t N, float alpha, void* workspace,
+                size_t workspace_bytes, rgbx_stream_t stream, const TnExtra& ex) {
+  if (K < 0 || M < 0 || N < 0) return fail(RGBX_E_ARG, "%s: negative size", name);
   if (M == 0 || N == 0) return RGBX_OK;
-  if (!C || (K > 0 && (!A || !B))) return fail(RGBX_E_ARG, "gemm_tn: null pointer");
-  if (M >= INT32_MAX || N >= INT32_MAX) return fail(RGBX_E_RANGE, "gemm_tn: M or N exceeds int32");
-  if (lda < M || ldb < N || ldc < N) return fail(RGBX_E_ARG, "gemm_tn: leading dimension too small");
+  if (!C || (K > 0 && (!A || !B))) return fail(RGBX_E_ARG, "%s: null pointer", name);
+  if (M >= INT32_MAX || N >= INT32_MAX) return fail(RGBX_E_RANGE, "%s: M or N exceeds int32", name);
+  if (lda < M || ldb < N || ldc < N) return fail(RGBX_E_ARG, "%s: leading dimension too small", name);
+  bool v4 = aligned16(A) && aligned16(B) && lda % 4 == 0 && ldb % 4 == 0;
+  if (mode == A_BN) {
+    if (K > 0 && (!ex.X || !ex.mean || !ex.rstd || !ex.ca || !ex.cb || !ex.ck))
+      return fail(RGBX_E_ARG, "%s: null pointer", name);
+    if (ex.ldx < M) return fail(RGBX_E_ARG, "%s: leading dimension too small", name);
+    v4 = v4 && aligned16(ex.X) && ex.ldx % 4 == 0;
+  }
+  if (mode == A_ROWS) {
+    if (ex.n_rows < 0 || ex.n_rows > K || (ex.n_rows > 0 && !ex.rows)) return fail(RGBX_E_ARG, "%s: bad row list", name);
+    if (K >= INT32_MAX) return fail(RGBX_E_RANGE, "%s: K exceeds int32", name);
+  }
+  if (mode != A_PLAIN && !v4)
+    return fail(RGBX_E_ALIGN, "%s: operands must be 16-byte aligned with leading dimensions that are multiples of 4", name);
   size_t need = 0;
   if (int rc = rgbx_gemm_tn_workspace_bytes(K, M, N, &need)) return rc;
   if (!workspace || workspace_bytes < need)
-    return fail(RGBX_E_WS, "gemm_tn: workspace %zu < %zu bytes", workspace_bytes, need);
+    return fail(RGBX_E_WS, "%s: workspace %zu < %zu bytes", name, workspace_bytes, need);
   hipStream_t s = (hipStream_t)stream;
   const int S = choose_splits(K, (int)M, (int)N);
   const int64_t slab = cdiv(cdiv(K > 0 ? K : 1, S), KT) * KT;
@@ -191,11 +304,12 @@
   float* colpart = a_colsum ? part + (size_t)S * M * N : nullptr;
   const int mt = tile_rows((int)M);
   dim3 grid(S, (unsigned)cdiv(M, mt), (unsigned)cdiv(N, BN));
-  const bool v4 = aligned16(A) && aligned16(B) && lda % 4 == 0 && ldb % 4 == 0;
-#define RGBX_GEMM_TN(V4, MT) \
-  gemm_tn_partial_kernel<V4, MT><<<grid, 256, 0, s>>>(A, lda, B, ldb, part, colpart, K, (int)M, (int)N, slab)
-  if (v4) { if (mt == 64) RGBX_GEMM_TN(true, 64); else RGBX_GEMM_TN(true, 128); }
-  else { if (mt == 64) RGBX_GEMM_TN(false, 64); else RGBX_GEMM_TN(false, 128); }
+#define RGBX_GEMM_TN(V4, MT, MODE) \
+  gemm_tn_partial_kernel<V4, MT, MODE><<<grid, 256, 0, s>>>(A, lda, B, ldb, part, colpart, K, (int)M, (int)N, slab, ex)
+  if (mode == A_BN) { if (mt == 64) RGBX_GEMM_TN(true, 64, A_BN); else RGBX_GEMM_TN(true, 128, A_BN); }
+  else if (mode == A_ROWS) { if (mt == 64) RGBX_GEMM_TN(true, 64, A_ROWS); else RGBX_GEMM_TN(true, 128, A_ROWS); }
+  else if (v4) { if (mt == 64) RGBX_GEMM_TN(true, 64, A_PLAIN); else RGBX_GEMM_TN(true, 128, A_PLAIN); }
+  else { if (mt == 64) RGBX_GEMM_TN(false, 64, A_PLAIN); else RGBX_GEMM_TN(false, 128, A_PLAIN); }
 #undef RGBX_GEMM_TN
   RGBX_CHECK_LAUNCH("gemm_tn_partial_kernel");
   const int64_t MN = M * N;
@@ -209,3 +323,34 @@
   }
   return RGBX_OK;
 }
+
+}
+}
+
+extern "C" int rgbx_gemm_tn_f32(const float* A, int64_t lda, const float* B, int64_t ldb, float* C,
+                                int64_t ldc, float* a_colsum, int64_t K, int64_t M, int64_t N, float alpha,
+                                void* workspace, size_t workspace_bytes, rgbx_stream_t stream) {
+  return run_gemm_tn("gemm_tn", A_PLAIN, A, lda, B, ldb, C, ldc, a_colsum, K, M, N, alpha, workspace, workspace_bytes,
+                     stream, TnExtra{});
+}
+
+extern "C" int rgbx_gemm_tn_bn_bwd_f32(const float* G, int64_t ldg, const float* X, int64_t ldx, const float* mean,
+                                       const float* rstd, const float* ca, const float* cb, const float* ck,
+                                       const float* B, int64_t ldb, float* C, int64_t ldc, float* a_colsum, int64_t K,
+                                       int64_t M, int64_t N, float alpha, void* workspace, size_t workspace_bytes,
+                                       rgbx_stream_t stream) {
+  TnExtra ex{};
+  ex.X = X, ex.ldx = ldx, ex.mean = mean, ex.rstd = rstd, ex.ca = ca, ex.cb = cb, ex.ck = ck;
+  return run_gemm_tn("gemm_tn_bn_bwd", A_BN, G, ldg, B, ldb, C, ldc, a_colsum, K, M, N, alpha, workspace,
+                     workspace_bytes, stream, ex);
+}
+
+extern "C" int rgbx_gemm_tn_rows_f32(const float* A, int64_t lda, const float* B, int64_t ldb, const int32_t* rows,
+                                     int64_t n_rows, float* C, int64_t ldc, float* a_colsum, int64_t K, int64_t M,
+                                     int64_t N, float alpha, void* workspace, size_t workspace_bytes,
+                                     rgbx_stream_t stream) {
+  TnExtra ex{};
+  ex.rows = rows, ex.n_rows = n_rows;
+  return run_gemm_tn("gemm_tn_rows", A_ROWS, A, lda, B, ldb, C, ldc, a_colsum, K, M, N, alpha, workspace,
+                     workspace_bytes, stream, ex);
+}
diff --git a/rgb_experiment_amd/csrc/rgbx_common.h b/rgb_experiment_amd/csrc/rgbx_common.h
--- a/rgb_experiment_amd/csrc/rgbx_common.h
+++ b/rgb_experiment_amd/csrc/rgbx_common.h
@@ -69,6 +69,10 @@
   *reinterpret_cast<V*>(p) = t;
 }
 
+__device__ __forceinline__ float bn_bwd_input_grad(float g, float x, float mu, float rs, float a, float b, float k) {
+  return __fmul_rn(fmaf(-b, __fmul_rn(__fsub_rn(x, mu), rs), __fsub_rn(g, a)), k);
+}
+
 constexpr int kMaxGrid = 256 * 8 * 4;
 
 }
diff --git a/rgb_experiment_amd/models/_stack.py b/rgb_experiment_amd/models/_stack.py
--- a/rgb_experiment_amd/models/_stack.py
+++ b/rgb_experiment_amd/models/_stack.py
@@ -143,6 +143,9 @@
             if affine is not None:
                 x = conv(x, edge_index, post_affine=affine, **ew)
             else:
+                if (extra.get("want_colsums") and getattr(conv, "owns_next_bn_backward", False)
+                        and hasattr(self.convs[i + 1], "forward_after_bn")):
+                    extra["next_bn"] = bn
                 x, pending = conv(x, edge_index, **extra), bn
         if ce is not None and not isinstance(x, tuple):
             x = ops.ce_from_logits(x, ce[0], ce[1])
diff --git a/rgb_experiment_amd/nn/batchnorm.py b/rgb_experiment_amd/nn/batchnorm.py
--- a/rgb_experiment_amd/nn/batchnorm.py
+++ b/rgb_experiment_amd/nn/batchnorm.py
@@ -115,6 +115,11 @@
 
 def train_backward(gy, x, weight, mean, rstd, n, reduce, grads_out=None, sums=None):
     gy = gy if gy.stride(-1) == 1 else gy.contiguous()
+    ca, cb, ck, gw, gb = train_backward_coefficients(gy, x, weight, mean, rstd, n, reduce, grads_out, sums)
+    return bwd_apply(gy, x, mean, rstd, ca, cb, ck), gw, gb
+
+
+def train_backward_coefficients(gy, x, weight, mean, rstd, n, reduce, grads_out=None, sums=None):
     d = x.size(1)
     if sums is None:
         local = bwd_sums(gy, x, mean, rstd)
@@ -139,7 +144,7 @@
             grads_out[0].copy_(gw)
             grads_out[1].copy_(gb)
             gw, gb = grads_out
-    return bwd_apply(gy, x, mean, rstd, ca, cb, ck), gw, gb
+    return ca, cb, ck, gw, gb
 
 
 class _AffineCols(torch.autograd.Function):
diff --git a/rgb_experiment_amd/nn/conv.py b/rgb_experiment_amd/nn/conv.py
--- a/rgb_experiment_amd/nn/conv.py
+++ b/rgb_experiment_amd/nn/conv.py
@@ -104,6 +104,7 @@
 
     folds_post_affine = True
     emits_colsums = True
+    owns_next_bn_backward = True
 
     def __init__(self, in_channels, out_channels):
         super().__init__()
@@ -119,14 +120,14 @@
     accepts_ce = True
     accepts_ce_pair = True
 
-    def forward(self, x, edge_index, edge_weight=None, post_affine=None, want_colsums=False, ce=None):
+    def forward(self, x, edge_index, edge_weight=None, post_affine=None, want_colsums=False, ce=None, next_bn=None):
         if ce is not None:
             return self._ce(x, edge_index, ce, None, None, edge_weight)
         weight, bias = self.lin.weight, self.bias
         if post_affine is not None:
             scale, shift = post_affine
             weight, bias = weight * scale[:, None], bias * scale + shift
-        return self._conv(x, edge_index, weight, bias, want_colsums, edge_weight)
+        return self._conv(x, edge_index, weight, bias, want_colsums, edge_weight, next_bn)
 
     def eval_operands(self, bn=None):
         return ops.fold_bn_linear(self.lin.weight, self.bias, bn=bn)
@@ -178,12 +179,12 @@
                                            want_colsums=want_colsums)
         return self.forward(bn(x, colsums=colsums), edge_index, edge_weight, want_colsums=want_colsums)
 
-    def _conv(self, x, edge_index, weight, bias, want_colsums=False, edge_weight=None):
+    def _conv(self, x, edge_index, weight, bias, want_colsums=False, edge_weight=None, next_bn=None):
         graph = get_graph(edge_index, x.size(0), LOOPS_ADD_REMAINING, edge_weight)
         if self._learned(edge_weight):
             return ops.propagate_gcn_edge_weight(ops.linear(x, weight), edge_weight, graph, bias=bias)
         if ops.fused_linear_ok(graph, self.in_channels, self.out_channels, x=x):
-            return ops.propagate_linear(x, graph, "gcn", weight, bias, want_colsums=want_colsums)
+            return ops.propagate_linear(x, graph, "gcn", weight, bias, want_colsums=want_colsums, next_bn=next_bn)
         if not x.requires_grad and self.in_channels <= self.out_channels:
             return ops.linear(ops.propagate_gcn(x, graph), weight, bias)
         if want_colsums and ops.rows_epilogue_ok(graph, self.out_channels, x):
@@ -195,6 +196,7 @@
 
     folds_post_affine = True
     emits_colsums = True
+    owns_next_bn_backward = True
 
     def __init__(self, in_channels, out_channels, aggr="mean"):
         super().__init__()
@@ -265,7 +267,7 @@
                                            root_weight=self.lin_r.weight, colsums=colsums, want_colsums=want_colsums)
         return self.forward(bn(x, colsums=colsums), edge_index, want_colsums=want_colsums)
 
-    def forward(self, x, edge_index, post_affine=None, want_colsums=False, ce=None):
+    def forward(self, x, edge_index, post_affine=None, want_colsums=False, ce=None, next_bn=None):
         if self.aggr != "mean":
             return _finish_composed(self._forward_composed(x, edge_index), post_affine, ce)
         if ce is not None:
@@ -276,7 +278,8 @@
             w_l, b_l, w_r = w_l * scale[:, None], b_l * scale + shift, w_r * scale[:, None]
         graph = get_graph(edge_index, x.size(0), LOOPS_KEEP)
         if ops.fused_linear_ok(graph, self.in_channels, self.out_channels, root=True, x=x):
-            return ops.propagate_linear(x, graph, "mean", w_l, b_l, root_weight=w_r, want_colsums=want_colsums)
+            return ops.propagate_linear(x, graph, "mean", w_l, b_l, root_weight=w_r, want_colsums=want_colsums,
+                                        next_bn=next_bn)
         if self.in_channels > self.out_channels and x.is_cuda and not getattr(graph, "is_distributed", False):
             h, n = self._transform_first(x, w_l, b_l, w_r)
             out = ops.propagate_rows(h, graph, "mean", n=n, want_colsums=want_colsums and n == self.out_channels)
@@ -294,6 +297,7 @@
 
     folds_post_affine = True
     emits_colsums = True
+    owns_next_bn_backward = True
 
     def __init__(self, in_channels, out_channels, add_self_loops=True, aggr="mean"):
         super().__init__()
@@ -373,7 +377,7 @@
                                                colsums=colsums, want_colsums=want_colsums)
         return self.forward(bn(x, colsums=colsums), edge_index, want_colsums=want_colsums)
 
-    def forward(self, x, edge_index, post_affine=None, want_colsums=False, ce=None):
+    def forward(self, x, edge_index, post_affine=None, want_colsums=False, ce=None, next_bn=None):
         if self.aggr != "mean":
             return _finish_composed(self._forward_composed(x, edge_index), post_affine, ce)
         if ce is not None:
@@ -383,16 +387,17 @@
             scale, shift = post_affine
             w_l, b_l = w_l * scale[:, None], b_l * scale
             w_r, b_r = w_r * scale[:, None], b_r * scale + shift
-        out = self._conv(x, edge_index, w_l, b_l, w_r, b_r, want_colsums)
+        out = self._conv(x, edge_index, w_l, b_l, w_r, b_r, want_colsums, next_bn)
         if post_affine is not None and not self.add_self_loops:
             out = out * post_affine[0] + post_affine[1]
         return out
 
-    def _conv(self, x, edge_index, w_l, b_l, w_r, b_r, want_colsums=False):
+    def _conv(self, x, edge_index, w_l, b_l, w_r, b_r, want_colsums=False, next_bn=None):
         mode = LOOPS_REMOVE_ADD if self.add_self_loops else LOOPS_KEEP
         graph = get_graph(edge_index, x.size(0), mode)
         if self.add_self_loops and ops.fused_linear_ok(graph, self.in_channels, self.out_channels, root=True, x=x):
-            return ops.propagate_linear(x, graph, "mean", w_l, b_l + b_r, root_weight=w_r, want_colsums=want_colsums)
+            return ops.propagate_linear(x, graph, "mean", w_l, b_l + b_r, root_weight=w_r, want_colsums=want_colsums,
+                                        next_bn=next_bn)
         fused_left = self.add_self_loops and ops.fused_linear_ok(graph, self.in_channels, self.out_channels, x=x)
         input_layer = not x.requires_grad and self.add_self_loops and self.in_channels <= self.out_channels
         if x.is_cuda and not getattr(graph, "is_distributed", False) and not fused_left and not input_layer:
diff --git a/rgb_experiment_amd/ops.py b/rgb_experiment_amd/ops.py
--- a/rgb_experiment_amd/ops.py
+++ b/rgb_experiment_amd/ops.py
@@ -935,10 +935,33 @@
     return wt, b_out, wrt
 
 
+FUSE_DENSE_BACKWARD = True
+
+BN_HANDOVER = "_rgbx_bn_handover"
+
+
+class BNHandover:
+    __slots__ = ("bn", "mean", "rstd", "n", "reduce")
+
+    def __init__(self, bn):
+        self.bn, self.mean, self.rstd, self.n, self.reduce = bn, None, None, None, None
+
+    def fill(self, mean, rstd, n, reduce):
+        self.mean, self.rstd, self.n, self.reduce = mean, rstd, n, reduce
+
+
+def _take_handover(x, bn):
+    rec = getattr(x, BN_HANDOVER, None)
+    if rec is None or rec.bn is not bn or rec.mean is not None or not x.requires_grad or not FUSE_DENSE_BACKWARD:
+        return None
+    return rec
+
+
 class _PropagateLinear(torch.autograd.Function):
 
     @staticmethod
-    def forward(ctx, x, graph, kind, weight, bias, need_z=True, root_weight=None, x_root=None, want_colsums=False):
+    def forward(ctx, x, graph, kind, weight, bias, need_z=True, root_weight=None, x_root=None, want_colsums=False,
+                bn_weight=None, bn_bias=None, handover=None):
         x = x.contiguous()
         xr = x if x_root is None else x_root.contiguous()
         w = graph.w if kind == "gcn" else None
@@ -950,8 +973,9 @@
                               None if root_weight is None else weight_t(root_weight),
                               kind=f"{getattr(graph, 'event_prefix', '')}{kind}_linear_fwd", want_colsums=want_colsums)
         out, z = res[0], res[1]
-        ctx.save_for_backward(z, weight, root_weight, xr if root_weight is not None else None)
-        ctx.graph, ctx.kind, ctx.has_bias = graph, kind, bias is not None
+        ctx.save_for_backward(z, weight, root_weight, xr if root_weight is not None else None,
+                              bn_weight if handover is not None else None, out if handover is not None else None)
+        ctx.graph, ctx.kind, ctx.has_bias, ctx.handover = graph, kind, bias is not None, handover
         if want_colsums:
             ctx.mark_non_differentiable(res[2])
             return out, res[2]
@@ -959,12 +983,24 @@
 
     @staticmethod
     def backward(ctx, gy, _g_colsums=None):
-        z, weight, root_weight, x = ctx.saved_tensors
+        z, weight, root_weight, x, bn_weight, y = ctx.saved_tensors
         g, kind = ctx.graph, ctx.kind
         gy = gy.contiguous()
-        gx = gw = gb = gwr = None
+        gx = gw = gb = gwr = g_bnw = g_bnb = None
         want_b = ctx.has_bias and ctx.needs_input_grad[4]
-        if ctx.needs_input_grad[3]:
+        rec, bn_a = ctx.handover, None
+        if rec is not None and rec.mean is not None:
+            from .nn import batchnorm as B
+            ca, cb, ck, g_bnw, g_bnb = B.train_backward_coefficients(gy, y, bn_weight, rec.mean, rec.rstd, rec.n,
+                                                                     rec.reduce)
+            if (ctx.needs_input_grad[0] or (root_weight is not None and ctx.needs_input_grad[6])
+                    or not ctx.needs_input_grad[3]):
+                gy = B.bwd_apply(gy, y, rec.mean, rec.rstd, ca, cb, ck)
+            else:
+                bn_a = (y, rec.mean, rec.rstd, ca, cb, ck)
+        if bn_a is not None:
+            gw, gb = gemm_tn_bn_bwd(gy, *bn_a, z, colsum=want_b)
+        elif ctx.needs_input_grad[3]:
             if want_b:
                 gw, gb = gemm_tn(gy, z, colsum=True)
             else:
@@ -975,7 +1011,7 @@
             gwr = gemm_tn(gy, x)
         if ctx.needs_input_grad[0]:
             gx = _propagate_linear_input_grad(g, kind, gy, weight, root_weight)
-        return gx, None, None, gw, gb, None, gwr, None, None
+        return gx, None, None, gw, gb, None, gwr, None, None, g_bnw, g_bnb, None
 
 
 def _propagate_linear_input_grad(g, kind, gy, weight, root_weight, ce_sel=None):
@@ -1000,10 +1036,13 @@
 
     @staticmethod
     def forward(ctx, x, bn_weight, bn_bias, graph, kind, weight, bias, root_weight, eps, reduce, running, need_z,
-                colsums=None, want_colsums=False):
+                colsums=None, want_colsums=False, handover=None):
         from .nn import batchnorm as B
         x = x.contiguous()
         mean, rstd, scale, shift, n = B.train_statistics(x, bn_weight, bn_bias, eps, reduce, running, colsums)
+        if handover is not None:
+            handover.fill(mean, rstd, n, reduce)
+        ctx.handed_over = handover is not None
         w, rs = (graph.w, None) if kind == "gcn" else (None, graph.inv_deg)
         res = spmm_linear_raw(graph.fwd, w, rs, x, weight_t(weight), None if bias is None else bias.detach(), need_z,
                               x if root_weight is not None else None,
@@ -1033,8 +1072,10 @@
         if root_weight is not None and ctx.needs_input_grad[7]:
             gwr = gemm_tn(gy, x) * scale + gcol[:, None] * shift
         g_h = _propagate_linear_input_grad(g, kind, gy, weight, root_weight)
+        if ctx.handed_over:
+            return g_h, None, None, None, None, gw, gb, gwr, None, None, None, None, None, None, None
         gx, g_bnw, g_bnb = B.train_backward(g_h, x, bn_weight, mean, rstd, n, ctx.reduce)
-        return gx, g_bnw, g_bnb, None, None, gw, gb, gwr, None, None, None, None, None, None
+        return gx, g_bnw, g_bnb, None, None, gw, gb, gwr, None, None, None, None, None, None, None
 
 
 _SCALE_CACHE = {}
@@ -1138,9 +1179,12 @@
         x = x.contiguous()
         pre = None
         if bn_weight is not None:
-            eps, reduce, running, colsums = bn_args
+            eps, reduce, running, colsums, handover = bn_args
             mean, rstd, scale, shift, n = B.train_statistics(x, bn_weight, bn_bias, eps, reduce, running, colsums)
             pre = (scale, shift, graph.rowsum(kind))
+            if handover is not None:
+                handover.fill(mean, rstd, n, reduce)
+        ctx.handed_over = bn_weight is not None and bn_args[4] is not None
         w, rs = (graph.w, None) if kind == "gcn" else (None, graph.inv_deg)
         grad_scale = mask_scale(y, mask, weight.size(0)) if want_grad else None
         dlogits, z, stats = spmm_linear_raw(
@@ -1174,7 +1218,8 @@
         gw = gb = gwr = gx = g_bnw = g_bnb = None
         gcol = None
         if ctx.needs_input_grad[3]:
-            gw, gcol = gemm_tn(gy, z, colsum=True)
+            rows = selected_rows(*ctx.ce_sel) if FUSE_DENSE_BACKWARD else None
+            gw, gcol = gemm_tn_rows(gy, z, rows, colsum=True)
         if ctx.has_bias and ctx.needs_input_grad[4]:
             gb = gcol if gcol is not None else gy.sum(0)
         if root_weight is not None and ctx.needs_input_grad[5]:
@@ -1193,7 +1238,7 @@
         gw, gb, gwr = sc.get("gw"), sc.get("gb"), sc.get("gwr")
         if need_h:
             g_h = _propagate_linear_input_grad(graph, kind, gy, sc["w"], sc.get("wr"), ce_sel=ctx.ce_sel)
-            if ctx.has_bn:
+            if ctx.has_bn and not ctx.handed_over:
                 gx, g_bnw, g_bnb = B.train_backward(g_h, x, bn_weight, mean, rstd, n, ctx.reduce)
             else:
                 gx = g_h
@@ -1205,7 +1250,7 @@
         t is not None and t.requires_grad
         for t in (weight, x, bias, root_weight) + ((bn.weight, bn.bias) if bn is not None else ()))
     if bn is not None:
-        bn_args = (bn.eps, bn._reduce, bn.begin_training_step(), colsums)
+        bn_args = (bn.eps, bn._reduce, bn.begin_training_step(), colsums, _take_handover(x, bn) if want_grad else None)
         return _PropagateLinearCE.apply(x, graph, kind, weight, bias, root_weight, y, mask, want_grad, bn.weight, bn.bias,
                                         bn_args)
     return _PropagateLinearCE.apply(x, graph, kind, weight, bias, root_weight, y, mask, want_grad, None, None, None)
@@ -1214,7 +1259,8 @@
 def bn_propagate_linear(x, bn, graph, kind, weight, bias=None, root_weight=None, colsums=None, want_colsums=False):
     need_z = weight.requires_grad
     return _tag_colsums(_BNPropagateLinear.apply(x, bn.weight, bn.bias, graph, kind, weight, bias, root_weight, bn.eps,
-                                                 bn._reduce, bn.begin_training_step(), need_z, colsums, want_colsums),
+                                                 bn._reduce, bn.begin_training_step(), need_z, colsums, want_colsums,
+                                                 _take_handover(x, bn)),
                         want_colsums)
 
 
@@ -1229,12 +1275,18 @@
     return out
 
 
-def propagate_linear(x, graph, kind, weight, bias=None, root_weight=None, want_colsums=False):
+def propagate_linear(x, graph, kind, weight, bias=None, root_weight=None, want_colsums=False, next_bn=None):
     if _is_dist(graph):
         return graph.propagate_linear(x, kind, weight, bias, root_weight)
     need_z = torch.is_grad_enabled() and weight.requires_grad
-    return _tag_colsums(_PropagateLinear.apply(x, graph, kind, weight, bias, need_z, root_weight, None, want_colsums),
-                        want_colsums)
+    if next_bn is None or not FUSE_DENSE_BACKWARD or not torch.is_grad_enabled():
+        return _tag_colsums(_PropagateLinear.apply(x, graph, kind, weight, bias, need_z, root_weight, None, want_colsums),
+                            want_colsums)
+    rec = BNHandover(next_bn)
+    out = _tag_colsums(_PropagateLinear.apply(x, graph, kind, weight, bias, need_z, root_weight, None, want_colsums,
+                                              next_bn.weight, next_bn.bias, rec), want_colsums)
+    setattr(out, BN_HANDOVER, rec)
+    return out
 
 
 def appnp_raw(csr, w, h, K, alpha, kind="appnp"):
@@ -2348,6 +2400,50 @@
     return (out, sums) if colsum else out
 
 
+def _gemm_tn_v4(*mats):
+    return all(t.is_cuda and t.dtype == torch.float32 and t.dim() == 2 and t.stride(1) == 1 and t.size(1) % 4 == 0
+               and t.stride(0) % 4 == 0 and t.stride(0) >= t.size(1) and t.data_ptr() % 16 == 0 for t in mats)
+
+
+def _gemm_tn_buffers(K, M, N, device, colsum):
+    nbytes = ctypes.c_size_t(0)
+    _lib.check(_lib.load().rgbx_gemm_tn_workspace_bytes(K, M, N, ctypes.byref(nbytes)), "rgbx_gemm_tn_workspace_bytes")
+    ws = torch.empty(max(nbytes.value, 1), dtype=torch.uint8, device=device)
+    out = torch.empty((M, N), dtype=torch.float32, device=device)
+    return ws, out, torch.empty(M, dtype=torch.float32, device=device) if colsum else None
+
+
+def gemm_tn_bn_bwd(g, x, mean, rstd, ca, cb, ck, b, colsum=False):
+    from .nn import batchnorm as B
+    _lib.require_device(g, x, b)
+    if not _gemm_tn_v4(g, x, b) or g.shape != x.shape:
+        res = gemm_tn(B.bwd_apply(g, x, mean, rstd, ca, cb, ck), b, colsum=colsum)
+        return res if colsum else (res, None)
+    K, M, N = g.size(0), g.size(1), b.size(1)
+    consts = [t.contiguous() for t in (mean, rstd, ca, cb, ck)]
+    ws, out, sums = _gemm_tn_buffers(K, M, N, g.device, colsum)
+    (pg, ldg), (px, ldx), (pb, ldb) = (_lib.mat(t, n) for t, n in ((g, "g"), (x, "x"), (b, "b")))
+    with _Timed("gemm_tn", f"{M}x{N}+bn_bwd" if _EVENT_SINK is not None else None):
+        _lib.check(_lib.load().rgbx_gemm_tn_bn_bwd_f32(
+            pg, ldg, px, ldx, *(_lib.ptr(t) for t in consts), pb, ldb, _lib.ptr(out), N, _lib.ptr(sums), K, M, N, 1.0,
+            _lib.ptr(ws), ws.numel(), _lib.stream_ptr()), "rgbx_gemm_tn_bn_bwd_f32")
+    return out, sums
+
+
+def gemm_tn_rows(a, b, rows, colsum=False):
+    _lib.require_device(a, b)
+    if rows is None or not _gemm_tn_v4(a, b) or a.size(0) != b.size(0) or a.size(0) >= 2**31:
+        return gemm_tn(a, b, colsum=colsum)
+    K, M, N = a.size(0), a.size(1), b.size(1)
+    ws, out, sums = _gemm_tn_buffers(K, M, N, a.device, colsum)
+    (pa, lda), (pb, ldb) = _lib.mat(a, "a"), _lib.mat(b, "b")
+    with _Timed("gemm_tn", f"{M}x{N}+rows" if _EVENT_SINK is not None else None):
+        _lib.check(_lib.load().rgbx_gemm_tn_rows_f32(
+            pa, lda, pb, ldb, _lib.ptr(rows), rows.numel(), _lib.ptr(out), N, _lib.ptr(sums), K, M, N, 1.0,
+            _lib.ptr(ws), ws.numel(), _lib.stream_ptr()), "rgbx_gemm_tn_rows_f32")
+    return (out, sums) if colsum else out
+
+
 class _Linear(torch.autograd.Function):
 
     @staticmethod
```

Result: faster. 16.32 billion, median of 6 (+1.9%).
